# YuliangXiu/ICON

Measured on AMD Instinct MI355X. Metric: query-points/sec at 256^3 grid, higher is better.
Workload: dtype f32 via 3x f16 split MFMA (22-bit operands, f32 accumulate)

## Files before the change

icon_amd/_lib.py:

```python
from __future__ import annotations

import ctypes as C
import os
import subprocess

_HERE = os.path.dirname(os.path.abspath(__file__))
LIB_PATH = os.environ.get("ICON_AMD_LIB") or os.path.join(_HERE, "libicon_amd.so")
CSRC = os.path.join(_HERE, "csrc")

PRIOR = {"icon": 0, "pamir": 1, "pifu": 2}
CMAP = {"reference": 0, "local": 1}
SEARCH = {"bvh": 0, "brute": 1}
PRECISION = {"f32": 0, "f16x3": 1}

SYMBOLS = [
    "icon_last_error", "icon_version", "icon_device_count",
    "icon_mesh_create", "icon_mesh_destroy", "icon_mesh_vertex_normals", "icon_mesh_stats",
    "icon_mesh_arena_bytes", "icon_mesh_create_arena", "icon_mesh_status", "icon_debug_set_mesh_build", "icon_debug_mesh_layout", "icon_debug_host_mesh_build",
    "icon_sdf_query",
    "icon_feat_create", "icon_feat_destroy", "icon_feat_set_smpl_feats",
    "icon_mlp_create", "icon_mlp_destroy", "icon_mlp_forward", "icon_mlp_set_last_op",
    "icon_work_create", "icon_work_destroy", "icon_work_profile", "icon_work_stage_ms", "icon_work_profile_detail", "icon_work_profile_workgroups", "icon_work_set_steal", "icon_work_set_reserve_cus",
    "icon_query_points", "icon_query_points_dcalib", "icon_query_rows", "icon_grid_rows",
    "icon_volume_any_above", "icon_adaptive_eval", "icon_adaptive_counts", "icon_adaptive_reruns", "icon_grid_eval_slab", "icon_grid_slab_features", "icon_grid_slab_finish", "icon_grid_slab_features_msg",
    "icon_grid_slab_finish_gathered", "icon_debug_set_shell_skip", "icon_debug_set_option", "icon_work_status", "icon_sdf_query_ties", "icon_work_set_tie_rule",
    "icon_export_mesh", "icon_mc_count", "icon_mc_emit", "icon_mc_count_range", "icon_mc_emit_keyed", "icon_debug_traversal_stats", "icon_debug_set_unfused",
    "icon_visibility", "icon_mesh_components", "icon_clean_mesh", "icon_semantic_voxelize",
    "icon_mesh_batch_create", "icon_mesh_batch_destroy", "icon_mesh_batch_status", "icon_feat_create_batch", "icon_query_points_batch",
    "icon_feat_batch_set_volume", "icon_semantic_voxelize_batch",
    "icon_query_color_bytes", "icon_query_color",
    "icon_render_bytes", "icon_render_normal",
    "icon_silhouette_bytes", "icon_silhouette_forward", "icon_silhouette_backward",
    "icon_render_normal_backward_bytes", "icon_render_normal_backward",
]

_lib = None


class IconAmdError(RuntimeError):
    pass


def build(force: bool = False) -> str:
    args = ["make", "-j8", "-C", CSRC] + (["-B"] if force else [])
    proc = subprocess.run(args, stdout=subprocess.PIPE, stderr=subprocess.STDOUT, text=True)
    if proc.returncode != 0:
        raise IconAmdError("building libicon_amd.so failed:\n" + proc.stdout[-4000:])
    return LIB_PATH


def lib():
    global _lib
    if _lib is not None:
        return _lib
    if not os.path.exists(LIB_PATH):
        raise IconAmdError(f"{LIB_PATH} not found - run `python -c 'import __graft_entry__ as g; g.build()'` "
                           "or `make -C icon_amd/csrc` (needs hipcc); there is no CPU fallback")
    import torch
    L = C.CDLL(LIB_PATH)
    L.icon_last_error.restype = C.c_char_p
    for name in SYMBOLS:
        if name != "icon_last_error":
            getattr(L, name).restype = C.c_int
    _lib = L
    return L


def check(rc: int, what: str = "") -> None:
    if rc != 0:
        msg = lib().icon_last_error().decode("utf-8", "replace")
        raise IconAmdError(f"{what or 'icon_amd'} failed (code {rc}): {msg}")


def device_count() -> int:
    return int(lib().icon_device_count())


def require_device() -> None:
    if device_count() < 1:
        raise IconAmdError("icon_amd needs a HIP device (MI355X); none is visible and there is no CPU fallback")


def ptr(t) -> C.c_void_p:
    if t is None:
        return C.c_void_p(0)
    if hasattr(t, "data_ptr"):
        assert t.is_contiguous(), "tensor must be contiguous"
        return C.c_void_p(t.data_ptr())
    return C.c_void_p(t.ctypes.data)
```

icon_amd/csrc/common.h:

```cpp
#pragma once
#include <hip/hip_runtime.h>
#include <stdint.h>
#include <functional>
#include <string>
#include <vector>

#include "../../include/icon_amd.h"

namespace icon {
constexpr int kWgRec = 6;
constexpr int kMaxProfGrid = 1024;

void set_error(const std::string &msg);
int fail(int code, const std::string &msg);

#define ICON_HIP(expr)                                                                          \
    do {                                                                                        \
        hipError_t _e = (expr);                                                                 \
        if (_e != hipSuccess)                                                                   \
            return ::icon::fail(ICON_ERR_HIP, std::string(#expr) + ": " + hipGetErrorString(_e)); \
    } while (0)

#define ICON_ARG(cond, msg)                                                  \
    do {                                                                     \
        if (!(cond)) return ::icon::fail(ICON_ERR_ARG, std::string(msg));    \
    } while (0)

struct alignas(64) BvhNode {
    float lo[3][2], hi[3][2];
    int32_t child0, child1;
    int32_t pad[2];
};
static_assert(sizeof(BvhNode) == 64, "BvhNode must be 64 bytes");

struct alignas(16) TriRec {
    float a[3], b[3], c[3];
    int32_t ia, ib, ic;
};
static_assert(sizeof(TriRec) == 48, "TriRec must be 48 bytes");

struct alignas(16) TriAttr {
    float n[3][3];
    float cm[3][3];
    float vis[3];
    int32_t face;
    int32_t pad[2];
};
static_assert(sizeof(TriAttr) == 96, "TriAttr must be 96 bytes");

struct alignas(32) TriPre {
    float a[3], b[3], ab[3], ac[3], bc[3];
    float i00, i11, ibc, a00, a01, a11, inn;
    int32_t face;
    int32_t pad;
};
static_assert(sizeof(TriPre) == 96, "TriPre must be 96 bytes");

struct alignas(32) LeafRec {
    float pair[2][24][2];
};
static_assert(sizeof(LeafRec) == 384, "LeafRec must be 384 bytes");

constexpr int kLeafMax = 4;
constexpr int kShareWavesMany = 8, kShareWavesFew = 16;
inline int share_waves(int64_t packets) { return packets <= 1500 ? kShareWavesFew : (packets <= 8000 ? kShareWavesMany : 1); }
constexpr int kStackDepth = 48;
constexpr int kXRow = 16;
constexpr int kCodeSlot = 15;

constexpr uint32_t kCodeOutlier = 1u;
constexpr uint32_t kCodeSignShift = 1;
constexpr uint32_t kCodeInCube = 8u;
constexpr uint32_t kCodeInside = 16u;

constexpr int kScanBlock = 256;
constexpr int kMaxWorld = 64;

struct MeshDyn {
    int32_t root;
    int32_t gy, gz;
    float bin_y0, bin_z0, bin_y1, bin_z1, bin_inv_y, bin_inv_z;
    float box_lo[3], box_hi[3];
    int32_t n_nodes, n_leaves, depth, bin_entries, max_bin;
    int32_t status;
    int32_t pad[11];
};
static_assert(sizeof(MeshDyn) == 128, "MeshDyn layout");
constexpr int kMeshBadFace = 1;
constexpr int kMeshBadVertex = 2;
constexpr int kMeshBinOverflow = 4;
constexpr int kMeshInternal = 8;
constexpr int kMeshBuilt = 0x100;

struct MeshDev {
    const BvhNode *nodes;
    const TriRec *tris;
    const TriAttr *attr;
    const int32_t *slot2face;
    const int32_t *face2slot;
    const LeafRec *leaves;
    const MeshDyn *dyn;
    int32_t n_tris;
    const int32_t *bin_start;
    const int32_t *bin_slots;
};

struct FeatDev {
    const float *planes;
    const float *vol;
    int32_t C, H, W, n_select, csel, cpad;
    int32_t Cv, Dv, Hv, Wv, vpad;
    int32_t smpl_mask;
};
constexpr int kSmplCmap = 1, kSmplNorm = 2;

struct BilinearTaps {
    int x0, y0;
    float nw, ne, sw, se;
    bool bx0, bx1, by0, by1;
};
__device__ __forceinline__ BilinearTaps bilinear_taps(float x, float y, int H, int W)
{
    BilinearTaps t;
    const float ix = ((x + 1.0f) / 2.0f) * (float)(W - 1);
    const float iy = ((y + 1.0f) / 2.0f) * (float)(H - 1);
    const float fx = floorf(ix), fy = floorf(iy);
    t.x0 = (int)fx; t.y0 = (int)fy;
    const int x1 = t.x0 + 1, y1 = t.y0 + 1;
    t.nw = ((float)x1 - ix) * ((float)y1 - iy);
    t.ne = (ix - (float)t.x0) * ((float)y1 - iy);
    t.sw = ((float)x1 - ix) * (iy - (float)t.y0);
    t.se = (ix - (float)t.x0) * (iy - (float)t.y0);
    t.bx0 = t.x0 >= 0 && t.x0 < W; t.bx1 = x1 >= 0 && x1 < W; t.by0 = t.y0 >= 0 && t.y0 < H; t.by1 = y1 >= 0 && y1 < H;
    return t;
}

struct Calib { float m[12]; const float *d; };

struct Lattice {
    int32_t res, z0, z1;
};

struct LatticeMap {
    int res, z0, nz;
    int tx, ty, tz;
    int remap;
    int off;
    int zs, nzi;
    int sx0, sx1, sy0, sy1;
    int sz0, sz1;
    int trim;
    float trim_need;
    int pk;
};

__device__ __forceinline__ bool not_finite(float y)
{
    uint32_t u = __float_as_uint(y);
    asm volatile("" : "+v"(u));
    return (u & 0x7f800000u) == 0x7f800000u;
}

__device__ __forceinline__ float apply_last_op(float y, int last_op)
{
    return last_op == ICON_LASTOP_SIGMOID ? 1.0f / (1.0f + expf(-y)) : y;
}

struct NearRef { uint16_t *lo; uint8_t *hi; float *d2; const int32_t *map; };

enum { kSignNone = 0, kSignSelf = 1, kSignGlobal = 2, kSignSeg = 3 };
struct FusedSigns {
    int mode;
    const int8_t *list;
    const int64_t *k_dev;
    int64_t k_host, rank_offset;
    const int8_t *gathered;
    int64_t stride;
    int world, rank;
};

struct BatchDev {
    const MeshDev *meshes;
    const float *calibs;
    int64_t n;
    int64_t plane_stride;
    int B;
    int64_t vol_stride;
};
enum class Src { Lattice, Points, Batch };

}

struct icon_mesh {
    int64_t V = 0, F = 0;
    char *arena = nullptr;
    size_t arena_bytes = 0;
    bool owns_arena = false;
    float *d_vnormals = nullptr;
    icon::MeshDyn *d_dyn = nullptr;
    icon::MeshDyn *h_dyn = nullptr;
    hipEvent_t built = nullptr;
    int depth_bound = 0;
    icon::MeshDev dev{};
};

struct icon_feat {
    float *d_planes = nullptr;
    float *d_vol = nullptr;
    icon::FeatDev dev{};
    int batch = 1;
    int64_t plane_stride = 0;
    int64_t vol_stride = 0;
};

struct icon_mesh_batch {
    int B = 0;
    int64_t V = 0, F = 0;
    int depth_bound = 0;
    std::vector<const icon_mesh *> subj;
    icon::MeshDev *d_table = nullptr;
    icon::MeshDev *h_table = nullptr;
    int *h_status = nullptr;
    hipEvent_t done = nullptr;
};

struct icon_adaptive;
struct icon_mlp {
    int c0 = 0;
    int last_op = 0;
    float *d_blob = nullptr;
    size_t blob_bytes = 0;
    size_t off_w0 = 0, off_b0 = 0, off_w1 = 0, off_b1 = 0, off_w2 = 0, off_w2x = 0, off_b2 = 0, off_w3 = 0;
    size_t off_plain = 0;
    size_t off_flag = 0;
    float b3 = 0.f;
    char *d_f16 = nullptr;
    float f16_inv[3] = {1.f, 1.f, 1.f};
};

namespace icon {
void parallel_for(int n, const std::function<void(int)> &fn);
void debug_sync(const char *what, hipStream_t st);
struct MeshLayout;
int mesh_host_state_get(MeshDyn **h, hipEvent_t *ev);
void mesh_host_state_put(MeshDyn *h, hipEvent_t ev);
void mesh_bind_arena(icon_mesh *m, const MeshLayout &L);
int mesh_build_device(icon_mesh *m, const float *d_verts, const int64_t *d_faces, const float *d_cmap, const float *d_vis, hipStream_t st);
void adaptive_destroy(icon_adaptive *a);
inline int lattice_packet()
{
    static const int pk_env = getenv("ICON_AMD_PACKET") ? atoi(getenv("ICON_AMD_PACKET")) : 0;
    return pk_env == 2 ? 2 : 4;
}
int outlier_list_dev(icon_work *w, const int *n_dev, int64_t n_max, hipStream_t st);
int ensure_work_points(icon_work *w, int64_t n_points);
struct McDevState;
void mc_destroy(McDevState *s);
struct CleanState;
void clean_destroy(CleanState *s);
int morton_order(icon_work *w, const float *d_points, const float *calib12, const float *d_calib12, int64_t N, hipStream_t st, const int32_t **perm);
int mlp_launch(const icon_mlp *mlp, const float *d_x, int64_t N, float *d_out, int precision, hipStream_t st);
int mlp_launch_ex(const icon_mlp *mlp, const float *d_x, int64_t N, float *d_out, bool mask, hipStream_t st);
int mlp_rescue_rows(const icon_mlp *mlp, const float *d_x, int64_t N, float *d_out, hipStream_t st);
int mlp_flag_reset(const icon_mlp *mlp, hipStream_t st);
int rescue_always();
int mlp_pack_f16x3(icon_mlp *m, const std::vector<std::vector<float>> &W, const std::vector<std::vector<float>> &B, hipStream_t st);
int mlp_launch_f16x3(const icon_mlp *mlp, const float *d_x, int64_t N, float *d_out, bool mask, hipStream_t st);
uint16_t f32_to_f16_rtn(float f);
float f16_to_f32(uint16_t h);
float pick_scale(const std::vector<float> &W);
int launch_sign(const icon_mesh *mesh, const Calib &cal, int res, int z0, const float *d_points, int64_t N, float sdf_clip,
                const icon_work *work, bool lattice, hipStream_t st, const BatchDev *bd = nullptr);
int launch_fused_f16x3(const icon_mesh *mesh, const icon_feat *feat, const icon_mlp *mlp, int prior, const Calib &cal,
                       const LatticeMap &L, int za, int zb, const float *d_points, int64_t N, float sdf_clip, int cmap_local,
                       const icon_work *work, const FusedSigns &fs, float *d_occ, bool lattice, hipStream_t st,
                       const BatchDev *bd = nullptr);
int morton_order_batch(icon_work *w, const float *d_points, const float *d_calibs, int64_t n, int B, hipStream_t st, const int32_t **perm);
int ensure_work(icon_work *w, int64_t n_points, bool need_x);
int outlier_list(icon_work *w, int64_t N, int8_t *signs, bool counted, hipStream_t st);
int patch_self(icon_work *w, int64_t N, int cmap_slot, hipStream_t st);
bool want_fused(int precision, int search);
void mark(icon_work *w, int k, hipStream_t st);
int device_cu_count(int *n_cu);
int once_per_device(int kernel_id, const std::function<hipError_t()> &set);
struct LatticeFast;
struct ShareDbg {
    int *err;
    int ring, lose, spin_log2;
};
int work_share_dbg(icon_work *w, ShareDbg *out);
int work_check_err(icon_work *w);
extern int g_qc_lanes;
extern int g_rn_lanes;
int share_waves_override();
}

struct icon_work {
    float *d_x = nullptr;
    int64_t cap_x = 0;
    uint16_t *d_near16 = nullptr;
    uint8_t *d_near_hi = nullptr;
    float *d_near_d2 = nullptr;
    int64_t cap_points_hi = 0;
    uint8_t *d_code8 = nullptr;
    int64_t cap_points = 0;
    uint64_t *d_grp_mask = nullptr;
    int32_t *d_block_counts = nullptr;
    int64_t *d_block_offsets = nullptr;
    int32_t *d_scan_local = nullptr;
    int64_t *d_scan_part = nullptr;
    int64_t cap_blocks = 0;
    int8_t *d_signs = nullptr;
    int64_t cap_signs = 0;
    int64_t *d_total = nullptr;
    int *d_flag = nullptr;
    mutable bool flag_clean = false;
    int64_t *d_seg = nullptr;
    int32_t *d_row_count = nullptr;
    int32_t *d_row_slots = nullptr;
    int64_t cap_rows = 0;
    int *h_err = nullptr;
    icon::LatticeFast *d_lfast = nullptr;
    uint32_t *d_sort_keys = nullptr;
    int32_t *d_sort_idx = nullptr;
    void *d_sort_tmp = nullptr;
    size_t sort_tmp_bytes = 0;
    int64_t cap_sort = 0;
    int slab_res = 0, slab_z0 = 0, slab_z1 = 0, slab_c0 = 0, slab_cmap_slot = 0;
    bool slab_ready = false, slab_needs_patch = false, slab_patched = false;
    int tie_rule = 0, tie_ulps = 0;
    const icon_mesh *q_mesh = nullptr;
    const icon_feat *q_feat = nullptr;
    int q_prior = 0, q_cmap_mode = 0, q_search = 0;
    float q_sdf_clip = 0.f;
    icon::Calib q_cal{};
    icon::LatticeMap q_L{};
    const float *q_points = nullptr;
    int64_t q_N = 0;
    bool q_lattice = false, q_rows_ready = false;
    const int32_t *q_map = nullptr;
    const int *q_n_dev = nullptr;
    int reserve_cus = 0;
    int *h_any = nullptr;
    int *defer_range_flag = nullptr;
    int range_reruns = 0;
    struct icon_adaptive *ad = nullptr;
    icon::McDevState *mc = nullptr;
    icon::CleanState *clean = nullptr;
    bool prof = false;
    hipEvent_t ev[6] = {nullptr, nullptr, nullptr, nullptr, nullptr, nullptr};
    bool ev_search = false;
    unsigned long long *d_clock = nullptr;
    mutable int clock_grid = 0;
    double clock_kernel_ms = 0.0;
    unsigned int *d_steal = nullptr;
    int steal_permille = 150, steal_grp = 2;
    bool ev_valid = false;
};

namespace icon {
constexpr int kNearLoSlots = 32768;
inline NearRef work_near(const icon_work *w, const icon_mesh *mesh)
{
    NearRef r;
    r.lo = w->d_near16; r.d2 = w->d_near_d2;
    r.hi = (mesh && mesh->F > kNearLoSlots) ? w->d_near_hi : nullptr;
    r.map = w->q_map;
    return r;
}
}
```

icon_amd/csrc/geom_device.h:

```cpp
#pragma once
#pragma clang fp contract(off)

#include "common.h"
#include "mesh_rules.h"

#include <cstdlib>
#include <cstring>

namespace icon {

struct f3 { float x, y, z; };
__device__ __forceinline__ f3 mk3(float x, float y, float z) { f3 r; r.x = x; r.y = y; r.z = z; return r; }
__device__ __forceinline__ f3 sub3(f3 a, f3 b) { return mk3(a.x - b.x, a.y - b.y, a.z - b.z); }
__device__ __forceinline__ float dot3(f3 a, f3 b) { return fmaf(a.z, b.z, fmaf(a.y, b.y, a.x * b.x)); }
__device__ __forceinline__ f3 cross3(f3 a, f3 b)
{
    return mk3(fmaf(a.y, b.z, -(a.z * b.y)), fmaf(a.z, b.x, -(a.x * b.z)), fmaf(a.x, b.y, -(a.y * b.x)));
}

struct TriC {
    f3 a, b, ab, ac, bc;
    float i00, i11, ibc, a00, a01, a11, inn;
};

// ... 27 lines not shown
{
    TriC t;
    t.a = mk3(q[0], q[1], q[2]); t.b = mk3(q[3], q[4], q[5]); t.ab = mk3(q[6], q[7], q[8]);
    t.ac = mk3(q[9], q[10], q[11]); t.bc = mk3(q[12], q[13], q[14]);
    t.i00 = q[15]; t.i11 = q[16]; t.ibc = q[17]; t.a00 = q[18]; t.a01 = q[19]; t.a11 = q[20]; t.inn = q[21];
    return t;
}

typedef float f2 __attribute__((ext_vector_type(2)));
typedef __attribute__((address_space(4))) const f2 cf2;
struct f3x2 { f2 x, y, z; };
__device__ __forceinline__ f2 bc2(float v) { f2 r; r.x = v; r.y = v; return r; }
__device__ __forceinline__ f2 fma2(f2 a, f2 b, f2 c) { return __builtin_elementwise_fma(a, b, c); }
__device__ __forceinline__ f3x2 sub3x2(f3x2 a, f3x2 b) { f3x2 r; r.x = a.x - b.x; r.y = a.y - b.y; r.z = a.z - b.z; return r; }
__device__ __forceinline__ f2 dot3x2(f3x2 a, f3x2 b) { return fma2(a.z, b.z, fma2(a.y, b.y, a.x * b.x)); }
__device__ __forceinline__ f2 clamp01x2(f2 v)
{
    f2 r; r.x = fminf(fmaxf(v.x, 0.0f), 1.0f); r.y = fminf(fmaxf(v.y, 0.0f), 1.0f); return r;
}
__device__ __forceinline__ f2 seg_dist2x2(f3x2 po, f3x2 e, f2 dot_e_po, f2 inv_len2)
{
    f2 t;
    asm("v_pk_mul_f32 %0, %1, %2 clamp" : "=v"(t) : "v"(dot_e_po), "s"(inv_len2));
    const f2 nt = -t;
    f3x2 d; d.x = fma2(nt, e.x, po.x); d.y = fma2(nt, e.y, po.y); d.z = fma2(nt, e.z, po.z);
    return dot3x2(d, d);
}

__device__ __forceinline__ f2 tri_dist2_pair(f3 p1, cf2 *q)
{
    f3x2 p; p.x = bc2(p1.x); p.y = bc2(p1.y); p.z = bc2(p1.z);
    f3x2 a, b, ab, ac, bc;
    a.x = q[0]; a.y = q[1]; a.z = q[2]; b.x = q[3]; b.y = q[4]; b.z = q[5];
    ab.x = q[6]; ab.y = q[7]; ab.z = q[8]; ac.x = q[9]; ac.y = q[10]; ac.z = q[11]; bc.x = q[12]; bc.y = q[13]; bc.z = q[14];
    const f2 i00 = q[15], i11 = q[16], ibc = q[17], a00 = q[18], a01 = q[19], a11 = q[20], inn = q[21];
    const f3x2 ap = sub3x2(p, a), bp = sub3x2(p, b);
    const f2 d1 = dot3x2(ab, ap), d2 = dot3x2(ac, ap), d3 = dot3x2(bc, bp);
    const f2 s = fma2(a11, d1, -(a01 * d2)) * inn;
    const f2 u = fma2(a00, d2, -(a01 * d1)) * inn;
    const f2 su = s + u;
    const bool in0 = (s.x >= 0.0f) & (u.x >= 0.0f) & (su.x <= 1.0f);
    const bool in1 = (s.y >= 0.0f) & (u.y >= 0.0f) & (su.y <= 1.0f);
    const f2 e0 = seg_dist2x2(ap, ab, d1, i00);
    const f2 e1 = seg_dist2x2(ap, ac, d2, i11);
    const f2 e2 = seg_dist2x2(bp, bc, d3, ibc);
    f2 r; r.x = fminf(fminf(e0.x, e1.x), e2.x); r.y = fminf(fminf(e0.y, e1.y), e2.y);
    if (__any(in0 | in1)) {
        const f2 ns = -s, nu = -u;
        f3x2 df; df.x = fma2(nu, ac.x, fma2(ns, ab.x, ap.x)); df.y = fma2(nu, ac.y, fma2(ns, ab.y, ap.y)); df.z = fma2(nu, ac.z, fma2(ns, ab.z, ap.z));
        const f2 d_face = dot3x2(df, df);
        float f0 = d_face.x, f1 = d_face.y, g0 = r.x, g1 = r.y;
        asm volatile("" : "+v"(f0), "+v"(f1), "+v"(g0), "+v"(g1));
        r.x = in0 ? f0 : g0; r.y = in1 ? f1 : g1;
    }
    return r;
}

__device__ __forceinline__ float edge_fn(float yi, float zi, float yj, float zj, float qy, float qz)
{
    const float t1 = (yi - qy) * (zj - qz);
    return fmaf(-(zi - qz), (yj - qy), t1);
}
__device__ __forceinline__ bool edge_side(float yi, float zi, float yj, float zj, float e)
{
    if (e > 0.0f) return true;
    if (e < 0.0f) return false;
    const float dz = zj - zi, dy = yj - yi;
    if (dz != 0.0f) return dz < 0.0f;
    return dy > 0.0f;
}
__device__ __forceinline__ void oriented_edge(int ia, f3 a, int ib, f3 b, float qy, float qz, float &val, bool &pos)
{
    if (ia < ib) { const float e = edge_fn(a.y, a.z, b.y, b.z, qy, qz); val = e; pos = edge_side(a.y, a.z, b.y, b.z, e); }
    else         { const float e = edge_fn(b.y, b.z, a.y, a.z, qy, qz); val = -e; pos = !edge_side(b.y, b.z, a.y, a.z, e); }
}
__device__ __forceinline__ int ray_hit(f3 p, f3 a, f3 b, f3 c, int ia, int ib, int ic)
{
    float e_ab, e_bc, e_ca; bool s_ab, s_bc, s_ca;
    oriented_edge(ia, a, ib, b, p.y, p.z, e_ab, s_ab);
    oriented_edge(ib, b, ic, c, p.y, p.z, e_bc, s_bc);
    oriented_edge(ic, c, ia, a, p.y, p.z, e_ca, s_ca);
    if (!(s_ab == s_bc && s_bc == s_ca)) return 0;
    const float num = fmaf(e_ab, c.x - p.x, fmaf(e_ca, b.x - p.x, e_bc * (a.x - p.x)));
    return s_ab ? (num > 0.0f) : (num < 0.0f);
}

typedef __attribute__((address_space(4))) const float cfloat;
__device__ __forceinline__ cfloat *as_const(const void *p) { return (cfloat *)(uintptr_t)p; }

__device__ __forceinline__ void load_tri_pos_uniform(const TriRec *t, f3 &a, f3 &b, f3 &c)
{
    cfloat *q = as_const(t);
    a = mk3(q[0], q[1], q[2]); b = mk3(q[3], q[4], q[5]); c = mk3(q[6], q[7], q[8]);
}

__device__ __forceinline__ void load_tri_pos(const TriRec *t, f3 &a, f3 &b, f3 &c)
{
    const float4 *q = reinterpret_cast<const float4 *>(t);
    const float4 q0 = q[0], q1 = q[1];
    const float q2 = reinterpret_cast<const float *>(t)[8];
    a = mk3(q0.x, q0.y, q0.z); b = mk3(q0.w, q1.x, q1.y); c = mk3(q1.z, q1.w, q2);
}
__device__ __forceinline__ void load_tri_full(const TriRec *t, f3 &a, f3 &b, f3 &c, int &ia, int &ib, int &ic)
{
    const float4 *q = reinterpret_cast<const float4 *>(t);
    const float4 q0 = q[0], q1 = q[1], q2 = q[2];
    a = mk3(q0.x, q0.y, q0.z); b = mk3(q0.w, q1.x, q1.y); c = mk3(q1.z, q1.w, q2.x);
    ia = __float_as_int(q2.y); ib = __float_as_int(q2.z); ic = __float_as_int(q2.w);
}

__host__ __device__ inline float far_box_dist2(float sdf_clip)
{
    const float cb = (sdf_clip > 0.0f ? sdf_clip : 0.0f) * 1.7320508f;
    return cb * cb * 1.0001f + 1e-6f;
}

__device__ __forceinline__ float box_dist2(float lx, float ly, float lz, float hx, float hy, float hz, f3 p)
{
    const float dx = fmaxf(fmaxf(lx - p.x, p.x - hx), 0.0f);
    const float dy = fmaxf(fmaxf(ly - p.y, p.y - hy), 0.0f);
    const float dz = fmaxf(fmaxf(lz - p.z, p.z - hz), 0.0f);
    return fmaf(dz, dz, fmaf(dy, dy, dx * dx));
}

__device__ __forceinline__ f2 box_dist2_pair(cf2 *q, f3 p)
{
    const f2 px = bc2(p.x), py = bc2(p.y), pz = bc2(p.z);
    const f2 ax = q[0] - px, bx = px - q[3];
    const f2 ay = q[1] - py, by = py - q[4];
    const f2 az = q[2] - pz, bz = pz - q[5];
    f2 dx, dy, dz;
    dx.x = fmaxf(fmaxf(ax.x, bx.x), 0.0f); dx.y = fmaxf(fmaxf(ax.y, bx.y), 0.0f);
    dy.x = fmaxf(fmaxf(ay.x, by.x), 0.0f); dy.y = fmaxf(fmaxf(ay.y, by.y), 0.0f);
    dz.x = fmaxf(fmaxf(az.x, bz.x), 0.0f); dz.y = fmaxf(fmaxf(az.y, bz.y), 0.0f);
    return fma2(dz, dz, fma2(dy, dy, dx * dx));
}

struct Nearest { float d2; int slot; int face; };

__device__ __forceinline__ int mesh_root(const MeshDev &m)
{
    return __builtin_amdgcn_readfirstlane(*reinterpret_cast<__attribute__((address_space(4))) const int *>((uintptr_t)&m.dyn->root));
}

__device__ __forceinline__ float prune_threshold(float best)
{
    return fmaf(best, 1.000083f, 2.1e-7f);
}

template <bool STATS = false, bool TIES = false>
__device__ __forceinline__ Nearest nearest_packet(const MeshDev &m, f3 p, bool live, int *wstack ,
                                                  int *n_nodes = nullptr, int *n_tris = nullptr, float thr0 = INFINITY,
                                                  unsigned long long *runner_up = nullptr, int center_lane = 21,
                                                  bool have_root = false, int root = 0)
{
    Nearest nr; nr.d2 = INFINITY; nr.slot = 0; nr.face = 0x7fffffff;
    unsigned long long key = 0x7f8000007fffffffull;
    unsigned long long key2 = 0x7f8000007fffffffull;
    float thr = live ? thr0 : -INFINITY;
    int sp = 0;
    int cur = have_root ? root : mesh_root(m);
    while (true) {
        if (cur < 0) {
            const int code = ~cur;
            const int leaf = code >> 2, cnt = (code & 3) + 1;
            if (STATS) *n_tris += cnt;
            const int npairs = __builtin_amdgcn_readfirstlane((cnt + 1) >> 1);
            for (int pr = 0; pr < npairs; ++pr) {
                cf2 *q = reinterpret_cast<cf2 *>(as_const(&m.leaves[leaf].pair[pr]));
                const f2 d2 = tri_dist2_pair(p, q);
                const f2 fc = q[22];
                const unsigned long long k0 = ((unsigned long long)(unsigned)__float_as_int(d2.x) << 32) | (unsigned)__float_as_int(fc.x);
                const unsigned long long k1 = ((unsigned long long)(unsigned)__float_as_int(d2.y) << 32) | (unsigned)__float_as_int(fc.y);
                if (TIES) {
                    if (k0 < key) { key2 = key; key = k0; } else if (k0 != key && k0 < key2) key2 = k0;
                    if (k1 < key) { key2 = key; key = k1; } else if (k1 != key && k1 < key2) key2 = k1;
                } else {
                    key = (k0 < key) ? k0 : key;
                    key = (k1 < key) ? k1 : key;
                }
            }
            nr.d2 = __int_as_float((int)(key >> 32));
            thr = live ? prune_threshold(nr.d2) : thr;
            if (sp == 0) break;
            cur = __builtin_amdgcn_readfirstlane(wstack[--sp]);
        } else {
            if (STATS) ++*n_nodes;
            cf2 *q = reinterpret_cast<cf2 *>(as_const(m.nodes + cur));
            const f2 dd = box_dist2_pair(q, p);
            const float d0 = dd.x, d1 = dd.y;
            const f2 ids = q[6];
            const int c0 = __float_as_int(ids.x), c1 = __float_as_int(ids.y);
            const bool v0 = __any(d0 <= thr), v1 = __any(d1 <= thr);
            if (v0 && v1) {
                const int e0 = __builtin_amdgcn_readlane(__float_as_int(d0), center_lane);
                const int e1 = __builtin_amdgcn_readlane(__float_as_int(d1), center_lane);
                const bool first0 = e0 <= e1;
                wstack[sp++] = first0 ? c1 : c0;
                cur = first0 ? c0 : c1;
            } else if (v0) cur = c0;
            else if (v1) cur = c1;
            else {
                if (sp == 0) break;
                cur = __builtin_amdgcn_readfirstlane(wstack[--sp]);
            }
        }
    }
    nr.d2 = __int_as_float((int)(key >> 32)); nr.face = (int)(key & 0xffffffffu);
    nr.slot = (nr.face != 0x7fffffff) ? m.face2slot[nr.face] : 0;
    if (TIES) *runner_up = key2;
    return nr;
}

constexpr int kRing = 64, kRingEmpty = 0x7fffffff;
constexpr int kShareSpinLog2 = 18;
constexpr int kShareErrPop = 1;
constexpr int kShareErrPush = 2;
constexpr int kShareErrIdle = 3;
struct ShareLds {
    unsigned thr[64];
    int head, tail, avail, active;
    int mask, lose, spins, pad1;
    int pad[8];
    int ring[kRing];
    unsigned long long keys[1];
};
__host__ __device__ constexpr size_t share_lds_bytes(int nw) { return sizeof(ShareLds) + (size_t)nw * 64 * 8; }

constexpr int kShareErrClaimed = -1;
__device__ __forceinline__ void share_report(const ShareDbg &dbg, int code, int ticket, const ShareLds &S)
{
    if (!dbg.err) return;
    int expected = 0;
    if (__hip_atomic_compare_exchange_strong(dbg.err, &expected, kShareErrClaimed, __ATOMIC_RELAXED, __ATOMIC_RELAXED, __HIP_MEMORY_SCOPE_SYSTEM)) {
        dbg.err[1] = (int)blockIdx.x; dbg.err[2] = ticket;
        dbg.err[3] = *(volatile const int *)&S.head; dbg.err[4] = *(volatile const int *)&S.tail;
        dbg.err[5] = *(volatile const int *)&S.avail; dbg.err[6] = *(volatile const int *)&S.active;
        dbg.err[7] = (int)(threadIdx.x >> 6);
        __threadfence_system();
        __hip_atomic_store(dbg.err, code, __ATOMIC_RELEASE, __HIP_MEMORY_SCOPE_SYSTEM);
    }
}

__device__ __forceinline__ int share_pop(ShareLds &S, int lane, const ShareDbg &dbg)
{
    int t = 0;
    if (lane == 0) t = atomicSub(&S.avail, 1);
    t = __builtin_amdgcn_readfirstlane(t);
    if (t <= 0) { if (lane == 0) atomicAdd(&S.avail, 1); return kRingEmpty; }
    int i = 0;
    if (lane == 0) i = atomicAdd(&S.head, 1);
    i = __builtin_amdgcn_readfirstlane(i);
    volatile int *slot = &S.ring[i & S.mask];
    int v = __builtin_amdgcn_readfirstlane(*slot);
    for (int spins = 0; v == kRingEmpty; ++spins) {
        if (spins >= S.spins) {
            if (lane == 0) share_report(dbg, kShareErrPop, i, S);
            return kRingEmpty;
        }
        __builtin_amdgcn_s_sleep(1);
        v = __builtin_amdgcn_readfirstlane(*slot);
    }
    if (lane == 0) *slot = kRingEmpty;
    return v;
}
__device__ __forceinline__ bool share_push(ShareLds &S, int lane, int node, const ShareDbg &dbg)
{
    int ok = 1;
    if (lane == 0) {
        const int i = atomicAdd(&S.tail, 1);
        if (i == S.lose) {
            atomicAdd(&S.avail, 1);
        } else {
            int spins = 0;
            while (atomicCAS(&S.ring[i & S.mask], kRingEmpty, node) != kRingEmpty) {
                if (++spins >= S.spins) { ok = 0; break; }
                __builtin_amdgcn_s_sleep(1);
            }
            if (ok) atomicAdd(&S.avail, 1);
            else share_report(dbg, kShareErrPush, i, S);
        }
    }
    return __builtin_amdgcn_readfirstlane(ok) != 0;
}

template <int NW>
__device__ __forceinline__ Nearest nearest_shared(const MeshDev &m, f3 p, bool live, int *wstack, char *smem , int center_lane,
                                                  const ShareDbg &dbg)
{
    ShareLds &S = *reinterpret_cast<ShareLds *>(smem);
    const int lane = threadIdx.x & 63, wave = threadIdx.x >> 6;
    __syncthreads();
    if (threadIdx.x < 64) { S.thr[lane] = 0x7f800000u; S.ring[lane] = lane == 0 ? mesh_root(m) : kRingEmpty; }
    if (threadIdx.x == 0) {
        S.head = 0; S.tail = 1; S.avail = 1; S.active = NW;
        S.mask = (dbg.ring >= 2 && dbg.ring <= kRing ? dbg.ring : kRing) - 1;
        S.lose = dbg.lose > 0 ? dbg.lose : -1;
        S.spins = 1 << (dbg.spin_log2 > 0 && dbg.spin_log2 < 30 ? dbg.spin_log2 : kShareSpinLog2);
    }
    __syncthreads();
    unsigned long long key = 0x7f8000007fffffffull;
    float thr = live ? INFINITY : -INFINITY;
    int sp = 0;
    while (true) {
        int cur;
        if (sp > 0) cur = __builtin_amdgcn_readfirstlane(wstack[--sp]);
        else {
            cur = share_pop(S, lane, dbg);
            if (cur == kRingEmpty) {
                if (lane == 0) atomicSub(&S.active, 1);
                int spins = 0;
                while (true) {
                    const int av = __builtin_amdgcn_readfirstlane(*(volatile int *)&S.avail);
                    const int ac = __builtin_amdgcn_readfirstlane(*(volatile int *)&S.active);
                    if (av > 0) {
                        if (lane == 0) atomicAdd(&S.active, 1);
                        cur = share_pop(S, lane, dbg);
                        if (cur != kRingEmpty) break;
                        if (lane == 0) atomicSub(&S.active, 1);
                    } else if (ac <= 0) break;
                    if (++spins > (4 << kShareSpinLog2)) { if (lane == 0) share_report(dbg, kShareErrIdle, spins, S); break; }
// ... 651 lines not shown
```

icon_amd/csrc/mesh_build.cpp:

```cpp
#include <algorithm>
#include <chrono>
#include <cmath>
#include <cstdio>
#include <cstdlib>
#include <cstring>
#include <limits>
#include <atomic>
#include <condition_variable>
#include <mutex>
#include <numeric>
#include <thread>

#include "common.h"
#include "mesh_rules.h"

namespace icon {

static thread_local std::string g_err;
void set_error(const std::string &msg) { g_err = msg; }
int fail(int code, const std::string &msg) { g_err = msg; return code; }
const char *last_error_cstr() { return g_err.c_str(); }

void debug_sync(const char *what, hipStream_t st)
{
// ... 44 lines not shown
            std::lock_guard<std::mutex> lk(mu);
            fn = &f; n = nn; next.store(0); active = n_workers; ++epoch;
        }
        cv_start.notify_all();
        for (int i = next.fetch_add(1); i < nn; i = next.fetch_add(1)) f(i);
        std::unique_lock<std::mutex> lk(mu);
        cv_done.wait(lk, [&] { return active == 0; });
    }
};

Pool *pool_instance()
{
    static Pool *p = [] {
        const int hw = (int)std::min(16u, std::max(1u, std::thread::hardware_concurrency()));
        return hw > 1 ? new Pool(hw - 1) : nullptr;
    }();
    return p;
}
}

void parallel_for(int n, const std::function<void(int)> &fn)
{
    int nt = (int)std::min(16u, std::max(1u, std::thread::hardware_concurrency()));
    if (const char *e = getenv("ICON_AMD_BUILD_THREADS")) nt = std::max(atoi(e), 1);
    static thread_local bool in_section = false;
    Pool *p = (nt > 1 && n > 1 && !in_section) ? pool_instance() : nullptr;
    if (p && p->job_mu.try_lock()) {
        in_section = true;
        p->run(n, [&](int i) { in_section = true; fn(i); });
        in_section = false;
        p->job_mu.unlock();
        return;
    }
    for (int i = 0; i < n; ++i) fn(i);
}

namespace {

struct V3 { float x, y, z; };
inline V3 sub(V3 a, V3 b) { return {a.x - b.x, a.y - b.y, a.z - b.z}; }
inline V3 cross(V3 a, V3 b)
{
    return {fmaf(a.y, b.z, -(a.z * b.y)), fmaf(a.z, b.x, -(a.x * b.z)), fmaf(a.x, b.y, -(a.y * b.x))};
}

struct HostBuild {
    int64_t V, F;
    int bound;
    std::vector<float> tbox, cen;
    std::vector<int32_t> order, tmp;
    std::vector<BvhNode> nodes;
    std::vector<uint8_t> leaf_cnt;
    MeshDyn dyn{};

    void link(int parent, int side, int ref, const float box[6])
    {
        if (parent < 0) { dyn.root = ref; return; }
        BvhNode &nd = nodes[parent];
        for (int a = 0; a < 3; ++a) { nd.lo[a][side] = box[a]; nd.hi[a][side] = box[3 + a]; }
        if (side) nd.child1 = ref; else nd.child0 = ref;
    }

    void bounds(int a, int b, float box[6], float cb[6]) const
    {
        for (int k = 0; k < 3; ++k) { box[k] = INFINITY; box[3 + k] = -INFINITY; cb[k] = INFINITY; cb[3 + k] = -INFINITY; }
        for (int i = a; i < b; ++i) {
            const int e = order[i];
            for (int k = 0; k < 3; ++k) {
                box[k] = fminf(box[k], tbox[6 * (size_t)e + k]); box[3 + k] = fmaxf(box[3 + k], tbox[6 * (size_t)e + 3 + k]);
                cb[k] = fminf(cb[k], cen[3 * (size_t)e + k]); cb[3 + k] = fmaxf(cb[3 + k], cen[3 * (size_t)e + k]);
            }
        }
    }

    void build(int begin, int end, int depth, int parent, int side, const float box[6], const float cb[6])
    {
        const int n = end - begin;
        if (n <= kLeafMax) {
            leaf_cnt[begin] = (uint8_t)n;
            link(parent, side, ~((begin << 2) | (n - 1)), box);
            dyn.n_leaves++; dyn.depth = std::max(dyn.depth, depth);
            return;
        }
        float lo[3], ext[3];
        for (int a = 0; a < 3; ++a) { lo[a] = cb[a]; ext[a] = cb[3 + a] - cb[a]; }
        bool valid = false;
        int best_axis = 0, best_bin = 0, nleft = 0;
        float cbox[2][6], ccb[2][6];
        if (!force_median(depth, n, bound)) {
            double best = std::numeric_limits<double>::infinity();
            for (int ax = 0; ax < 3; ++ax) {
                if (!(ext[ax] > 0.0f)) continue;
                int cnt[kSahBins] = {0};
                float bb[kSahBins][6], bc[kSahBins][6];
                for (int b = 0; b < kSahBins; ++b)
                    for (int k = 0; k < 3; ++k) { bb[b][k] = INFINITY; bb[b][3 + k] = -INFINITY; bc[b][k] = INFINITY; bc[b][3 + k] = -INFINITY; }
                for (int i = begin; i < end; ++i) {
                    const int e = order[i];
                    const int b = sah_bin(cen[3 * (size_t)e + ax], lo[ax], ext[ax]);
                    cnt[b]++;
                    for (int k = 0; k < 3; ++k) {
                        bb[b][k] = fminf(bb[b][k], tbox[6 * (size_t)e + k]); bb[b][3 + k] = fmaxf(bb[b][3 + k], tbox[6 * (size_t)e + 3 + k]);
                        bc[b][k] = fminf(bc[b][k], cen[3 * (size_t)e + k]); bc[b][3 + k] = fmaxf(bc[b][3 + k], cen[3 * (size_t)e + k]);
                    }
                }
                for (int b = 0; b < kSahBins - 1; ++b) {
                    float sb[2][6], sc[2][6];
                    int c2[2] = {0, 0};
                    for (int s = 0; s < 2; ++s)
                        for (int k = 0; k < 3; ++k) { sb[s][k] = INFINITY; sb[s][3 + k] = -INFINITY; sc[s][k] = INFINITY; sc[s][3 + k] = -INFINITY; }
                    for (int q = 0; q < kSahBins; ++q) {
                        if (!cnt[q]) continue;
                        const int s = q <= b ? 0 : 1;
                        c2[s] += cnt[q];
                        for (int k = 0; k < 3; ++k) {
                            sb[s][k] = fminf(sb[s][k], bb[q][k]); sb[s][3 + k] = fmaxf(sb[s][3 + k], bb[q][3 + k]);
                            sc[s][k] = fminf(sc[s][k], bc[q][k]); sc[s][3 + k] = fmaxf(sc[s][3 + k], bc[q][3 + k]);
                        }
                    }
                    if (!c2[0] || !c2[1]) continue;
                    const double cost = box_area(sb[0], sb[0] + 3) * c2[0] + box_area(sb[1], sb[1] + 3) * c2[1];
                    if (cost < best) {
                        best = cost; valid = true; best_axis = ax; best_bin = b; nleft = c2[0];
                        memcpy(cbox, sb, sizeof(sb)); memcpy(ccb, sc, sizeof(sc));
                    }
                }
            }
        }
        if (valid) {
            int l = begin, r = 0;
            for (int i = begin; i < end; ++i) {
                const int e = order[i];
                if (sah_bin(cen[3 * (size_t)e + best_axis], lo[best_axis], ext[best_axis]) <= best_bin) order[l++] = e; else tmp[r++] = e;
            }
            for (int i = 0; i < r; ++i) order[l + i] = tmp[i];
        } else {
            nleft = n / 2;
            bounds(begin, begin + nleft, cbox[0], ccb[0]);
            bounds(begin + nleft, end, cbox[1], ccb[1]);
        }
        const int mid = begin + nleft, id = mid - 1;
        link(parent, side, id, box);
        dyn.n_nodes++;
        build(begin, mid, depth + 1, id, 0, cbox[0], ccb[0]);
        build(mid, end, depth + 1, id, 1, cbox[1], ccb[1]);
    }
};

struct HostArrays {
    MeshDyn dyn{};
    std::vector<float> vn;
    std::vector<BvhNode> nodes;
    std::vector<LeafRec> leafrec;
    std::vector<TriRec> tris;
    std::vector<TriAttr> attr;
    std::vector<int32_t> order, face2slot, bin_start, bin_slots;
};

int host_build(const std::vector<float> &verts, const std::vector<int64_t> &faces, const std::vector<float> &cmap, const std::vector<float> &vis,
               int64_t V, int64_t F, int bound, HostArrays &out)
{
    for (int64_t i = 0; i < 3 * F; ++i)
        ICON_ARG(faces[i] >= 0 && faces[i] < V, "icon_mesh_create: face index out of range");
    for (int64_t i = 0; i < 3 * V; ++i)
        ICON_ARG(!bad_coord(verts[i]), "icon_mesh_create: non-finite (or absurdly large) vertex coordinate");
    HostBuild hb;
    hb.V = V; hb.F = F; hb.bound = bound;

    std::vector<float> &vn = out.vn;
    vn.assign(3 * V, 0.f);
    for (int64_t f = 0; f < F; ++f) {
        const int64_t id[3] = {faces[3 * f], faces[3 * f + 1], faces[3 * f + 2]};
        const V3 a{verts[3 * id[0]], verts[3 * id[0] + 1], verts[3 * id[0] + 2]};
        const V3 b{verts[3 * id[1]], verts[3 * id[1] + 1], verts[3 * id[1] + 2]};
        const V3 c{verts[3 * id[2]], verts[3 * id[2] + 1], verts[3 * id[2] + 2]};
        const V3 n = cross(sub(b, a), sub(c, a));
        for (int k = 0; k < 3; ++k) { vn[3 * id[k]] += n.x; vn[3 * id[k] + 1] += n.y; vn[3 * id[k] + 2] += n.z; }
    }
    for (int64_t v = 0; v < V; ++v) {
        const float x = vn[3 * v], y = vn[3 * v + 1], z = vn[3 * v + 2];
        float len = sqrtf(fmaf(z, z, fmaf(y, y, x * x)));
        if (len < 1e-6f) len = 1e-6f;
        vn[3 * v] = x / len; vn[3 * v + 1] = y / len; vn[3 * v + 2] = z / len;
    }

    hb.tbox.resize(6 * F); hb.cen.resize(3 * F); hb.order.resize(F); hb.tmp.resize(F);
    hb.nodes.assign(F, BvhNode{}); hb.leaf_cnt.assign(F, 0);
    std::iota(hb.order.begin(), hb.order.end(), 0);
    float box[6], cb[6];
    for (int64_t f = 0; f < F; ++f)
        for (int a = 0; a < 3; ++a) {
            const float p0 = verts[3 * faces[3 * f] + a], p1 = verts[3 * faces[3 * f + 1] + a], p2 = verts[3 * faces[3 * f + 2] + a];
            const float lo = canon(fminf(fminf(p0, p1), p2)), hi = canon(fmaxf(fmaxf(p0, p1), p2));
            hb.tbox[6 * f + a] = lo; hb.tbox[6 * f + 3 + a] = hi; hb.cen[3 * f + a] = canon(0.5f * (lo + hi));
        }
    hb.bounds(0, (int)F, box, cb);
    hb.build(0, (int)F, 0, -1, 0, box, cb);
    MeshDyn &dyn = hb.dyn;
    for (int a = 0; a < 3; ++a) { dyn.box_lo[a] = box[a]; dyn.box_hi[a] = box[3 + a]; }
    const BinGrid g = bin_grid(dyn.box_lo, dyn.box_hi, F);
    dyn.gy = g.gy; dyn.gz = g.gz; dyn.bin_y0 = g.y0; dyn.bin_z0 = g.z0; dyn.bin_y1 = g.y1; dyn.bin_z1 = g.z1; dyn.bin_inv_y = g.inv_y; dyn.bin_inv_z = g.inv_z;

    const std::vector<int32_t> &order = hb.order;
    std::vector<TriRec> &tris = out.tris;
    std::vector<TriAttr> &attr = out.attr;
    std::vector<int32_t> &face2slot = out.face2slot;
    std::vector<LeafRec> &leafrec = out.leafrec;
    tris.resize(F); attr.resize(F); face2slot.resize(F); leafrec.resize(F);
    memset((void *)leafrec.data(), 0, sizeof(LeafRec) * F);
    for (int64_t p = 0; p < F; ++p) {
        const int64_t f = order[p];
        const int64_t id[3] = {faces[3 * f], faces[3 * f + 1], faces[3 * f + 2]};
        TriRec &tr = tris[p];
        for (int k = 0; k < 3; ++k) { tr.a[k] = verts[3 * id[0] + k]; tr.b[k] = verts[3 * id[1] + k]; tr.c[k] = verts[3 * id[2] + k]; }
        tr.ia = (int32_t)id[0]; tr.ib = (int32_t)id[1]; tr.ic = (int32_t)id[2];
        TriAttr &a = attr[p];
        for (int c = 0; c < 3; ++c) {
            for (int k = 0; k < 3; ++k) { a.n[c][k] = vn[3 * id[c] + k]; a.cm[c][k] = cmap[3 * id[c] + k]; }
            a.vis[c] = vis[id[c]];
        }
        a.face = (int32_t)f; a.pad[0] = a.pad[1] = 0;
        face2slot[f] = (int32_t)p;
    }
    for (int64_t L = 0; L < F; ++L) {
        const int cnt = hb.leaf_cnt[L];
        for (int t = 0; t < (cnt ? kLeafMax : 0); ++t) {
            const int64_t p = L + std::min(t, cnt - 1);
            TriPre pre;
            tri_setup(tris[p].a, tris[p].b, tris[p].c, order[p], pre);
            const float *src = reinterpret_cast<const float *>(&pre);
            for (int fld = 0; fld < 24; ++fld) leafrec[L].pair[t >> 1][fld][t & 1] = src[fld];
        }
    }

    const int64_t n_cells = (int64_t)g.gy * g.gz;
    std::vector<int32_t> &bin_start = out.bin_start;
    std::vector<int32_t> &bin_slots = out.bin_slots;
    bin_start.assign(n_cells + 1, 0);
    auto range = [&](int64_t p, int &cy0, int &cy1, int &cz0, int &cz1) {
        const float *tb = &hb.tbox[6 * (size_t)order[p]];
        cy0 = bin_cell_of(tb[1] - kBinEps, g.y0, g.inv_y, g.gy); cy1 = bin_cell_of(tb[4] + kBinEps, g.y0, g.inv_y, g.gy);
        cz0 = bin_cell_of(tb[2] - kBinEps, g.z0, g.inv_z, g.gz); cz1 = bin_cell_of(tb[5] + kBinEps, g.z0, g.inv_z, g.gz);
    };
    for (int64_t p = 0; p < F; ++p) {
        int cy0, cy1, cz0, cz1; range(p, cy0, cy1, cz0, cz1);
        for (int cz = cz0; cz <= cz1; ++cz)
            for (int cy = cy0; cy <= cy1; ++cy) bin_start[(size_t)cz * g.gy + cy + 1]++;
    }
    int64_t max_bin = 0, total = 0;
    for (int64_t i = 1; i <= n_cells; ++i) { max_bin = std::max<int64_t>(max_bin, bin_start[i]); total += bin_start[i]; }
    bin_slots.clear();
    if (total <= bin_entries_cap(F)) {
        for (int64_t i = 1; i <= n_cells; ++i) bin_start[i] += bin_start[i - 1];
        bin_slots.resize(total);
        std::vector<int32_t> fill(bin_start.begin(), bin_start.end() - 1);
        for (int64_t p = 0; p < F; ++p) {
            int cy0, cy1, cz0, cz1; range(p, cy0, cy1, cz0, cz1);
            for (int cz = cz0; cz <= cz1; ++cz)
                for (int cy = cy0; cy <= cy1; ++cy) bin_slots[fill[(size_t)cz * g.gy + cy]++] = (int32_t)p;
        }
        dyn.bin_entries = (int32_t)total; dyn.max_bin = (int32_t)max_bin;
    } else {
        std::fill(bin_start.begin(), bin_start.end(), 0);
        dyn.gy = dyn.gz = 0; dyn.status |= kMeshBinOverflow;
    }
    dyn.status |= kMeshBuilt;
    out.dyn = dyn;
    out.nodes.swap(hb.nodes);
    out.order.swap(hb.order);
    return ICON_OK;
}

template <class Put>
int emit_arena(const HostArrays &h, const MeshLayout &Ly, Put put_fn)
{
    int rc;
    std::vector<MeshDyn> dynv(1, h.dyn);
    if ((rc = put_fn(Ly.dyn, dynv.data(), sizeof(MeshDyn))) || (rc = put_fn(Ly.vnormals, h.vn.data(), h.vn.size() * 4)) ||
        (rc = put_fn(Ly.nodes, h.nodes.data(), h.nodes.size() * sizeof(BvhNode))) ||
        (rc = put_fn(Ly.leaves, h.leafrec.data(), h.leafrec.size() * sizeof(LeafRec))) ||
        (rc = put_fn(Ly.tris, h.tris.data(), h.tris.size() * sizeof(TriRec))) || (rc = put_fn(Ly.attr, h.attr.data(), h.attr.size() * sizeof(TriAttr))) ||
        (rc = put_fn(Ly.slot2face, h.order.data(), h.order.size() * 4)) || (rc = put_fn(Ly.face2slot, h.face2slot.data(), h.face2slot.size() * 4)) ||
        (rc = put_fn(Ly.bin_start, h.bin_start.data(), h.bin_start.size() * 4)) || (rc = put_fn(Ly.bin_slots, h.bin_slots.data(), h.bin_slots.size() * 4)))
        return rc;
    return ICON_OK;
}

int mesh_build_host(icon_mesh *m, const float *d_verts, const int64_t *d_faces, const float *d_cmap, const float *d_vis, hipStream_t st)
{
    const int64_t V = m->V, F = m->F;
    std::vector<float> verts(3 * V), cmap(3 * V), vis(V);
    std::vector<int64_t> faces(3 * F);
    ICON_HIP(hipMemcpyAsync(verts.data(), d_verts, sizeof(float) * 3 * V, hipMemcpyDeviceToHost, st));
    ICON_HIP(hipMemcpyAsync(faces.data(), d_faces, sizeof(int64_t) * 3 * F, hipMemcpyDeviceToHost, st));
    ICON_HIP(hipMemcpyAsync(cmap.data(), d_cmap, sizeof(float) * 3 * V, hipMemcpyDeviceToHost, st));
    ICON_HIP(hipMemcpyAsync(vis.data(), d_vis, sizeof(float) * V, hipMemcpyDeviceToHost, st));
    ICON_HIP(hipStreamSynchronize(st));
    HostArrays h;
    int rc = host_build(verts, faces, cmap, vis, V, F, m->depth_bound, h);
    if (rc) return rc;
    char *ar = m->arena;
    rc = emit_arena(h, mesh_layout(V, F), [&](size_t off, const void *src, size_t bytes) -> int {
        if (bytes) ICON_HIP(hipMemcpyAsync(ar + off, src, bytes, hipMemcpyHostToDevice, st));
        return ICON_OK;
    });
    if (rc) return rc;
    ICON_HIP(hipStreamSynchronize(st));
    *m->h_dyn = h.dyn;
    ICON_HIP(hipEventRecord(m->built, st));
    return ICON_OK;
}

int g_mesh_build_host = -1;

int mesh_create_common(const float *d_verts, int64_t V, const int64_t *d_faces, int64_t F, const float *d_cmap, const float *d_vis,
                       void *d_arena, size_t arena_bytes, bool owns, hipStream_t st, icon_mesh_t **out)
{
    icon_mesh *m = new icon_mesh();
    m->V = V; m->F = F; m->arena = (char *)d_arena; m->arena_bytes = arena_bytes; m->owns_arena = owns;
    m->depth_bound = depth_bound(F);
    int rc = mesh_host_state_get(&m->h_dyn, &m->built);
    if (rc) { icon_mesh_destroy(m); return rc; }
    mesh_bind_arena(m, mesh_layout(V, F));
    if (g_mesh_build_host < 0) { const char *e = getenv("ICON_AMD_MESH_BUILD"); g_mesh_build_host = (e && !strcmp(e, "host")) ? 1 : 0; }
    rc = g_mesh_build_host ? mesh_build_host(m, d_verts, d_faces, d_cmap, d_vis, st) : mesh_build_device(m, d_verts, d_faces, d_cmap, d_vis, st);
    if (rc) { icon_mesh_destroy(m); return rc; }
    *out = m;
    return ICON_OK;
}

int mesh_check_args(const float *d_verts, int64_t V, const int64_t *d_faces, int64_t F, const float *d_cmap, const float *d_vis, icon_mesh_t **out)
{
    ICON_ARG(out != nullptr, "icon_mesh_create: out is null");
    *out = nullptr;
    ICON_ARG(d_verts && d_faces && d_cmap && d_vis, "icon_mesh_create: null input pointer");
    ICON_ARG(V >= 3 && F >= 1, "icon_mesh_create: need V >= 3 and F >= 1");
    ICON_ARG(F <= (1 << 23) && V < (1ll << 31), "icon_mesh_create: mesh too large (more than 2^23 faces)");
    return ICON_OK;
}

}
}

using namespace icon;

extern "C" const char *icon_last_error(void) { return icon::last_error_cstr(); }
extern "C" int icon_version(void) { return ICON_AMD_VERSION; }
extern "C" int icon_device_count(void)
{
    int n = 0;
    if (hipGetDeviceCount(&n) != hipSuccess) { (void)hipGetLastError(); return 0; }
    return n;
}

extern "C" int icon_mesh_arena_bytes(int64_t V, int64_t F, int64_t *bytes)
{
    ICON_ARG(bytes != nullptr && V >= 3 && F >= 1 && F <= (1 << 23), "icon_mesh_arena_bytes: bad argument");
    *bytes = (int64_t)mesh_layout(V, F).total;
    return ICON_OK;
}

extern "C" int icon_mesh_create_arena(const float *d_verts, int64_t V, const int64_t *d_faces, int64_t F,
                                      const float *d_cmap, const float *d_vis, void *d_arena, int64_t arena_bytes,
                                      void *stream, icon_mesh_t **out)
{
    int rc = mesh_check_args(d_verts, V, d_faces, F, d_cmap, d_vis, out);
    if (rc) return rc;
    ICON_ARG(d_arena != nullptr && ((uintptr_t)d_arena & 255) == 0, "icon_mesh_create_arena: the arena must be 256-byte aligned device memory");
    ICON_ARG(arena_bytes >= (int64_t)mesh_layout(V, F).total, "icon_mesh_create_arena: arena smaller than icon_mesh_arena_bytes(V, F)");
    return mesh_create_common(d_verts, V, d_faces, F, d_cmap, d_vis, d_arena, (size_t)arena_bytes, false, (hipStream_t)stream, out);
}

extern "C" int icon_mesh_create(const float *d_verts, int64_t V, const int64_t *d_faces, int64_t F,
                                const float *d_cmap, const float *d_vis, void *stream, icon_mesh_t **out)
{
    int rc = mesh_check_args(d_verts, V, d_faces, F, d_cmap, d_vis, out);
    if (rc) return rc;
    const size_t bytes = mesh_layout(V, F).total;
    void *arena = nullptr;
    ICON_HIP(hipMalloc(&arena, bytes));
    rc = mesh_create_common(d_verts, V, d_faces, F, d_cmap, d_vis, arena, bytes, true, (hipStream_t)stream, out);
    if (rc && !*out) (void)hipFree(arena);
    return rc;
}

extern "C" int icon_mesh_destroy(icon_mesh_t *m)
{
    if (!m) return ICON_OK;
    if (m->owns_arena && m->arena) (void)hipFree(m->arena);
    mesh_host_state_put(m->h_dyn, m->built);
    delete m;
    return ICON_OK;
}

extern "C" int icon_debug_set_mesh_build(int host)
{
    icon::g_mesh_build_host = host ? 1 : 0;
    return ICON_OK;
}

extern "C" int icon_mesh_vertex_normals(const icon_mesh_t *m, float *d_out, void *stream)
{
    ICON_ARG(m && d_out, "icon_mesh_vertex_normals: null argument");
    ICON_HIP(hipMemcpyAsync(d_out, m->d_vnormals, sizeof(float) * 3 * m->V, hipMemcpyDeviceToDevice, (hipStream_t)stream));
    return ICON_OK;
}

extern "C" int icon_mesh_status(const icon_mesh_t *m, int wait, int *bits)
{
    ICON_ARG(m != nullptr, "icon_mesh_status: mesh is null");
    if (wait) ICON_HIP(hipEventSynchronize(m->built));
    const int st = *reinterpret_cast<const volatile int32_t *>(&m->h_dyn->status);
    if (!(st & kMeshBuilt)) { if (bits) *bits = -1; return ICON_OK; }
    if (bits) *bits = st & ~kMeshBuilt;
    if (st & kMeshBadFace) return fail(ICON_ERR_ARG, "icon_mesh_create: face index out of range");
    if (st & kMeshBadVertex) return fail(ICON_ERR_ARG, "icon_mesh_create: non-finite (or absurdly large) vertex coordinate");
    if (st & kMeshInternal) return fail(ICON_ERR_STATE, "icon_mesh_create: the device BVH build failed an internal check");
    return ICON_OK;
}

extern "C" int icon_mesh_stats(const icon_mesh_t *m, int64_t out[6])
{
    ICON_ARG(m && out, "icon_mesh_stats: null argument");
    ICON_HIP(hipEventSynchronize(m->built));
    const MeshDyn &d = *m->h_dyn;
    out[0] = d.n_nodes; out[1] = d.depth; out[2] = d.bin_entries; out[3] = d.max_bin; out[4] = d.n_leaves; out[5] = m->F;
    return ICON_OK;
}

extern "C" int icon_debug_host_mesh_build(const float *h_verts, int64_t V, const int64_t *h_faces, int64_t F,
                                          const float *h_cmap, const float *h_vis, void *h_arena, int64_t arena_bytes)
{
    ICON_ARG(h_verts && h_faces && h_cmap && h_vis && h_arena, "icon_debug_host_mesh_build: null argument");
    ICON_ARG(V >= 3 && F >= 1 && F <= (1 << 23), "icon_debug_host_mesh_build: bad sizes");
    const MeshLayout Ly = mesh_layout(V, F);
    ICON_ARG(arena_bytes >= (int64_t)Ly.total, "icon_debug_host_mesh_build: arena too small");
    std::vector<float> verts(h_verts, h_verts + 3 * V), cmap(h_cmap, h_cmap + 3 * V), vis(h_vis, h_vis + V);
    std::vector<int64_t> faces(h_faces, h_faces + 3 * F);
    HostArrays h;
    int rc = host_build(verts, faces, cmap, vis, V, F, depth_bound(F), h);
    if (rc) return rc;
    char *ar = (char *)h_arena;
    return emit_arena(h, Ly, [&](size_t off, const void *src, size_t bytes) -> int { if (bytes) memcpy(ar + off, src, bytes); return ICON_OK; });
}

extern "C" int icon_debug_mesh_layout(int64_t V, int64_t F, int64_t out[12])
{
    ICON_ARG(out && V >= 3 && F >= 1 && F <= (1 << 23), "icon_debug_mesh_layout: bad argument");
    const MeshLayout L = mesh_layout(V, F);
    const size_t v[12] = {L.dyn, L.vnormals, L.nodes, L.leaves, L.tris, L.attr, L.slot2face, L.face2slot, L.bin_start, L.bin_slots, L.tbox, L.total};
    for (int k = 0; k < 12; ++k) out[k] = (int64_t)v[k];
    return ICON_OK;
}
```

icon_amd/csrc/mesh_device.hip:

```cpp
#pragma clang fp contract(off)

#include "common.h"
#include "mesh_rules.h"

#include <cstring>
#include <mutex>
#include <vector>

namespace icon {

namespace {

struct BuildCtx {
    const float *verts; const int64_t *faces; const float *cmap; const float *vis;
    int32_t V, F, bound;
    MeshDyn *dyn; BuildHdr *hdr;
    int32_t *valence; uint8_t *leaf_cnt; BTask *tasks; uint32_t *hist; int32_t *cell_count, *cell_cursor;
    float *vnormals; BvhNode *nodes; LeafRec *leaves; TriRec *tris; TriAttr *attr; int32_t *slot2face, *face2slot;
    int32_t *bin_start, *bin_slots;
    float *tbox, *cen; int32_t *order[2]; int32_t *adj; int32_t *chunkcnt; int32_t *subq; struct STask *sublist; uint32_t *bounds_part;
    int32_t nck; int64_t cells_cap, entries_cap;
};

__device__ __forceinline__ uint32_t enc(float f) { const uint32_t u = __float_as_uint(f); return (u & 0x80000000u) ? ~u : (u | 0x80000000u); }
__device__ __forceinline__ float dec(uint32_t u) { return __uint_as_float((u & 0x80000000u) ? (u & 0x7fffffffu) : ~u); }
__device__ __forceinline__ uint32_t enc_min(float f) { return ~enc(f); }
__device__ __forceinline__ float dec_min(uint32_t u) { return dec(~u); }

template <bool GLOBAL = false>
__device__ __forceinline__ void wave_sync()
{
    if (GLOBAL) asm volatile("s_waitcnt vmcnt(0) lgkmcnt(0)" ::: "memory");
    else asm volatile("s_waitcnt lgkmcnt(0)" ::: "memory");
    __builtin_amdgcn_wave_barrier();
}

__device__ __forceinline__ float sane(float v, int *bad) { if (bad_coord(v)) { *bad = 1; return 0.0f; } return v; }

__device__ __forceinline__ void load_face(const BuildCtx &c, int f, int id[3], float p[3][3], int *bad_face, int *bad_vert)
{
    for (int k = 0; k < 3; ++k) {
        int64_t v = c.faces[3 * (int64_t)f + k];
        if (v < 0 || v >= c.V) { *bad_face = 1; v = 0; }
        id[k] = (int)v;
        for (int a = 0; a < 3; ++a) p[k][a] = sane(c.verts[3 * v + a], bad_vert);
    }
}

__global__ __launch_bounds__(256) void k_face_prep(BuildCtx c)
{
    const int f = blockIdx.x * 256 + threadIdx.x;
    const bool live = f < c.F;
    float lo[3] = {INFINITY, INFINITY, INFINITY}, hi[3] = {-INFINITY, -INFINITY, -INFINITY}, ce[3] = {0.f, 0.f, 0.f};
    int bf = 0, bv = 0;
    if (live) {
        int id[3]; float p[3][3];
        load_face(c, f, id, p, &bf, &bv);
        for (int a = 0; a < 3; ++a) {
            lo[a] = canon(fminf(fminf(p[0][a], p[1][a]), p[2][a]));
            hi[a] = canon(fmaxf(fmaxf(p[0][a], p[1][a]), p[2][a]));
            ce[a] = canon(0.5f * (lo[a] + hi[a]));
            c.tbox[6 * f + a] = lo[a]; c.tbox[6 * f + 3 + a] = hi[a]; c.cen[3 * f + a] = ce[a];
        }
        c.order[0][f] = f;
        if (!bf)
            for (int k = 0; k < 3; ++k) {
                const int pos = atomicAdd(&c.valence[id[k]], 1);
                if (pos < kAdjCap) c.adj[(size_t)id[k] * kAdjCap + pos] = 3 * f + k;
            }
        if (bf | bv) atomicOr(&c.dyn->status, (bf ? kMeshBadFace : 0) | (bv ? kMeshBadVertex : 0));
    }
    __shared__ uint32_t s_part[4][12];
    uint32_t u[12];
    for (int a = 0; a < 3; ++a) {
        u[a] = live ? enc_min(lo[a]) : 0u; u[3 + a] = live ? enc(hi[a]) : 0u;
        u[6 + a] = live ? enc_min(ce[a]) : 0u; u[9 + a] = live ? enc(ce[a]) : 0u;
    }
#pragma unroll
    for (int k = 0; k < 12; ++k) {
        uint32_t v = u[k];
        for (int d = 1; d < 64; d <<= 1) { const uint32_t o = (uint32_t)__shfl_xor((int)v, d); v = v > o ? v : o; }
        if ((threadIdx.x & 63) == 0) s_part[threadIdx.x >> 6][k] = v;
    }
    __syncthreads();
    if (threadIdx.x < 12) {
        const uint32_t a0 = s_part[0][threadIdx.x], a1 = s_part[1][threadIdx.x], a2 = s_part[2][threadIdx.x], a3 = s_part[3][threadIdx.x];
        const uint32_t m01 = a0 > a1 ? a0 : a1, m23 = a2 > a3 ? a2 : a3;
        c.bounds_part[(size_t)blockIdx.x * 12 + threadIdx.x] = m01 > m23 ? m01 : m23;
    }
}

__device__ __forceinline__ void face_normal(const BuildCtx &c, int f, float n[3])
{
    int id[3]; float p[3][3]; int bf = 0, bv = 0;
    load_face(c, f, id, p, &bf, &bv);
    const float ux = p[1][0] - p[0][0], uy = p[1][1] - p[0][1], uz = p[1][2] - p[0][2];
    const float vx = p[2][0] - p[0][0], vy = p[2][1] - p[0][1], vz = p[2][2] - p[0][2];
    n[0] = fmaf(uy, vz, -(uz * vy)); n[1] = fmaf(uz, vx, -(ux * vz)); n[2] = fmaf(ux, vy, -(uy * vx));
}

__global__ __launch_bounds__(256) void k_vertex_normals(BuildCtx c)
{
    const int v = blockIdx.x * 256 + threadIdx.x;
    __shared__ uint32_t s_red[256];
    if (blockIdx.x == 0) {
        const int nbF = (c.F + 255) / 256;
        const int k = threadIdx.x % 12, r0 = threadIdx.x / 12;
        uint32_t m = 0;
        if (threadIdx.x < 252)
            for (int r = r0; r < nbF; r += 21) { const uint32_t x = c.bounds_part[(size_t)r * 12 + k]; m = x > m ? x : m; }
        s_red[threadIdx.x] = m;
        __syncthreads();
        uint32_t mm = 0;
        if (threadIdx.x < 12)
            for (int g = 0; g < 21; ++g) { const uint32_t x = s_red[g * 12 + threadIdx.x]; mm = x > mm ? x : mm; }
        __syncthreads();
        if (threadIdx.x < 12) s_red[threadIdx.x] = mm;
        __syncthreads();
    }
    if (v == 0) {
        float box[6], cb[6];
        for (int a = 0; a < 3; ++a) {
            box[a] = dec_min(s_red[a]); box[3 + a] = dec(s_red[3 + a]);
            cb[a] = dec_min(s_red[6 + a]); cb[3 + a] = dec(s_red[9 + a]);
        }
        BTask &r = c.tasks[0];
        r.begin = 0; r.end = c.F; r.depth = 0; r.parent = -1; r.side = 0; r.buf = 0; r.from_atomics = 0;
        for (int k = 0; k < 6; ++k) { r.box[k] = box[k]; r.cb[k] = cb[k]; }
        if (c.F > kSubMax && kTopLevels > 0) r.kind = 1;
        else { r.kind = 2; c.subq[atomicAdd(&c.hdr->n_sub, 1)] = 0; }
        MeshDyn &d = *c.dyn;
        for (int a = 0; a < 3; ++a) { d.box_lo[a] = box[a]; d.box_hi[a] = box[3 + a]; }
        const BinGrid g = bin_grid(d.box_lo, d.box_hi, c.F);
        d.gy = g.gy; d.gz = g.gz; d.bin_y0 = g.y0; d.bin_z0 = g.z0; d.bin_y1 = g.y1; d.bin_z1 = g.z1; d.bin_inv_y = g.inv_y; d.bin_inv_z = g.inv_z;
    }
    if (v >= c.V) return;
    int bv = 0;
    for (int a = 0; a < 3; ++a) (void)sane(c.verts[3 * (int64_t)v + a], &bv);
    if (bv) atomicOr(&c.dyn->status, kMeshBadVertex);
    float x = 0.f, y = 0.f, z = 0.f;
    const int cnt = c.valence[v];
    if (cnt <= kAdjCap) {
        int e[kAdjCap];
        for (int k = 0; k < kAdjCap; ++k) e[k] = k < cnt ? c.adj[(size_t)v * kAdjCap + k] : 0x7fffffff;
        for (int i = 1; i < kAdjCap; ++i) {
            const int key = e[i];
            int j = i - 1;
            while (j >= 0 && e[j] > key) { e[j + 1] = e[j]; --j; }
            e[j + 1] = key;
        }
        for (int k = 0; k < cnt; ++k) {
            float n[3];
            face_normal(c, e[k] / 3, n);
            x += n[0]; y += n[1]; z += n[2];
        }
    } else {
        for (int f = 0; f < c.F; ++f) {
            int hit = 0; bool ok = true;
            for (int k = 0; k < 3; ++k) {
                const int64_t q = c.faces[3 * (int64_t)f + k];
                if (q < 0 || q >= c.V) ok = false;
                if (q == v) ++hit;
            }
            if (!ok || !hit) continue;
            float n[3];
            face_normal(c, f, n);
            for (int h = 0; h < hit; ++h) { x += n[0]; y += n[1]; z += n[2]; }
        }
    }
    float len = sqrtf(fmaf(z, z, fmaf(y, y, x * x)));
    if (len < 1e-6f) len = 1e-6f;
// ... 305 lines not shown
            hist_add(h, lo, ext, [&](int a) { return acc.cen(j, a); }, [&](int q) { return acc.tb(j, q); });
        }
        wave_sync<A::kGlobal>();
        sah_choose(h, ext, lane, D);
        wave_sync<A::kGlobal>();
        valid = D->valid != 0;
    }
    int nleft, cbuf;
    float cbox[2][6], ccb[2][6];
    if (valid) {
        const int axis = D->axis, bin = D->bin;
        nleft = D->nleft;
        for (int s = 0; s < 2; ++s)
            for (int k = 0; k < 6; ++k) { cbox[s][k] = D->cbox[s][k]; ccb[s][k] = D->ccb[s][k]; }
        int lb = 0, rb = nleft;
        const unsigned long long lt = (1ull << lane) - 1ull;
        const float lo_ax = axis == 0 ? lo[0] : (axis == 1 ? lo[1] : lo[2]), ext_ax = axis == 0 ? ext[0] : (axis == 1 ? ext[1] : ext[2]);
        for (int i0 = 0; i0 < n; i0 += 64) {
            const int i = i0 + lane;
            const bool act = i < n;
            const int j = act ? acc.get(t.buf, t.begin + i) : 0;
            const bool isl = act && sah_bin(acc.cen(j, axis), lo_ax, ext_ax) <= bin;
            const unsigned long long bl = __ballot(isl), br = __ballot(act && !isl);
            if (isl) acc.put(t.buf ^ 1, t.begin + lb + __popcll(bl & lt), j);
            else if (act) acc.put(t.buf ^ 1, t.begin + rb + __popcll(br & lt), j);
            lb += __popcll(bl); rb += __popcll(br);
        }
        if (lb != nleft && lane == 0) atomicOr(&c.dyn->status, kMeshInternal);
        cbuf = t.buf ^ 1;
        wave_sync<A::kGlobal>();
    } else {
        nleft = n / 2; cbuf = t.buf;
        range_bounds(acc, t.buf, t.begin, t.begin + nleft, lane, cbox[0], ccb[0]);
        range_bounds(acc, t.buf, t.begin + nleft, t.end, lane, cbox[1], ccb[1]);
    }
    const int mid = t.begin + nleft, id = mid - 1;
    if (lane == 0) { link_node(c, t.parent, t.side, id, t.box); atomicAdd(&S->n_nodes, 1); }
#pragma unroll
    for (int s = 0; s < 2; ++s) {
        STask ch;
        ch.begin = s ? mid : t.begin; ch.end = s ? t.end : mid; ch.depth = t.depth + 1; ch.parent = id; ch.side = s; ch.buf = cbuf;
        for (int k = 0; k < 6; ++k) { ch.box[k] = cbox[s][k]; ch.cb[k] = ccb[s][k]; }
        ch.pad[0] = ch.pad[1] = 0;
        if (ch.end - ch.begin <= kLeafMax) finalize_leaf(c, acc, S, ch, lane);
        else emit(ch);
    }
}

template <class A>
__device__ __forceinline__ void sub_levels(const BuildCtx &c, const A &acc, SubLds *S, STask *list0, STask *list1, int cap,
                                           int wave, int lane, int nwaves)
{
    for (int lv = 0;; ++lv) {
        __syncthreads();
        const int cur = lv & 1, nc = S->count[cur];
        if (nc == 0) break;
        STask *const lcur = cur ? list1 : list0, *const lnext = cur ? list0 : list1;
        for (int i = wave; i < nc; i += nwaves) {
            const STask t = lcur[i];
            process_node(c, acc, S, S->hist[wave], &S->dec[wave], t, lane, [&](const STask &ch) {
                int idx = 0;
                if (lane == 0) idx = atomicAdd(&S->count[cur ^ 1], 1);
                idx = __builtin_amdgcn_readfirstlane(idx);
                if (idx < cap) {
                    if (lane == 0) lnext[idx] = ch;
                } else if (lane == 0) {
                    atomicOr(&c.dyn->status, kMeshInternal);
                }
            });
        }
        __syncthreads();
        if (threadIdx.x == 0) S->count[cur] = 0;
    }
}

__global__ __launch_bounds__(kSubWaves * 64) void k_bvh_sub(BuildCtx c)
{
    extern __shared__ __attribute__((aligned(16))) char sub_smem[];
    SubLds *S = reinterpret_cast<SubLds *>(sub_smem);
    if ((int)blockIdx.x >= c.hdr->n_sub) return;
    const BTask &T = c.tasks[c.subq[blockIdx.x]];
    const int lane = threadIdx.x & 63, wave = threadIdx.x >> 6;
    const int n = T.end - T.begin;
    const bool in_lds = n <= kSubMax;
    if (threadIdx.x == 0) {
        STask r;
        r.begin = T.begin; r.end = T.end; r.depth = T.depth; r.parent = T.parent; r.side = T.side;
        r.buf = in_lds ? 0 : T.buf;
        task_bounds(T, r.box, r.cb);
        r.pad[0] = r.pad[1] = 0;
        (in_lds ? S->list[0] : c.sublist + (size_t)(T.begin / 5) * 2)[0] = r;
        S->count[0] = 1; S->count[1] = 0;
        S->n_nodes = 0; S->n_leaves = 0; S->depth = 0;
    }
    if (in_lds) {
        for (int i = threadIdx.x; i < n; i += kSubWaves * 64) {
            const int e = (T.buf ? c.order[1] : c.order[0])[T.begin + i];
            S->gid[i] = e; S->ord[0][i] = (uint16_t)i;
            for (int a = 0; a < 3; ++a) S->cen[i * 3 + a] = c.cen[3 * (size_t)e + a];
            for (int q = 0; q < 6; ++q) S->tbox[i * 6 + q] = c.tbox[6 * (size_t)e + q];
        }
        LdsAcc acc{S, T.begin};
        sub_levels(c, acc, S, S->list[0], S->list[1], kListCap, wave, lane, kSubWaves);
    } else {
        GlbAcc acc{{c.order[0], c.order[1]}, c.cen, c.tbox};
        STask *base = c.sublist + (size_t)(T.begin / 5) * 2;
        const int cap = n / 5;
        sub_levels(c, acc, S, base, base + cap, cap, wave, lane, kSubWaves);
    }
    if (threadIdx.x == 0) {
        if (S->n_nodes) atomicAdd(&c.dyn->n_nodes, S->n_nodes);
        atomicAdd(&c.dyn->n_leaves, S->n_leaves);
        atomicMax(&c.dyn->depth, S->depth);
    }
}

__device__ __forceinline__ BinGrid grid_of(const BuildCtx &c) { return bin_grid(c.dyn->box_lo, c.dyn->box_hi, c.F); }
__device__ __forceinline__ void cell_range(const BinGrid &g, const float *tb, int &cy0, int &cy1, int &cz0, int &cz1)
{
    cy0 = bin_cell_of(tb[1] - kBinEps, g.y0, g.inv_y, g.gy); cy1 = bin_cell_of(tb[4] + kBinEps, g.y0, g.inv_y, g.gy);
    cz0 = bin_cell_of(tb[2] - kBinEps, g.z0, g.inv_z, g.gz); cz1 = bin_cell_of(tb[5] + kBinEps, g.z0, g.inv_z, g.gz);
}

__global__ __launch_bounds__(256) void k_tri_records(BuildCtx c)
{
    const int p = blockIdx.x * 256 + threadIdx.x;
    if (p >= c.F) return;
    const int f = c.slot2face[p];
    int id[3]; float v[3][3]; int bf = 0, bv = 0;
    load_face(c, f, id, v, &bf, &bv);
    c.face2slot[f] = p;
    TriRec &tr = c.tris[p];
    for (int k = 0; k < 3; ++k) { tr.a[k] = v[0][k]; tr.b[k] = v[1][k]; tr.c[k] = v[2][k]; }
    tr.ia = id[0]; tr.ib = id[1]; tr.ic = id[2];
    TriAttr &at = c.attr[p];
    for (int q = 0; q < 3; ++q) {
        for (int k = 0; k < 3; ++k) { at.n[q][k] = c.vnormals[3 * (size_t)id[q] + k]; at.cm[q][k] = c.cmap[3 * (size_t)id[q] + k]; }
        at.vis[q] = c.vis[id[q]];
    }
    at.face = f; at.pad[0] = at.pad[1] = 0;
    int leaf = -1, myt = 0, cnt = 0;
    for (int t = 0; t < kLeafMax; ++t) {
        const int q = p - t;
        if (q >= 0 && c.leaf_cnt[q] > t) { leaf = q; myt = t; cnt = c.leaf_cnt[q]; break; }
    }
    if (leaf < 0) { atomicOr(&c.dyn->status, kMeshInternal); return; }
    TriPre pre;
    tri_setup(v[0], v[1], v[2], f, pre);
    const float *src = reinterpret_cast<const float *>(&pre);
    LeafRec &lr = c.leaves[leaf];
    const int tend = (myt == cnt - 1) ? kLeafMax : myt + 1;
    for (int t = myt; t < tend; ++t)
        for (int fld = 0; fld < 24; ++fld) lr.pair[t >> 1][fld][t & 1] = src[fld];
    const BinGrid g = grid_of(c);
    int cy0, cy1, cz0, cz1;
    cell_range(g, c.tbox + 6 * (size_t)f, cy0, cy1, cz0, cz1);
    for (int cz = cz0; cz <= cz1; ++cz)
        for (int cy = cy0; cy <= cy1; ++cy) atomicAdd(&c.cell_count[(size_t)cz * g.gy + cy], 1);
}

__global__ __launch_bounds__(1024) void k_scan_cells(BuildCtx c)
{
    __shared__ int wtot[16];
    const BinGrid g = grid_of(c);
    const int n = g.gy * g.gz;
    const int lane = threadIdx.x & 63, w = threadIdx.x >> 6;
    int64_t carry = 0;
    for (int base = 0; base < n; base += 4096) {
        const int i = base + (int)threadIdx.x * 4;
        int v[4];
#pragma unroll
        for (int k = 0; k < 4; ++k) v[k] = (i + k < n) ? c.cell_count[i + k] : 0;
        const int mine = v[0] + v[1] + v[2] + v[3];
        int incl = mine;
        for (int d = 1; d < 64; d <<= 1) { const int up = __shfl_up(incl, d); if (lane >= d) incl += up; }
        __syncthreads();
        if (lane == 63) wtot[w] = incl;
        __syncthreads();
        int before = 0, all = 0;
#pragma unroll
        for (int q = 0; q < 16; ++q) { const int t = wtot[q]; before += q < w ? t : 0; all += t; }
        int64_t run = carry + before + incl - mine;
#pragma unroll
        for (int k = 0; k < 4; ++k) { if (i + k < n) c.bin_start[i + k] = (int32_t)run; run += v[k]; }
        carry += all;
    }
    const bool fits = carry <= c.entries_cap;
    __syncthreads();
    if (!fits)
        for (int i = threadIdx.x; i <= n; i += 1024) c.bin_start[i] = 0;
    if (threadIdx.x == 0) {
        if (fits) c.bin_start[n] = (int32_t)carry;
        c.dyn->bin_entries = fits ? (int32_t)carry : 0;
        if (!fits) { c.dyn->gy = 0; c.dyn->gz = 0; atomicOr(&c.dyn->status, kMeshBinOverflow); }
    }
}

__global__ __launch_bounds__(256) void k_bin_fill(BuildCtx c)
{
    const int t = blockIdx.x * 256 + threadIdx.x;
    const int p = t >> 3, sub = t & 7;
    if (p >= c.F || (c.dyn->status & kMeshBinOverflow)) return;
    const BinGrid g = grid_of(c);
    int cy0, cy1, cz0, cz1;
    cell_range(g, c.tbox + 6 * (size_t)c.slot2face[p], cy0, cy1, cz0, cz1);
    int q = 0;
    for (int cz = cz0; cz <= cz1; ++cz)
        for (int cy = cy0; cy <= cy1; ++cy, ++q) {
            if ((q & 7) != sub) continue;
            const size_t cell = (size_t)cz * g.gy + cy;
            c.bin_slots[c.bin_start[cell] + atomicAdd(&c.cell_cursor[cell], 1)] = p;
        }
}

template <int N>
__device__ __forceinline__ void sort_regs(int32_t *q, int len)
{
    int v[N];
#pragma unroll
    for (int k = 0; k < N; ++k) v[k] = k < len ? q[k] : 0x7fffffff;
#pragma unroll
    for (int p = 1; p < N; p <<= 1)
#pragma unroll
        for (int k = p; k >= 1; k >>= 1)
#pragma unroll
            for (int j = k % p; j + k < N; j += 2 * k)
#pragma unroll
                for (int i = 0; i < k; ++i)
                    if (i + j + k < N && (i + j) / (2 * p) == (i + j + k) / (2 * p)) {
                        const int lo = min(v[i + j], v[i + j + k]), hi = max(v[i + j], v[i + j + k]);
                        v[i + j] = lo; v[i + j + k] = hi;
                    }
#pragma unroll
    for (int k = 0; k < N; ++k) if (k < len) q[k] = v[k];
}

__global__ __launch_bounds__(256) void k_bin_sort(BuildCtx c)
{
    const int64_t cell = (int64_t)blockIdx.x * 256 + threadIdx.x;
    if (cell == 0) atomicOr(&c.dyn->status, kMeshBuilt);
    if (c.dyn->status & kMeshBinOverflow) return;
    const BinGrid g = grid_of(c);
    const bool live = cell < (int64_t)g.gy * g.gz;
    const int a = live ? c.bin_start[cell] : 0, b = live ? c.bin_start[cell + 1] : 0, len = b - a;
    {
        int m = len;
        for (int d = 1; d < 64; d <<= 1) m = max(m, __shfl_xor(m, d));
        if ((threadIdx.x & 63) == 0 && m > 0) atomicMax(&c.dyn->max_bin, m);
    }
    int32_t *q = c.bin_slots + a;
    if (len > 1 && len <= 32) sort_regs<32>(q, len);
    else if (len > 32 && len <= 64) sort_regs<64>(q, len);
    else if (len > 64) {
        for (int i = 1; i < len; ++i) {
            const int key = q[i];
            int j = i - 1;
            while (j >= 0 && q[j] > key) { q[j + 1] = q[j]; --j; }
            q[j + 1] = key;
        }
    }
}

std::mutex g_pool_mu;
std::vector<MeshDyn *> g_free_dyn;
std::vector<hipEvent_t> g_free_ev;
std::vector<std::pair<MeshDyn *, hipEvent_t>> g_in_flight;

}

int mesh_host_state_get(MeshDyn **h, hipEvent_t *ev)
{
    std::lock_guard<std::mutex> lk(g_pool_mu);
    for (size_t i = 0; i < g_in_flight.size();) {
        if (hipEventQuery(g_in_flight[i].second) != hipErrorNotReady) {
            g_free_dyn.push_back(g_in_flight[i].first); g_free_ev.push_back(g_in_flight[i].second);
            g_in_flight[i] = g_in_flight.back(); g_in_flight.pop_back();
        } else ++i;
    }
    (void)hipGetLastError();
    if (g_free_dyn.empty()) {
        constexpr int kBatch = 32;
        MeshDyn *blk = nullptr;
        ICON_HIP(hipHostMalloc((void **)&blk, sizeof(MeshDyn) * kBatch, hipHostMallocDefault));
        for (int i = 0; i < kBatch; ++i) g_free_dyn.push_back(blk + i);
    }
    if (g_free_ev.empty()) {
        hipEvent_t e;
        ICON_HIP(hipEventCreateWithFlags(&e, hipEventDisableTiming));
        g_free_ev.push_back(e);
    }
    *h = g_free_dyn.back(); g_free_dyn.pop_back();
    *ev = g_free_ev.back(); g_free_ev.pop_back();
    memset(*h, 0, sizeof(MeshDyn));
    return ICON_OK;
}

void mesh_host_state_put(MeshDyn *h, hipEvent_t ev)
{
    std::lock_guard<std::mutex> lk(g_pool_mu);
    if (h && ev && hipEventQuery(ev) == hipErrorNotReady) { g_in_flight.emplace_back(h, ev); (void)hipGetLastError(); return; }
    (void)hipGetLastError();
    if (h) g_free_dyn.push_back(h);
    if (ev) g_free_ev.push_back(ev);
}

void mesh_bind_arena(icon_mesh *m, const MeshLayout &L)
{
    char *b = m->arena;
    m->d_dyn = reinterpret_cast<MeshDyn *>(b + L.dyn);
    m->d_vnormals = reinterpret_cast<float *>(b + L.vnormals);
    MeshDev &d = m->dev;
    d.nodes = reinterpret_cast<const BvhNode *>(b + L.nodes);
    d.tris = reinterpret_cast<const TriRec *>(b + L.tris);
    d.attr = reinterpret_cast<const TriAttr *>(b + L.attr);
    d.slot2face = reinterpret_cast<const int32_t *>(b + L.slot2face);
    d.face2slot = reinterpret_cast<const int32_t *>(b + L.face2slot);
    d.leaves = reinterpret_cast<const LeafRec *>(b + L.leaves);
    d.dyn = m->d_dyn;
    d.n_tris = (int32_t)m->F;
    d.bin_start = reinterpret_cast<const int32_t *>(b + L.bin_start);
    d.bin_slots = reinterpret_cast<const int32_t *>(b + L.bin_slots);
}

int mesh_build_device(icon_mesh *m, const float *d_verts, const int64_t *d_faces, const float *d_cmap, const float *d_vis, hipStream_t st)
{
    const MeshLayout L = mesh_layout(m->V, m->F);
    char *b = m->arena;
    BuildCtx c{};
    c.verts = d_verts; c.faces = d_faces; c.cmap = d_cmap; c.vis = d_vis;
    c.V = (int32_t)m->V; c.F = (int32_t)m->F; c.bound = m->depth_bound;
    c.dyn = reinterpret_cast<MeshDyn *>(b + L.dyn); c.hdr = reinterpret_cast<BuildHdr *>(b + L.hdr);
    c.valence = reinterpret_cast<int32_t *>(b + L.valence); c.leaf_cnt = reinterpret_cast<uint8_t *>(b + L.leaf_cnt);
    c.tasks = reinterpret_cast<BTask *>(b + L.tasks); c.hist = reinterpret_cast<uint32_t *>(b + L.hist);
    c.cell_count = reinterpret_cast<int32_t *>(b + L.cell_count); c.cell_cursor = reinterpret_cast<int32_t *>(b + L.cell_cursor);
    c.vnormals = reinterpret_cast<float *>(b + L.vnormals); c.nodes = reinterpret_cast<BvhNode *>(b + L.nodes);
    c.leaves = reinterpret_cast<LeafRec *>(b + L.leaves); c.tris = reinterpret_cast<TriRec *>(b + L.tris);
    c.attr = reinterpret_cast<TriAttr *>(b + L.attr); c.slot2face = reinterpret_cast<int32_t *>(b + L.slot2face);
    c.face2slot = reinterpret_cast<int32_t *>(b + L.face2slot); c.bin_start = reinterpret_cast<int32_t *>(b + L.bin_start);
    c.bin_slots = reinterpret_cast<int32_t *>(b + L.bin_slots); c.tbox = reinterpret_cast<float *>(b + L.tbox);
    c.cen = reinterpret_cast<float *>(b + L.cen); c.order[0] = reinterpret_cast<int32_t *>(b + L.order0);
    c.order[1] = reinterpret_cast<int32_t *>(b + L.order1); c.adj = reinterpret_cast<int32_t *>(b + L.adj);
    c.chunkcnt = reinterpret_cast<int32_t *>(b + L.chunkcnt); c.subq = reinterpret_cast<int32_t *>(b + L.subq);
    c.sublist = reinterpret_cast<STask *>(b + L.sublist); c.bounds_part = reinterpret_cast<uint32_t *>(b + L.bounds_part);
    c.nck = (int32_t)L.nck; c.cells_cap = bin_cells_cap(m->F); c.entries_cap = bin_entries_cap(m->F);

    ICON_HIP(hipMemsetAsync(b + L.dyn, 0, L.zero_end - L.dyn, st));
    const unsigned nbF = (unsigned)((m->F + 255) / 256), nbV = (unsigned)((m->V + 255) / 256);
    hipLaunchKernelGGL(k_face_prep, dim3(nbF), dim3(256), 0, st, c);
    debug_sync("k_face_prep", st);
    hipLaunchKernelGGL(k_vertex_normals, dim3(nbV), dim3(256), 0, st, c);
    debug_sync("k_vertex_normals", st);
    if (m->F > kSubMax) {
        for (int lv = 0; lv < kTopLevels; ++lv) {
            const unsigned nb = (unsigned)(m->F / kChunk + (1 << lv) + 1);
            hipLaunchKernelGGL(k_bvh_bin, dim3(nb), dim3(kChunk), 0, st, c, lv);
            hipLaunchKernelGGL(k_bvh_part, dim3(nb), dim3(kChunk), 0, st, c, lv);
            debug_sync("k_bvh_bin + k_bvh_part", st);
        }
    }
    static_assert(sizeof(SubLds) <= 160 * 1024 - 2048, "k_bvh_sub: LDS");
    {
        const int rc = once_per_device(8, [] { return hipFuncSetAttribute(reinterpret_cast<const void *>(k_bvh_sub), hipFuncAttributeMaxDynamicSharedMemorySize, (int)sizeof(SubLds)); });
        if (rc) return rc;
    }
    hipLaunchKernelGGL(k_bvh_sub, dim3((unsigned)(m->F > kSubMax ? kTaskSlots + 1 : 1)), dim3(kSubWaves * 64), sizeof(SubLds), st, c);
    debug_sync("k_bvh_sub", st);
    hipLaunchKernelGGL(k_tri_records, dim3(nbF), dim3(256), 0, st, c);
    debug_sync("k_tri_records", st);
    hipLaunchKernelGGL(k_scan_cells, dim3(1), dim3(1024), 0, st, c);
    hipLaunchKernelGGL(k_bin_fill, dim3((unsigned)((m->F * 8 + 255) / 256)), dim3(256), 0, st, c);
    hipLaunchKernelGGL(k_bin_sort, dim3((unsigned)((c.cells_cap + 255) / 256)), dim3(256), 0, st, c);
    debug_sync("ray bins", st);
    ICON_HIP(hipGetLastError());
    ICON_HIP(hipMemcpyAsync(m->h_dyn, c.dyn, sizeof(MeshDyn), hipMemcpyDeviceToHost, st));
    ICON_HIP(hipEventRecord(m->built, st));
    return ICON_OK;
}

}
```

icon_amd/csrc/mesh_rules.h:

```cpp
#pragma once
#include "common.h"

namespace icon {

__host__ __device__ inline int ilog2_ceil(int64_t n) { int l = 0; while (((int64_t)1 << l) < n) ++l; return l; }
__host__ __device__ inline int median_levels(int n) { int l = 0; while (n > kLeafMax) { n = (n + 1) / 2; ++l; } return l; }
__host__ __device__ inline int depth_bound(int64_t F)
{
    const int b = ilog2_ceil(F < 2 ? 2 : F) + 10;
    return b < kStackDepth - 2 ? b : kStackDepth - 2;
}
__host__ __device__ inline bool force_median(int depth, int n, int bound) { return depth + 1 + median_levels(n - 1) > bound; }

__host__ __device__ inline bool bad_coord(float v) { return !(v >= -1e6f && v <= 1e6f); }
__host__ __device__ inline float canon(float v) { return v + 0.0f; }

constexpr int kSahBins = 16;
__host__ __device__ inline int sah_bin(float c, float lo, float ext)
{
    int b = (int)((c - lo) / ext * (float)kSahBins);
    return b < 0 ? 0 : (b > kSahBins - 1 ? kSahBins - 1 : b);
}
struct BoxD { float lo[3], hi[3]; };
__host__ __device__ inline double box_area(const float lo[3], const float hi[3])
{
    const double dx0 = (double)hi[0] - lo[0], dy0 = (double)hi[1] - lo[1], dz0 = (double)hi[2] - lo[2];
    const double dx = dx0 > 0.0 ? dx0 : 0.0, dy = dy0 > 0.0 ? dy0 : 0.0, dz = dz0 > 0.0 ? dz0 : 0.0;
    return 2.0 * (dx * dy + dy * dz + dz * dx);
}

struct BinGrid { float y0, z0, y1, z1, inv_y, inv_z; int gy, gz; };
constexpr float kBinEps = 1e-5f;
__host__ __device__ inline BinGrid bin_grid(const float box_lo[3], const float box_hi[3], int64_t F)
{
    BinGrid g;
    g.y0 = box_lo[1] - 4 * kBinEps; g.y1 = box_hi[1] + 4 * kBinEps;
    g.z0 = box_lo[2] - 4 * kBinEps; g.z1 = box_hi[2] + 4 * kBinEps;
    const float ey = g.y1 - g.y0, ez = g.z1 - g.z0;
    float a = ey * ez;
    if (!(a > 1e-12f)) a = 1e-12f;
    const float cell = sqrtf(a / (2.0f * (float)F));
    int gy = (int)ceilf(ey / cell), gz = (int)ceilf(ez / cell);
    g.gy = gy < 1 ? 1 : (gy > 2048 ? 2048 : gy);
    g.gz = gz < 1 ? 1 : (gz > 2048 ? 2048 : gz);
    g.inv_y = (float)g.gy / ey; g.inv_z = (float)g.gz / ez;
    return g;
}
__host__ __device__ inline int bin_cell_of(float v, float v0, float inv, int g)
{
    const int c = (int)floorf((v - v0) * inv);
    return c < 0 ? 0 : (c > g - 1 ? g - 1 : c);
}
__host__ __device__ inline int64_t bin_cells_cap(int64_t F) { return 2 * F + 4100; }
__host__ __device__ inline int64_t bin_entries_cap(int64_t F) { return 48 * F + 2 * bin_cells_cap(F); }

__host__ __device__ inline float dot3r(const float *a, const float *b) { return fmaf(a[2], b[2], fmaf(a[1], b[1], a[0] * b[0])); }
__host__ __device__ inline void tri_setup(const float *a, const float *b, const float *c, int32_t face, TriPre &t)
{
    for (int k = 0; k < 3; ++k) { t.a[k] = a[k]; t.b[k] = b[k]; t.ab[k] = b[k] - a[k]; t.ac[k] = c[k] - a[k]; t.bc[k] = c[k] - b[k]; }
    t.a00 = dot3r(t.ab, t.ab); t.a01 = dot3r(t.ab, t.ac); t.a11 = dot3r(t.ac, t.ac);
    const float b11 = dot3r(t.bc, t.bc);
    t.i00 = (t.a00 > 0.0f) ? 1.0f / t.a00 : 0.0f;
    t.i11 = (t.a11 > 0.0f) ? 1.0f / t.a11 : 0.0f;
    t.ibc = (b11 > 0.0f) ? 1.0f / b11 : 0.0f;
    const float nn = fmaf(t.a00, t.a11, -(t.a01 * t.a01));
    t.inn = (nn > 0.0f) ? 1.0f / nn : __builtin_nanf("");
    t.face = face; t.pad = 0;
}

constexpr int kTopLevels = 7;
constexpr int kSubMax = 256;
constexpr int kChunk = 256;
constexpr int kAdjCap = 16;
constexpr int kHistWords = 3 * kSahBins * 13;
constexpr int kTaskSlots = (1 << (kTopLevels + 1)) - 1;

struct BTask {
    int32_t begin, end, depth, parent, side, kind, buf, from_atomics;
    float box[6], cb[6];
    uint32_t ubox[12];
};
static_assert(sizeof(BTask) == 128, "BTask layout");

struct BuildHdr {
    int32_t n_sub;
    int32_t pad[3];
};

struct MeshLayout {
    size_t dyn, hdr, valence, leaf_cnt, tasks, hist, cell_count, cell_cursor, zero_end;
    size_t vnormals, nodes, leaves, tris, attr, slot2face, face2slot, bin_start, bin_slots;
    size_t tbox, cen, order0, order1, adj, chunkcnt, subq, sublist, bounds_part, total;
    int64_t nck;
};
inline size_t align_up(size_t v, size_t a = 256) { return (v + a - 1) / a * a; }
inline MeshLayout mesh_layout(int64_t V, int64_t F)
{
    MeshLayout L{};
    size_t o = 0;
    auto take = [&](size_t bytes) { const size_t at = o; o = align_up(o + bytes); return at; };
    const int64_t cells = bin_cells_cap(F);
    L.nck = F / kChunk + (1 << kTopLevels) + 2;
    L.dyn = take(sizeof(MeshDyn));
    L.hdr = take(sizeof(BuildHdr));
    L.valence = take(sizeof(int32_t) * V);
    L.leaf_cnt = take((size_t)F);
    L.tasks = take(sizeof(BTask) * kTaskSlots);
    L.hist = take(sizeof(uint32_t) * kHistWords * ((1 << kTopLevels) - 1));
    L.cell_count = take(sizeof(int32_t) * (cells + 1));
    L.cell_cursor = take(sizeof(int32_t) * cells);
    L.zero_end = o;
    L.vnormals = take(sizeof(float) * 3 * V);
    L.nodes = take(sizeof(BvhNode) * F);
    L.leaves = take(sizeof(LeafRec) * F);
    L.tris = take(sizeof(TriRec) * F);
    L.attr = take(sizeof(TriAttr) * F);
    L.slot2face = take(sizeof(int32_t) * F);
    L.face2slot = take(sizeof(int32_t) * F);
    L.bin_start = take(sizeof(int32_t) * (cells + 1));
    L.bin_slots = take(sizeof(int32_t) * bin_entries_cap(F));
    L.tbox = take(sizeof(float) * 6 * F);
    L.cen = take(sizeof(float) * 3 * F);
    L.order0 = take(sizeof(int32_t) * F);
    L.order1 = take(sizeof(int32_t) * F);
    L.adj = take(sizeof(int32_t) * kAdjCap * V);
    L.chunkcnt = take(sizeof(int32_t) * 3 * kSahBins * L.nck * kTopLevels);
    L.subq = take(sizeof(int32_t) * (kTaskSlots + 1));
    L.sublist = take((size_t)80 * 2 * (F / 5 + 4));
    L.bounds_part = take(sizeof(uint32_t) * 12 * ((size_t)F / 256 + 1));
    L.total = o;
    return L;
}

}
```

icon_amd/csrc/query_kernels.hip:

```cpp
#pragma clang fp contract(off)

#include "query_device.h"

namespace icon {

template <bool BRUTE>
__global__ __launch_bounds__(kBlock) void k_sdf_query(MeshDev m, const float *__restrict__ pts, int64_t N,
                                                      float *sdf, float *nrm, float *cm, float *vis,
                                                      int64_t *face, uint8_t *inside_out, const int32_t *__restrict__ perm)
{
    __shared__ int lds[kBruteTile * 24];
    int64_t i = (int64_t)blockIdx.x * kBlock + threadIdx.x;
    const bool live = i < N;
    if (live && perm) i = perm[i];
    const int64_t ic = live ? i : (N - 1);
    const f3 p = clamp_raw(mk3(pts[3 * ic], pts[3 * ic + 1], pts[3 * ic + 2]));
    Nearest nr;
    bool ins;
    if (BRUTE) { nr = nearest_brute<kBlock>(m, p, reinterpret_cast<float *>(lds)); ins = inside_brute(m, p); }
    else       { nr = nearest_packet(m, p, live, lds + (threadIdx.x >> 6) * kStackDepth); ins = inside_bins(m, p); }
    if (!live) return;
    const SdfOut o = sdf_attrs(m, p, nr, ins);
    sdf[i] = o.sdf;
    nrm[3 * i] = o.nrm.x; nrm[3 * i + 1] = o.nrm.y; nrm[3 * i + 2] = o.nrm.z;
    cm[3 * i] = o.cm.x; cm[3 * i + 1] = o.cm.y; cm[3 * i + 2] = o.cm.z;
    vis[i] = o.vis;
    if (face) face[i] = nr.face;
    if (inside_out) inside_out[i] = ins ? 1 : 0;
}

__global__ __launch_bounds__(kCoopWaves * 64) void k_sdf_query_coop(MeshDev m, const float *__restrict__ pts, int64_t N,
                                                                   float *sdf, float *nrm, float *cm, float *vis,
                                                                   int64_t *face, uint8_t *inside_out, int cap)
{
    extern __shared__ __attribute__((aligned(16))) char coop_smem[];
    const int64_t i = (int64_t)blockIdx.x * kCoopWaves + (threadIdx.x >> 6);
    if (i >= N) return;
    const f3 p = clamp_raw(mk3(pts[3 * i], pts[3 * i + 1], pts[3 * i + 2]));
    const Nearest nr = nearest_coop(m, p, coop_lds(coop_smem, threadIdx.x >> 6, cap));
    if ((threadIdx.x & 63) != 0) return;
    const bool ins = inside_bins(m, p);
    const SdfOut o = sdf_attrs(m, p, nr, ins);
    sdf[i] = o.sdf;
    nrm[3 * i] = o.nrm.x; nrm[3 * i + 1] = o.nrm.y; nrm[3 * i + 2] = o.nrm.z;
    cm[3 * i] = o.cm.x; cm[3 * i + 1] = o.cm.y; cm[3 * i + 2] = o.cm.z;
    vis[i] = o.vis;
    if (face) face[i] = nr.face;
    if (inside_out) inside_out[i] = ins ? 1 : 0;
}

template <bool LATTICE, bool ALT = false>
__global__ __launch_bounds__(kBlock) void k_nearest(MeshDev m, Calib cal, LatticeMap L, const float *__restrict__ pts, int64_t N,
                                                    NearRef near, const int32_t *__restrict__ perm,
                                                    float sdf_clip, int tie_ulps, const LatticeFast *lf)
{
    __shared__ int lds[(kBlock / 64) * kStackDepth];
    int64_t i; bool live; f3 p;
    int root = 0;
    if (LATTICE) {
        int cx, cy, cz;
        if (lf) {
            const LatticeFast F = lattice_fast_load(lf);
            if ((int)blockIdx.x >= F.nb) return;
            live = lattice_point_fast(F, blockIdx.x, threadIdx.x >> 6, threadIdx.x & 63, cx, cy, cz);
            p = lattice_world_fast(lf, cx, cy, cz + L.z0);
            root = F.root;
        } else {
            L = lattice_trim(L, m);
            if ((int)blockIdx.x >= L.tx * L.ty * L.tz) return;
            int ix, iy, iz;
            live = lattice_point(L, ix, iy, iz);
            lattice_clamp(L, ix, iy, iz, cx, cy, cz);
            p = lattice_world(L.res, cx, cy, cz + L.z0);
            root = mesh_root(m);
        }
        i = ((int64_t)cz * L.res + cy) * L.res + cx;
    } else {
        i = (int64_t)blockIdx.x * kBlock + threadIdx.x;
        live = i < N;
        if (!live) i = N - 1;
        if (perm) i = perm[i];
        p = project(resolve_calib(cal), mk3(pts[3 * i], pts[3 * i + 1], pts[3 * i + 2]));
        root = mesh_root(m);
    }
    Nearest nr = nearest_packet(m, p, live, lds + (threadIdx.x >> 6) * kStackDepth, nullptr, nullptr, INFINITY, nullptr,
                                LATTICE ? packet_center_lane(L) : 21, true, root);
    if (ALT) nr = nearest_packet_alt(m, p, live, lds + (threadIdx.x >> 6) * kStackDepth, (uint32_t)__float_as_int(nr.d2), (uint32_t)tie_ulps);
    if (live) store_near(near, i, nr, sdf_clip);
}

template <int NW>
__global__ __launch_bounds__(NW * 64) void k_nearest_shared(MeshDev m, LatticeMap L, NearRef near, float sdf_clip, ShareDbg dbg)
{
    __shared__ int lds[NW * kStackDepth];
    __shared__ __attribute__((aligned(16))) char smem[share_lds_bytes(NW)];
    L = lattice_trim(L, m);
    if ((int)(blockIdx.x >> 2) >= L.tx * L.ty * L.tz) return;
    int ix, iy, iz, cx, cy, cz;
    const bool live = lattice_point_at(L, (int)(blockIdx.x >> 2), (int)(blockIdx.x & 3), threadIdx.x & 63, ix, iy, iz);
    lattice_clamp(L, ix, iy, iz, cx, cy, cz);
    const f3 p = lattice_world(L.res, cx, cy, cz + L.z0);
    const Nearest nr = nearest_shared<NW>(m, p, live, lds + (threadIdx.x >> 6) * kStackDepth, smem, packet_center_lane(L), dbg);
    if (live && threadIdx.x < 64) store_near(near, ((int64_t)cz * L.res + cy) * L.res + cx, nr, sdf_clip);
}

__global__ __launch_bounds__(kBlock) void k_nearest_ties(MeshDev m, const float *__restrict__ pts, int64_t N, const int32_t *__restrict__ perm,
                                                         int32_t *__restrict__ face, int32_t *__restrict__ face2, uint8_t *__restrict__ ulps)
{
    __shared__ int lds[(kBlock / 64) * kStackDepth];
    int64_t i = (int64_t)blockIdx.x * kBlock + threadIdx.x;
    const bool live = i < N;
    if (!live) i = N - 1;
    if (perm) i = perm[i];
    const f3 p = clamp_raw(mk3(pts[3 * i], pts[3 * i + 1], pts[3 * i + 2]));
    unsigned long long k2 = 0;
    const Nearest nr = nearest_packet<false, true>(m, p, live, lds + (threadIdx.x >> 6) * kStackDepth, nullptr, nullptr, INFINITY, &k2);
    if (!live) return;
    const uint32_t b1 = (uint32_t)__float_as_int(nr.d2), b2 = (uint32_t)(k2 >> 32);
    const int f2 = (int)(k2 & 0xffffffffu);
    const bool has2 = f2 != 0x7fffffff && b2 >= b1;
    face[i] = nr.face;
    face2[i] = has2 ? f2 : -1;
    ulps[i] = (uint8_t)(has2 ? min(b2 - b1, 255u) : 255u);
}

__global__ __launch_bounds__(kBlock) void k_traversal_stats(MeshDev m, LatticeMap L, unsigned long long *out , int seeded)
{
    __shared__ int lds[(kBlock / 64) * kStackDepth];
    L = lattice_trim(L, m);
    if ((int)blockIdx.x >= L.tx * L.ty * L.tz) return;
    int ix, iy, iz, cx, cy, cz;
    const bool live = lattice_point(L, ix, iy, iz);
    lattice_clamp(L, ix, iy, iz, cx, cy, cz);
    const f3 p = lattice_world(L.res, cx, cy, cz + L.z0);
    int nn = 0, nt = 0;
    Nearest nr = nearest_packet<true>(m, p, live, lds + (threadIdx.x >> 6) * kStackDepth, &nn, &nt);
    if (seeded) {
        nn = 0; nt = 0;
        float thr0 = prune_threshold(nr.d2);
        if (seeded == 2) {
            const float dc = sqrtf(__int_as_float(__builtin_amdgcn_readlane(__float_as_int(nr.d2), 21)));
            const float h = 2.0f / (float)(L.res - 1);
            const float rad = 2.6f * h;
            thr0 = prune_threshold((dc + rad) * (dc + rad));
        }
        if (seeded == 3) {
            const float h = 2.0f / (float)(L.res - 1);
            int na = 0, nb = 0;
            const Nearest pv = nearest_packet<true>(m, mk3(p.x - 4.0f * h, p.y, p.z), live, lds + (threadIdx.x >> 6) * kStackDepth, &na, &nb);
            const float dn = sqrtf(pv.d2) + 4.0001f * h;
            thr0 = prune_threshold(dn * dn);
        }
        nr = nearest_packet<true>(m, p, live, lds + (threadIdx.x >> 6) * kStackDepth, &nn, &nt, thr0);
    }
    if ((threadIdx.x & 63) == 0) {
        atomicAdd(&out[0], 1ull); atomicAdd(&out[1], (unsigned long long)nn); atomicAdd(&out[2], (unsigned long long)nt);
    }
    if (live && nr.slot < 0) atomicAdd(&out[3], 1ull);
    if ((threadIdx.x & 63) == 0) atomicMax(&out[4], (unsigned long long)(nn + nt));
}

__global__ __launch_bounds__(kBlock) void k_row_crossings(MeshDev m, LatticeMap L, int32_t *row_count, int32_t *row_slots, LatticeFast *lf)
{
    if (lf && blockIdx.x == 0 && threadIdx.x == 0) lattice_fast_write(lf, L, m);
    if (lf) lattice_fast_coords(lf, L.res, (int64_t)blockIdx.x * kBlock + threadIdx.x);
    const int64_t row = (int64_t)blockIdx.x * kBlock + threadIdx.x;
    if (row >= (int64_t)L.nz * L.res) return;
    const int iy = (int)(row % L.res), iz = (int)(row / L.res);
    const f3 p = lattice_world(L.res, 0, iy, iz + L.z0);
    int n = 0;
    const MeshDyn &d = *m.dyn;
    if (d.gy == 0) { row_count[row] = -1; return; }
    if (p.y >= d.bin_y0 && p.y <= d.bin_y1 && p.z >= d.bin_z0 && p.z <= d.bin_z1) {
        const int cy = bin_cell(p.y, d.bin_y0, d.bin_inv_y, d.gy);
        const int cz = bin_cell(p.z, d.bin_z0, d.bin_inv_z, d.gz);
        const int cell = cz * d.gy + cy;
        const int beg = m.bin_start[cell], end = m.bin_start[cell + 1];
        for (int k = beg; k < end; ++k) {
            const int slot = m.bin_slots[k];
            f3 a, b, c; int ia, ib, ic;
            load_tri_full(m.tris + slot, a, b, c, ia, ib, ic);
            if (ray_covers(p, a, b, c, ia, ib, ic)) {
                if (n < kRowCap) row_slots[row * kRowCap + n] = slot;
                ++n;
            }
        }
    }
    row_count[row] = (n <= kRowCap) ? n : -1;
}


__device__ __forceinline__ uint32_t row_code(const float *X, int64_t i)
{
    return (uint32_t)__float_as_int(X[i * kXRow + kCodeSlot]);
}

__global__ __launch_bounds__(kScanBlock) void k_outlier_count(const uint8_t *__restrict__ code8, int64_t N, int32_t *block_counts)
{
    __shared__ int wsum[kScanBlock / 64];
    const int64_t i = (int64_t)blockIdx.x * kScanBlock + threadIdx.x;
    const bool o = (i < N) && (code8[i] & kCodeOutlier);
    const unsigned long long b = __ballot(o);
    if ((threadIdx.x & 63) == 0) wsum[threadIdx.x >> 6] = __popcll(b);
    __syncthreads();
    if (threadIdx.x == 0) {
        int s = 0;
        for (int w = 0; w < kScanBlock / 64; ++w) s += wsum[w];
        block_counts[blockIdx.x] = s;
    }
}

__global__ __launch_bounds__(kBlock) void k_row_crossings_wide(MeshDev m, LatticeMap L, int32_t *row_count, int32_t *row_slots, LatticeFast *lf)
{
    if (lf && blockIdx.x == 0 && threadIdx.x == 0) lattice_fast_write(lf, L, m);
    if (lf) lattice_fast_coords(lf, L.res, (int64_t)blockIdx.x * kBlock + threadIdx.x);
    const int lane = threadIdx.x & 63, g = lane >> 4, s = lane & 15;
    const int64_t row = ((int64_t)blockIdx.x * kBlock + threadIdx.x) >> 4;
    const bool have = row < (int64_t)L.nz * L.res;
    const MeshDyn &d = *m.dyn;
    if (d.gy == 0) { if (have && s == 0) row_count[row] = -1; return; }
    const int iy = have ? (int)(row % L.res) : 0, iz = have ? (int)(row / L.res) : 0;
    const f3 p = lattice_world(L.res, 0, iy, iz + L.z0);
    int beg = 0, end = 0;
    if (have && p.y >= d.bin_y0 && p.y <= d.bin_y1 && p.z >= d.bin_z0 && p.z <= d.bin_z1) {
        const int cy = bin_cell(p.y, d.bin_y0, d.bin_inv_y, d.gy);
        const int cz = bin_cell(p.z, d.bin_z0, d.bin_inv_z, d.gz);
        const int cell = cz * d.gy + cy;
        beg = m.bin_start[cell]; end = m.bin_start[cell + 1];
    }
    int n = 0;
    for (int k = beg + s; __any(k - s < end); k += 16) {
        bool hit = false;
        int slot = 0;
        if (k < end) {
            slot = m.bin_slots[k];
            f3 a, b, c; int ia, ib, ic;
            load_tri_full(m.tris + slot, a, b, c, ia, ib, ic);
            hit = ray_covers(p, a, b, c, ia, ib, ic);
        }
        const unsigned grp = (unsigned)(__ballot(hit) >> (16 * g)) & 0xffffu;
        const int at = n + __popc(grp & ((1u << s) - 1u));
        if (hit && at < kRowCap) row_slots[row * kRowCap + at] = slot;
        n += __popc(grp);
    }
    if (have && s == 0) row_count[row] = (n <= kRowCap) ? n : -1;
}

__device__ __forceinline__ int64_t block_exclusive_scan_1024(int64_t v, int64_t *wtot , int64_t *block_total)
{
    const int lane = threadIdx.x & 63, w = threadIdx.x >> 6;
    int64_t incl = v;
#pragma unroll
    for (int d = 1; d < 64; d <<= 1) {
        const int64_t up = __shfl_up(incl, d);
        if (lane >= d) incl += up;
    }
    if (lane == 63) wtot[w] = incl;
    __syncthreads();
    int64_t base = 0, all = 0;
#pragma unroll
    for (int k = 0; k < 16; ++k) { const int64_t t = wtot[k]; if (k < w) base += t; all += t; }
    *block_total = all;
    return base + incl - v;
}

__global__ __launch_bounds__(1024) void k_scan_local(const int32_t *__restrict__ counts, int64_t n, int32_t *__restrict__ local, int64_t *__restrict__ part,
                                                     const int *__restrict__ n_points_dev)
{
    __shared__ int64_t wtot[16];
    if (n_points_dev) n = ((int64_t)*n_points_dev + kScanBlock - 1) / kScanBlock;
    const int64_t i = (int64_t)blockIdx.x * 1024 + threadIdx.x;
    const int64_t v = (i < n) ? counts[i] : 0;
    int64_t total;
    const int64_t ex = block_exclusive_scan_1024(v, wtot, &total);
    if (i < n) local[i] = (int32_t)ex;
    if (threadIdx.x == 0) part[blockIdx.x] = total;
}

__global__ __launch_bounds__(1024) void k_scan_apply(const int32_t *__restrict__ local, const int64_t *__restrict__ part, int64_t nchunks, int64_t n,
                                                     int64_t *__restrict__ offsets, int64_t *__restrict__ total, const int *__restrict__ n_points_dev)
{
    __shared__ int64_t wtot[16];
    if (n_points_dev) n = ((int64_t)*n_points_dev + kScanBlock - 1) / kScanBlock;
    int64_t before = 0, all = 0;
    for (int64_t k = threadIdx.x; k < nchunks; k += 1024) { const int64_t t = part[k]; all += t; if (k < blockIdx.x) before += t; }
    int64_t sum_all, sum_before;
    (void)block_exclusive_scan_1024(all, wtot, &sum_all);
    __syncthreads();
    (void)block_exclusive_scan_1024(before, wtot, &sum_before);
    const int64_t i = (int64_t)blockIdx.x * 1024 + threadIdx.x;
    if (i < n) offsets[i] = sum_before + local[i];
    if (blockIdx.x == 0 && threadIdx.x == 0) *total = sum_all;
}

__device__ __forceinline__ int64_t outlier_rank(bool o, const int64_t *block_offsets, int *wsum)
{
    const unsigned long long b = __ballot(o);
    const int lane = threadIdx.x & 63, w = threadIdx.x >> 6;
    if (lane == 0) wsum[w] = __popcll(b);
    __syncthreads();
    int before = 0;
    for (int k = 0; k < w; ++k) before += wsum[k];
    before += __popcll(b & ((1ull << lane) - 1ull));
    return block_offsets[blockIdx.x] + before;
}

__global__ __launch_bounds__(kScanBlock) void k_outlier_compact(const uint8_t *__restrict__ code8, int64_t N,
                                                                const int64_t *block_offsets, int8_t *signs, const int *__restrict__ n_dev)
{
    __shared__ int wsum[kScanBlock / 64];
    if (n_dev) { N = *n_dev; if ((int64_t)blockIdx.x * kScanBlock >= N) return; }
    const int64_t i = (int64_t)blockIdx.x * kScanBlock + threadIdx.x;
    const uint32_t code = (i < N) ? code8[i] : 0u;
    const bool o = code & kCodeOutlier;
// ... 274 lines not shown
    return ICON_OK;
}

extern "C" int icon_work_profile_detail(icon_work_t *w, double out[4])
{
    ICON_ARG(w != nullptr && out != nullptr, "icon_work_profile_detail: null argument");
    if (!w->prof || !w->ev_valid) return fail(ICON_ERR_STATE, "icon_work_profile_detail: no profiled call on this workspace");
    ICON_HIP(hipEventSynchronize(w->ev[3]));
    out[0] = out[1] = out[2] = out[3] = 0.0;
    if (w->ev_search) {
        float ms = 0.0f;
        ICON_HIP(hipEventElapsedTime(&ms, w->ev[4], w->ev[5]));
        out[0] = ms;
    }
    unsigned long long c[4] = {0, 0, 0, 0};
    ICON_HIP(hipMemcpy(c, w->d_clock, sizeof(c), hipMemcpyDeviceToHost));
    int dev = 0, khz = 0;
    ICON_HIP(hipGetDevice(&dev));
    ICON_HIP(hipDeviceGetAttribute(&khz, hipDeviceAttributeWallClockRate, dev));
    if (c[2] > c[0] && c[3] > c[1] && khz > 0) {
        out[1] = (double)(c[2] - c[0]);
        out[2] = (double)(c[3] - c[1]) / (double)khz;
        out[3] = out[1] / out[2] * 1e-3;
    }
    return ICON_OK;
}

extern "C" int icon_work_profile_workgroups(icon_work_t *w, double *rec, int cap, int *n)
{
    ICON_ARG(w != nullptr && rec != nullptr && n != nullptr && cap >= 0, "icon_work_profile_workgroups: bad argument");
    if (!w->prof || !w->ev_valid) return fail(ICON_ERR_STATE, "icon_work_profile_workgroups: no profiled call on this workspace");
    ICON_HIP(hipEventSynchronize(w->ev[3]));
    const int g = std::min(w->clock_grid, kMaxProfGrid);
    *n = g;
    if (g <= 0) return ICON_OK;
    std::vector<unsigned long long> c((size_t)kWgRec * g);
    ICON_HIP(hipMemcpy(c.data(), w->d_clock + 4, c.size() * sizeof(unsigned long long), hipMemcpyDeviceToHost));
    int dev = 0, khz = 0;
    ICON_HIP(hipGetDevice(&dev));
    ICON_HIP(hipDeviceGetAttribute(&khz, hipDeviceAttributeWallClockRate, dev));
    ICON_ARG(khz > 0, "icon_work_profile_workgroups: the device reports no wall clock rate");
    unsigned long long t0 = ~0ull;
    for (int b = 0; b < g; ++b) t0 = std::min(t0, c[(size_t)kWgRec * b + 1]);
    for (int b = 0; b < g && b < cap; ++b) {
        const unsigned long long *r = &c[(size_t)kWgRec * b];
        rec[5 * b + 0] = (double)(r[4] >> 32);
        rec[5 * b + 1] = (double)(r[1] - t0) / (double)khz;
        rec[5 * b + 2] = (double)(r[3] - r[1]) / (double)khz;
        rec[5 * b + 3] = (double)(r[2] - r[0]);
        rec[5 * b + 4] = (double)r[5];
    }
    return ICON_OK;
}

extern "C" int icon_work_set_steal(icon_work_t *w, int permille, int group)
{
    ICON_ARG(w != nullptr && permille >= 0 && permille <= 1000 && group >= 1 && group <= 127, "icon_work_set_steal: bad argument");
    w->steal_permille = permille; w->steal_grp = group;
    return ICON_OK;
}

namespace icon {
__global__ __launch_bounds__(256) void k_any_above(const float *__restrict__ occ, int res, int sx, int sy, int sz, int nx, int ny, int nz, float level, int *flag)
{
    const int64_t i = (int64_t)blockIdx.x * 256 + threadIdx.x;
    bool pos = false;
    if (i < (int64_t)nx * ny * nz) {
        const int x = (int)(i % nx), y = (int)((i / nx) % ny), z = (int)(i / ((int64_t)nx * ny));
        pos = occ[((int64_t)z * sz * res + (int64_t)y * sy) * res + (int64_t)x * sx] > level;
    }
    if (__any(pos) && (threadIdx.x & 63) == 0) *flag = 1;
}
}

extern "C" int icon_volume_any_above(const float *d_occ, int res, int sx, int sy, int sz, float level, icon_work_t *w, void *stream, int *h_any)
{
    ICON_ARG(d_occ && w && h_any && res >= 1 && sx >= 1 && sy >= 1 && sz >= 1, "icon_volume_any_above: bad argument");
    if (!w->h_any) {
        ICON_HIP(hipHostMalloc((void **)&w->h_any, sizeof(int), hipHostMallocMapped | hipHostMallocPortable));
    }
    void *dev = nullptr;
    ICON_HIP(hipHostGetDevicePointer(&dev, w->h_any, 0));
    *(volatile int *)w->h_any = 0;
    const int nx = (res - 1) / sx + 1, ny = (res - 1) / sy + 1, nz = (res - 1) / sz + 1;
    const int64_t n = (int64_t)nx * ny * nz;
    hipStream_t st = (hipStream_t)stream;
    hipLaunchKernelGGL(icon::k_any_above, dim3((unsigned)((n + 255) / 256)), dim3(256), 0, st, d_occ, res, sx, sy, sz, nx, ny, nz, level, (int *)dev);
    ICON_HIP(hipGetLastError());
    ICON_HIP(hipStreamSynchronize(st));
    *h_any = *(volatile int *)w->h_any;
    return ICON_OK;
}

extern "C" int icon_work_set_reserve_cus(icon_work_t *w, int n)
{
    ICON_ARG(w != nullptr && n >= 0, "icon_work_set_reserve_cus: bad argument");
    w->reserve_cus = n;
    return ICON_OK;
}

extern "C" int icon_work_profile(icon_work_t *w, int enable)
{
    ICON_ARG(w != nullptr, "icon_work_profile: work is null");
    if (enable && !w->ev[0])
        for (int k = 0; k < 6; ++k) ICON_HIP(hipEventCreate(&w->ev[k]));
    if (enable && !w->d_clock) {
        const size_t bytes = (size_t)(4 + kWgRec * kMaxProfGrid) * sizeof(unsigned long long);
        ICON_HIP(hipMalloc((void **)&w->d_clock, bytes));
        ICON_HIP(hipMemset(w->d_clock, 0, bytes));
    }
    w->clock_grid = 0;
    w->ev_search = false;
    w->prof = enable != 0;
    w->ev_valid = false;
    return ICON_OK;
}

extern "C" int icon_work_stage_ms(icon_work_t *w, float out_ms[3])
{
    ICON_ARG(w && out_ms, "icon_work_stage_ms: null argument");
    if (!w->prof || !w->ev_valid) return fail(ICON_ERR_STATE, "icon_work_stage_ms: no profiled call on this workspace");
    ICON_HIP(hipEventSynchronize(w->ev[3]));
    for (int k = 0; k < 3; ++k) ICON_HIP(hipEventElapsedTime(&out_ms[k], w->ev[k], w->ev[k + 1]));
    return ICON_OK;
}

namespace icon {
__global__ __launch_bounds__(kScanBlock) void k_outlier_patch_self(float *__restrict__ X, const uint8_t *__restrict__ code8, int64_t N, int cmap_slot,
                                                                   const int64_t *block_offsets, const int8_t *signs,
                                                                   const int64_t *k_total_dev)
{
    __shared__ int wsum[kScanBlock / 64];
    const int64_t K = *k_total_dev;
    const int64_t i = (int64_t)blockIdx.x * kScanBlock + threadIdx.x;
    const uint32_t code = (i < N) ? code8[i] : 0u;
    const bool o = code & kCodeOutlier;
    const int64_t j = outlier_rank(o, block_offsets, wsum);
    if (o) {
        float *row = X + i * kXRow + cmap_slot;
#pragma unroll
        for (int k = 0; k < 3; ++k) {
            int64_t mm = 3 * j + k;
            if (mm >= K) mm -= K;
            if (mm >= K) mm -= K;
            row[k] = (float)signs[mm];
        }
    }
}
}

namespace icon {
int g_share_ring = 0, g_share_lose = 0, g_share_spin_log2 = 0;
int g_lattice_fast = -1;
int g_share_waves = -2;
int share_waves_override()
{
    if (g_share_waves == -2) g_share_waves = getenv("ICON_AMD_SHARE") ? atoi(getenv("ICON_AMD_SHARE")) : -1;
    return g_share_waves;
}

int work_share_dbg(icon_work *w, ShareDbg *out)
{
    if (!w->h_err) {
        ICON_HIP(hipHostMalloc((void **)&w->h_err, 8 * sizeof(int), hipHostMallocMapped | hipHostMallocPortable));
        memset(w->h_err, 0, 8 * sizeof(int));
    }
    void *dev = nullptr;
    ICON_HIP(hipHostGetDevicePointer(&dev, w->h_err, 0));
    out->err = (int *)dev;
    out->ring = g_share_ring; out->lose = g_share_lose; out->spin_log2 = g_share_spin_log2;
    return ICON_OK;
}

int work_check_err(icon_work *w)
{
    if (!w || !w->h_err) return ICON_OK;
    volatile int *e = w->h_err;
    const int code = e[0];
    if (code == 0 || code == kShareErrClaimed) return ICON_OK;
    char buf[320];
    static const char *what[] = {"", "a wave waited in vain for the node of its queue ticket (lost or abandoned push)",
                                 "a wave waited in vain for its ring slot to be cleared (ring a full turn behind)",
                                 "an idle wave outlasted its bound while the workgroup was still active"};
    snprintf(buf, sizeof(buf), "shared-walk search: %s [code %d, workgroup %d, wave %d, ticket %d, head %d, tail %d, avail %d, active %d]; the results of "
             "that launch are not to be trusted", what[code >= 1 && code <= 3 ? code : 0], code, e[1], e[7], e[2], e[3], e[4], e[5], e[6]);
    for (int k = 0; k < 8; ++k) e[k] = 0;
    return fail(ICON_ERR_STATE, buf);
}


void mark(icon_work *w, int k, hipStream_t st)
{
    if (w->prof) { (void)hipEventRecord(w->ev[k], st); if (k == 3) w->ev_valid = true; }
}

int ensure_work(icon_work *w, int64_t n_points, bool need_x)
{
    { const int rc = work_check_err(w); if (rc) return rc; }
    if (n_points > w->cap_points) {
        (void)hipFree(w->d_near16); (void)hipFree(w->d_near_d2); w->d_near16 = nullptr; w->d_near_d2 = nullptr; w->cap_points = 0;
        ICON_HIP(hipMalloc((void **)&w->d_near16, (size_t)n_points * sizeof(uint16_t)));
        ICON_HIP(hipMalloc((void **)&w->d_near_d2, (size_t)n_points * sizeof(float)));
        (void)hipFree(w->d_code8); w->d_code8 = nullptr;
        ICON_HIP(hipMalloc((void **)&w->d_code8, (size_t)n_points));
        w->cap_points = n_points;
    }
    if (need_x && n_points > w->cap_x) {
        (void)hipFree(w->d_x); w->d_x = nullptr; w->cap_x = 0;
        ICON_HIP(hipMalloc((void **)&w->d_x, (size_t)n_points * kXRow * sizeof(float)));
        w->cap_x = n_points;
    }
    const int64_t nblk = (n_points + kScanBlock - 1) / kScanBlock;
    if (nblk > w->cap_blocks) {
        (void)hipFree(w->d_block_counts); (void)hipFree(w->d_block_offsets); (void)hipFree(w->d_scan_local); (void)hipFree(w->d_scan_part);
        w->d_block_counts = nullptr; w->d_block_offsets = nullptr; w->d_scan_local = nullptr; w->d_scan_part = nullptr; w->cap_blocks = 0;
        (void)hipFree(w->d_grp_mask); w->d_grp_mask = nullptr;
        ICON_HIP(hipMalloc((void **)&w->d_grp_mask, (size_t)nblk * 4 * sizeof(uint64_t)));
        ICON_HIP(hipMalloc((void **)&w->d_block_counts, (size_t)nblk * sizeof(int32_t)));
        ICON_HIP(hipMalloc((void **)&w->d_block_offsets, (size_t)nblk * sizeof(int64_t)));
        ICON_HIP(hipMalloc((void **)&w->d_scan_local, (size_t)nblk * sizeof(int32_t)));
        ICON_HIP(hipMalloc((void **)&w->d_scan_part, (size_t)((nblk + 1023) / 1024) * sizeof(int64_t)));
        w->cap_blocks = nblk;
    }
    if (n_points > w->cap_signs) {
        (void)hipFree(w->d_signs); w->d_signs = nullptr; w->cap_signs = 0;
        ICON_HIP(hipMalloc((void **)&w->d_signs, (size_t)n_points));
        w->cap_signs = n_points;
    }
    if (!w->d_total) ICON_HIP(hipMalloc((void **)&w->d_total, sizeof(int64_t)));
    if (!w->d_flag) ICON_HIP(hipMalloc((void **)&w->d_flag, sizeof(int)));
    if (!w->d_steal) {
        ICON_HIP(hipMalloc((void **)&w->d_steal, 9 * sizeof(unsigned int)));
        ICON_HIP(hipMemset(w->d_steal, 0, 9 * sizeof(unsigned int)));
    }
    if (!w->d_seg) ICON_HIP(hipMalloc((void **)&w->d_seg, (kMaxWorld + 1) * sizeof(int64_t)));
    return ICON_OK;
}

}

namespace {

int check_prior(const icon_mesh_t *mesh, const icon_feat_t *feat, int prior, int *c0)
{
    ICON_ARG(feat != nullptr, "feature handle is null");
    const FeatDev &f = feat->dev;
    if (prior == ICON_PRIOR_ICON) {
        ICON_ARG(mesh != nullptr, "icon prior needs a mesh handle");
        *c0 = f.csel + 1 + ((f.smpl_mask & kSmplCmap) ? 3 : 0) + ((f.smpl_mask & kSmplNorm) ? 3 : 0);
    } else if (prior == ICON_PRIOR_PAMIR) {
        ICON_ARG(f.n_select == 1 && f.vol != nullptr, "pamir prior needs n_select = 1 and a volume");
        *c0 = f.csel + f.Cv;
    } else if (prior == ICON_PRIOR_PIFU) {
        ICON_ARG(f.n_select == 1, "pifu prior needs n_select = 1");
        *c0 = f.csel + 1;
    } else {
        return fail(ICON_ERR_ARG, "unknown prior_type");
    }
    if (*c0 > kCodeSlot) return fail(ICON_ERR_UNSUPPORTED, "more than 15 MLP input channels");
    return ICON_OK;
}

template <bool LATTICE>
int launch_nearest(const icon_mesh_t *mesh, const Calib &cal, const LatticeMap &L, const float *d_points, int64_t N, float sdf_clip,
                   icon_work *work, hipStream_t st)
{
    LatticeFast *lf = nullptr;
    if (LATTICE) {
        const int64_t rows = (int64_t)L.nz * L.res;
        if (rows > work->cap_rows) {
            (void)hipFree(work->d_row_count); (void)hipFree(work->d_row_slots);
            work->d_row_count = nullptr; work->d_row_slots = nullptr; work->cap_rows = 0;
            ICON_HIP(hipMalloc((void **)&work->d_row_count, (size_t)rows * sizeof(int32_t)));
            ICON_HIP(hipMalloc((void **)&work->d_row_slots, (size_t)rows * kRowCap * sizeof(int32_t)));
            work->cap_rows = rows;
        }
        if (g_lattice_fast < 0) g_lattice_fast = getenv("ICON_AMD_LATTICE_FAST") ? (atoi(getenv("ICON_AMD_LATTICE_FAST")) != 0) : 1;
        if (g_lattice_fast && (L.pk == 0 || L.pk == 4) && L.remap == 0 && L.res <= kLatticeFastMaxRes) {
            if (!work->d_lfast) ICON_HIP(hipMalloc((void **)&work->d_lfast, kLatticeFastBytes));
            lf = work->d_lfast;
        }
        if (rows <= 20000)
            hipLaunchKernelGGL(k_row_crossings_wide, dim3((unsigned)((rows * 16 + kBlock - 1) / kBlock)), dim3(kBlock), 0, st, mesh->dev, L,
                               work->d_row_count, work->d_row_slots, lf);
        else
            hipLaunchKernelGGL(k_row_crossings, dim3((unsigned)((rows + kBlock - 1) / kBlock)), dim3(kBlock), 0, st, mesh->dev, L,
                               work->d_row_count, work->d_row_slots, lf);
    }
    int64_t nb;
    if (LATTICE) nb = (int64_t)L.tx * L.ty * L.tz; else nb = (N + kBlock - 1) / kBlock;
    ICON_ARG(nb >= 0 && nb < (1ll << 31), "too many workgroups for one launch");
    if (mesh->F > kNearLoSlots && work->cap_points_hi < work->cap_points) {
        (void)hipFree(work->d_near_hi); work->d_near_hi = nullptr; work->cap_points_hi = 0;
        ICON_HIP(hipMalloc((void **)&work->d_near_hi, (size_t)work->cap_points));
        work->cap_points_hi = work->cap_points;
    }
    const NearRef near = work_near(work, mesh);
    const int32_t *perm = nullptr;
    static const int mode = getenv("ICON_AMD_POINT_SEARCH") ? atoi(getenv("ICON_AMD_POINT_SEARCH")) : 0;
    const bool alt = work->tie_rule != 0;
    if (!LATTICE && !alt && mode != 3 && (N < kPacketMinPoints || mode == 2)) {
        const int cap = coop_cap(mesh->depth_bound);
        hipLaunchKernelGGL(k_nearest_coop<false>, dim3((unsigned)((N + kCoopWaves - 1) / kCoopWaves)), dim3(kCoopWaves * 64),
                           kCoopWaves * coop_wave_bytes(cap), st, mesh->dev, cal, d_points, N, near, cap, sdf_clip, BatchDev{});
    } else if (nb > 0) {
        if (!LATTICE) {
// ... 287 lines not shown
    const int64_t N = (int64_t)L.nz * res * res;
    ICON_ARG(N < (1ll << 31), "icon_grid_slab_features: more than 2^31 points in one slab");
    if ((rc = ensure_work(work, N, false))) return rc;
    Calib cal{};
    work->slab_ready = false;
    mark(work, 0, st);
    if ((rc = phase1<true>(mesh, feat, prior_type, sdf_clip, cmap_mode, cal, L, nullptr, N, search, d_signs_local, work, st))) return rc;
    work->slab_c0 = c0;
    if (d_count_local) {
        if (work->slab_needs_patch) ICON_HIP(hipMemcpyAsync(d_count_local, work->d_total, sizeof(int64_t), hipMemcpyDeviceToDevice, st));
        else ICON_HIP(hipMemsetAsync(d_count_local, 0, sizeof(int64_t), st));
    }
    if (d_msg) {
        const int64_t cap = msg_bytes - 8;
        ICON_ARG(msg_bytes >= 8 && cap * 4 >= N, "icon_grid_slab_features_msg: message buffer too small (8 + ceil(points / 4) bytes)");
        if (work->slab_needs_patch) {
            const int64_t nb = (std::max<int64_t>(cap, 1) + 255) / 256;
            hipLaunchKernelGGL(k_pack_signs, dim3((unsigned)nb), dim3(256), 0, st, d_signs_local ? d_signs_local : work->d_signs, work->d_total,
                               (uint8_t *)d_msg, cap);
            ICON_HIP(hipGetLastError());
        } else {
            ICON_HIP(hipMemsetAsync(d_msg, 0, sizeof(int64_t), st));
        }
    }
    mark(work, 1, st);
    work->slab_res = res; work->slab_z0 = z0; work->slab_z1 = z1; work->slab_ready = true;
    return ICON_OK;
}

extern "C" int icon_grid_slab_features(const icon_mesh_t *mesh, const icon_feat_t *feat,
                                       int prior_type, float sdf_clip, int cmap_mode,
                                       int res, int z0, int z1, int8_t *d_signs_local, int64_t *d_count_local,
                                       int search, icon_work_t *work, void *stream)
{
    return slab_features_impl(mesh, feat, prior_type, sdf_clip, cmap_mode, res, z0, z1, d_signs_local, d_count_local, nullptr, 0, search, work, stream);
}

extern "C" int icon_grid_slab_features_msg(const icon_mesh_t *mesh, const icon_feat_t *feat,
                                           int prior_type, float sdf_clip, int cmap_mode,
                                           int res, int z0, int z1, void *d_msg, int64_t msg_bytes,
                                           int search, icon_work_t *work, void *stream)
{
    ICON_ARG(d_msg != nullptr, "icon_grid_slab_features_msg: message buffer is null");
    return slab_features_impl(mesh, feat, prior_type, sdf_clip, cmap_mode, res, z0, z1, nullptr, nullptr, d_msg, msg_bytes, search, work, stream);
}

extern "C" int icon_grid_slab_finish(const icon_mlp_t *mlp, int res, int z0, int z1,
                                     const int8_t *d_signs_global, int64_t k_total, int64_t rank_offset,
                                     float *d_occ, int precision, icon_work_t *work, void *stream)
{
    ICON_ARG(mlp && work && d_occ, "icon_grid_slab_finish: null argument");
    if (!work->slab_ready || work->slab_res != res || work->slab_z0 != z0 || work->slab_z1 != z1)
        return fail(ICON_ERR_STATE, "icon_grid_slab_finish: no matching icon_grid_slab_features call on this workspace");
    ICON_ARG(work->slab_c0 == mlp->c0, "icon_grid_slab_finish: MLP input width does not match the feature layout");
    FusedSigns fs{};
    if (work->slab_needs_patch) {
        ICON_ARG(k_total == 0 || d_signs_global != nullptr, "icon_grid_slab_finish: sign list is null");
        fs.mode = kSignGlobal; fs.list = d_signs_global; fs.k_host = k_total; fs.rank_offset = rank_offset;
    }
    work->slab_ready = false;
    return phase2(mlp, fs, d_occ, precision, work, (hipStream_t)stream, z0, z1);
}

extern "C" int icon_grid_slab_finish_gathered(const icon_mlp_t *mlp, int res, int z0, int z1, int za, int zb,
                                              const void *d_gathered, int64_t stride, int world, int rank,
                                              float *d_occ, int precision, icon_work_t *work, void *stream)
{
    ICON_ARG(mlp && work && d_occ, "icon_grid_slab_finish_gathered: null argument");
    if (!work->slab_ready || work->slab_res != res || work->slab_z0 != z0 || work->slab_z1 != z1)
        return fail(ICON_ERR_STATE, "icon_grid_slab_finish_gathered: no matching icon_grid_slab_features call on this workspace");
    ICON_ARG(za >= z0 && zb > za && zb <= z1, "icon_grid_slab_finish_gathered: planes [za, zb) must lie inside the slab");
    ICON_ARG(work->slab_c0 == mlp->c0, "icon_grid_slab_finish_gathered: MLP input width does not match the feature layout");
    FusedSigns fs{};
    if (work->slab_needs_patch) {
        if (d_gathered) {
            ICON_ARG(world >= 1 && world <= kMaxWorld && rank >= 0 && rank < world, "icon_grid_slab_finish_gathered: bad world / rank");
            ICON_ARG(stride >= 8 && (stride & 7) == 0, "icon_grid_slab_finish_gathered: stride must be a multiple of 8 (int64 header)");
            fs.mode = kSignSeg; fs.gathered = (const int8_t *)d_gathered; fs.stride = stride; fs.world = world; fs.rank = rank;
        } else {
            fs = self_signs(work);
        }
    }
    return phase2(mlp, fs, d_occ, precision, work, (hipStream_t)stream, za, zb);
}

static int copy_rows_out(icon_work *work, float *d_rows, hipStream_t st)
{
    int rc = materialise_rows(work, self_signs(work), st);
    if (rc) return rc;
    ICON_HIP(hipMemcpyAsync(d_rows, work->d_x, (size_t)work->q_N * kXRow * sizeof(float), hipMemcpyDeviceToDevice, st));
    return ICON_OK;
}

extern "C" int icon_query_rows(const icon_mesh_t *mesh, const icon_feat_t *feat, int prior_type, float sdf_clip, int cmap_mode,
                               const float *h_calib, const float *d_calib, const float *d_points, int64_t N, float *d_rows,
                               int search, icon_work_t *work, void *stream)
{
    ICON_ARG(work && d_points && d_rows, "icon_query_rows: null argument");
    ICON_ARG(N >= 0, "icon_query_rows: negative N");
    int c0 = 0;
    int rc = check_prior(mesh, feat, prior_type, &c0);
    if (rc) return rc;
    if (N == 0) return ICON_OK;
    hipStream_t st = (hipStream_t)stream;
    if ((rc = ensure_work(work, N, false))) return rc;
    Calib cal;
    static const float ident[12] = {1, 0, 0, 0, 0, 1, 0, 0, 0, 0, 1, 0};
    memcpy(cal.m, h_calib ? h_calib : ident, sizeof(cal.m));
    cal.d = d_calib;
    LatticeMap L{};
    work->slab_ready = false;
    if ((rc = phase1<false>(mesh, feat, prior_type, sdf_clip, cmap_mode, cal, L, d_points, N, search, nullptr, work, st))) return rc;
    return copy_rows_out(work, d_rows, st);
}

extern "C" int icon_grid_rows(const icon_mesh_t *mesh, const icon_feat_t *feat, int prior_type, float sdf_clip, int cmap_mode,
                              int res, int z0, int z1, float *d_rows, int search, icon_work_t *work, void *stream)
{
    ICON_ARG(work && d_rows, "icon_grid_rows: null argument");
    int c0 = 0;
    int rc = check_prior(mesh, feat, prior_type, &c0);
    if (rc) return rc;
    LatticeMap L;
    if ((rc = lattice_map(res, z0, z1, nullptr, sdf_clip, false, &L))) return rc;
    hipStream_t st = (hipStream_t)stream;
    const int64_t N = (int64_t)L.nz * res * res;
    ICON_ARG(N < (1ll << 31), "icon_grid_rows: more than 2^31 points in one slab");
    if ((rc = ensure_work(work, N, false))) return rc;
    Calib cal{};
    work->slab_ready = false;
    if ((rc = phase1<true>(mesh, feat, prior_type, sdf_clip, cmap_mode, cal, L, nullptr, N, search, nullptr, work, st))) return rc;
    return copy_rows_out(work, d_rows, st);
}

extern "C" int icon_debug_traversal_stats(const icon_mesh_t *mesh, int res, int z0, int z1, uint64_t out[4])
{
    ICON_ARG(mesh && out, "icon_debug_traversal_stats: null argument");
    LatticeMap L;
    int rc = lattice_map(res, z0, z1, mesh, 0.05f, true, &L);
    if (rc) return rc;
    unsigned long long *d = nullptr;
    ICON_HIP(hipMalloc((void **)&d, 8 * sizeof(unsigned long long)));
    ICON_HIP(hipMemset(d, 0, 8 * sizeof(unsigned long long)));
    hipLaunchKernelGGL(k_traversal_stats, dim3((unsigned)(L.tx * L.ty * L.tz)), dim3(kBlock), 0, 0, mesh->dev, L, d,
                       getenv("ICON_AMD_STATS_SEEDED") ? atoi(getenv("ICON_AMD_STATS_SEEDED")) : 0);
    unsigned long long h[8];
    hipError_t e = hipMemcpy(h, d, sizeof(h), hipMemcpyDeviceToHost);
    (void)hipFree(d);
    if (e != hipSuccess) return fail(ICON_ERR_HIP, std::string("traversal stats: ") + hipGetErrorString(e));
    out[0] = h[0]; out[1] = h[1]; out[2] = h[2]; out[3] = h[4];
    return ICON_OK;
}

extern "C" int icon_grid_eval_slab(const icon_mesh_t *mesh, const icon_feat_t *feat, const icon_mlp_t *mlp,
                                   int prior_type, float sdf_clip, int cmap_mode,
                                   int res, int z0, int z1, float *d_occ,
                                   int search, int precision, icon_work_t *work, void *stream)
{
    ICON_ARG(mlp && work && d_occ, "icon_grid_eval_slab: null argument");
    int rc = icon_grid_slab_features(mesh, feat, prior_type, sdf_clip, cmap_mode, res, z0, z1, nullptr, nullptr, search, work, stream);
    if (rc) return rc;
    ICON_ARG(work->slab_c0 == mlp->c0, "icon_grid_eval_slab: MLP input width does not match the feature layout");
    work->slab_ready = false;
    return phase2(mlp, self_signs(work), d_occ, precision, work, (hipStream_t)stream, z0, z1);
}

extern "C" int icon_work_status(icon_work_t *work)
{
    ICON_ARG(work != nullptr, "icon_work_status: work is null");
    return work_check_err(work);
}

extern "C" int icon_debug_set_option(const char *key, int value)
{
    ICON_ARG(key != nullptr, "icon_debug_set_option: key is null");
    const std::string k(key);
    if (k == "lattice_fast") g_lattice_fast = value ? 1 : 0;
    else if (k == "share_waves") { ICON_ARG(value == -1 || value == 1 || value == 4 || value == 8 || value == 16, "share_waves: -1 (by launch size), 1, 4, 8 or 16"); g_share_waves = value; }
    else if (k == "share_ring") { ICON_ARG(value == 0 || (value >= 2 && value <= 64 && (value & (value - 1)) == 0), "share_ring: 0 or a power of two in 2..64"); g_share_ring = value; }
    else if (k == "share_lose_push") { ICON_ARG(value >= 0, "share_lose_push: a ticket >= 1, or 0"); g_share_lose = value; }
    else if (k == "share_spin_log2") { ICON_ARG(value >= 0 && value < 30, "share_spin_log2: 0..29"); g_share_spin_log2 = value; }
    else if (k == "qc_lanes") { ICON_ARG(value == 0 || value == 64, "qc_lanes: 0 (default) or 64"); g_qc_lanes = value; }
    else if (k == "rn_lanes") { ICON_ARG(value == 0 || value == 1 || value == 8, "rn_lanes: 0 (default), 1 or 8"); g_rn_lanes = value; }
    else return fail(ICON_ERR_ARG, "icon_debug_set_option: unknown key " + k);
    return ICON_OK;
}

extern "C" int icon_debug_set_shell_skip(int on)
{
    g_shell_skip = on ? 1 : 0;
    return ICON_OK;
}

extern "C" int icon_work_set_tie_rule(icon_work_t *work, int rule, int ulps)
{
    ICON_ARG(work != nullptr, "icon_work_set_tie_rule: work is null");
    ICON_ARG(rule == 0 || rule == 1, "icon_work_set_tie_rule: rule must be 0 (definition) or 1 (highest index within ulps)");
    ICON_ARG(ulps >= 0 && ulps <= 255, "icon_work_set_tie_rule: ulps must be 0..255");
    work->tie_rule = rule; work->tie_ulps = ulps;
    return ICON_OK;
}

extern "C" int icon_sdf_query_ties(const icon_mesh_t *mesh, const float *d_points, int64_t N,
                                   int32_t *d_face, int32_t *d_face2, uint8_t *d_ulps, void *stream)
{
    ICON_ARG(mesh && d_points && d_face && d_face2 && d_ulps, "icon_sdf_query_ties: null argument");
    ICON_ARG(N >= 0, "icon_sdf_query_ties: negative N");
    if (N == 0) return ICON_OK;
    const int64_t nb = (N + kBlock - 1) / kBlock;
    ICON_ARG(nb < (1ll << 31), "icon_sdf_query_ties: N too large for one launch");
    hipStream_t st = (hipStream_t)stream;
    icon_work tmp;
    static const float ident[12] = {1, 0, 0, 0, 0, 1, 0, 0, 0, 0, 1, 0};
    const int32_t *perm = nullptr;
    int rc = morton_order(&tmp, d_points, ident, nullptr, N, st, &perm);
    if (!rc) {
        hipLaunchKernelGGL(k_nearest_ties, dim3((unsigned)nb), dim3(kBlock), 0, st, mesh->dev, d_points, N, perm, d_face, d_face2, d_ulps);
        if (hipGetLastError() != hipSuccess || hipStreamSynchronize(st) != hipSuccess) rc = fail(ICON_ERR_HIP, "icon_sdf_query_ties: launch failed");
    }
    (void)hipFree(tmp.d_sort_keys); (void)hipFree(tmp.d_sort_idx); (void)hipFree(tmp.d_sort_tmp);
    return rc;
}
```

icon_amd/engine.py:

```python
from __future__ import annotations

import contextlib
import ctypes as C
from typing import Optional, Sequence

import numpy as np
import torch
import torch.nn as nn

from . import _lib
from ._lib import IconAmdError, check, ptr


def _stream() -> C.c_void_p:
    return C.c_void_p(torch.cuda.current_stream().cuda_stream)


def _on(t: torch.Tensor):
    return torch.cuda.device(t.device) if t.is_cuda else contextlib.nullcontext()


def _key(*tensors) -> tuple:
    return tuple((t.data_ptr(), t._version, t.shape, t.device) for t in tensors)


def _dev_f32(t: torch.Tensor, what: str) -> torch.Tensor:
    if not t.is_cuda:
        raise IconAmdError(f"{what} is on {t.device}; icon_amd has no CPU path - move it to the HIP device")
    return t.detach().to(torch.float32).contiguous()


class _Handle:
    _destroy = None

    def __init__(self):
        self.h = C.c_void_p(0)

    def close(self):
        if self.h and self.h.value:
            getattr(_lib.lib(), self._destroy)(self.h)
            self.h = C.c_void_p(0)

    def __del__(self):
        try:
            self.close()
        except Exception:
            pass


class MeshHandle(_Handle):
    _destroy = "icon_mesh_destroy"

    def __init__(self, smpl_verts, smpl_faces, smpl_cmap, smpl_vis, validate: bool = True):
        super().__init__()
        _lib.require_device()
        for t, what in ((smpl_verts, "smpl_verts"), (smpl_faces, "smpl_faces"), (smpl_cmap, "smpl_cmap"), (smpl_vis, "smpl_vis")):
            if t.dim() == 3 and t.shape[0] > 1:
                raise IconAmdError(f"{what} has batch size {t.shape[0]}: a MeshHandle holds one subject (MeshBatchHandle for [B,...])")
        v = _dev_f32(smpl_verts, "smpl_verts").reshape(-1, 3)
        f = smpl_faces.detach()
        if not f.is_cuda:
            raise IconAmdError("smpl_faces must be on the HIP device")
        f = f.to(torch.int64).reshape(-1, 3).contiguous()
        cm = _dev_f32(smpl_cmap, "smpl_cmap").reshape(-1, 3)
        vs = _dev_f32(smpl_vis, "smpl_vis").reshape(-1)
        if cm.shape[0] != v.shape[0] or vs.shape[0] != v.shape[0]:
            raise IconAmdError("smpl_cmap / smpl_vis do not match smpl_verts")
        self.V, self.F = int(v.shape[0]), int(f.shape[0])
        self.device = v.device
        self.checked = False
        nbytes = C.c_int64(0)
        check(_lib.lib().icon_mesh_arena_bytes(C.c_int64(self.V), C.c_int64(self.F), C.byref(nbytes)), "icon_mesh_arena_bytes")
        with _on(v):
            self.arena = torch.empty(int(nbytes.value), dtype=torch.uint8, device=v.device)
            check(_lib.lib().icon_mesh_create_arena(ptr(v), C.c_int64(self.V), ptr(f), C.c_int64(self.F), ptr(cm), ptr(vs),
                                                    ptr(self.arena), nbytes, _stream(), C.byref(self.h)), "icon_mesh_create")
        if validate:
            self.status(wait=True)

    def status(self, wait: bool = False) -> Optional[int]:
        if self.checked:
            return 0
        bits = C.c_int(0)
        check(_lib.lib().icon_mesh_status(self.h, C.c_int(int(wait)), C.byref(bits)), "icon_mesh_create")
        if bits.value < 0:
            return None
        self.checked = True
        return int(bits.value)

    def vertex_normals(self) -> torch.Tensor:
        out = torch.empty((self.V, 3), dtype=torch.float32, device=self.device)
        check(_lib.lib().icon_mesh_vertex_normals(self.h, ptr(out), _stream()), "icon_mesh_vertex_normals")
        return out

    def stats(self) -> dict:
        arr = (C.c_int64 * 6)()
        check(_lib.lib().icon_mesh_stats(self.h, arr), "icon_mesh_stats")
        return dict(nodes=arr[0], depth=arr[1], bin_entries=arr[2], max_bin=arr[3], leaves=arr[4], slots=arr[5])

    def traversal_stats(self, res: int, z0: int = 0, z1: Optional[int] = None) -> dict:
        arr = (C.c_uint64 * 4)()
        check(_lib.lib().icon_debug_traversal_stats(self.h, C.c_int(res), C.c_int(z0), C.c_int(res if z1 is None else z1), arr),
              "icon_debug_traversal_stats")
        return dict(waves=arr[0], nodes=arr[1], tris=arr[2], nodes_per_wave=arr[1] / max(arr[0], 1),
                    tris_per_wave=arr[2] / max(arr[0], 1), longest_walk=arr[3])

    def sdf_query(self, points: torch.Tensor, search: str = "bvh"):
        p = _dev_f32(points, "points").reshape(-1, 3)
        n = p.shape[0]
        dev = p.device
        out = dict(sdf=torch.empty(n, device=dev), norm=torch.empty((n, 3), device=dev),
                   cmap=torch.empty((n, 3), device=dev), vis=torch.empty(n, device=dev),
                   face=torch.empty(n, dtype=torch.int64, device=dev),
                   inside=torch.empty(n, dtype=torch.uint8, device=dev))
        check(_lib.lib().icon_sdf_query(self.h, ptr(p), C.c_int64(n), ptr(out["sdf"]), ptr(out["norm"]),
                                        ptr(out["cmap"]), ptr(out["vis"]), ptr(out["face"]), ptr(out["inside"]),
                                        C.c_int(_lib.SEARCH[search]), _stream()), "icon_sdf_query")
        out["inside"] = out["inside"].bool()
        return out


    def sdf_query_ties(self, points: torch.Tensor) -> dict:
        p = _dev_f32(points, "points").reshape(-1, 3)
        n, dev = p.shape[0], p.device
        out = dict(face=torch.empty(n, dtype=torch.int32, device=dev), face2=torch.empty(n, dtype=torch.int32, device=dev),
                   ulps=torch.empty(n, dtype=torch.uint8, device=dev))
        check(_lib.lib().icon_sdf_query_ties(self.h, ptr(p), C.c_int64(n), ptr(out["face"]), ptr(out["face2"]), ptr(out["ulps"]),
                                             _stream()), "icon_sdf_query_ties")
        return out


class MeshBatchHandle(_Handle):
    _destroy = "icon_mesh_batch_destroy"

    def __init__(self, smpl_verts, smpl_faces, smpl_cmap, smpl_vis):
        super().__init__()
        ts = (smpl_verts, smpl_faces, smpl_cmap, smpl_vis)
        if any(t.dim() != 3 for t in ts):
            raise IconAmdError("smpl_feat_dict tensors must be [B,V,3] / [B,F,3] / [B,V,3] / [B,V,1] for a batched query")
        self.B = int(smpl_verts.shape[0])
        if any(int(t.shape[0]) != self.B for t in ts):
            raise IconAmdError(f"smpl_feat_dict batch sizes disagree: {[int(t.shape[0]) for t in ts]}")
        self.subjects = [MeshHandle(smpl_verts[b], smpl_faces[b], smpl_cmap[b], smpl_vis[b], validate=False) for b in range(self.B)]
        arr = (C.c_void_p * self.B)(*[m.h.value for m in self.subjects])
        with _on(smpl_verts):
            check(_lib.lib().icon_mesh_batch_create(arr, C.c_int(self.B), _stream(), C.byref(self.h)), "icon_mesh_batch_create")
        self.checked = False

    @property
    def V(self):
        return self.subjects[0].V

    def status(self, wait: bool = False) -> Optional[int]:
        if self.checked:
            return 0
        pending = False
        for m in self.subjects:
            if m.status(wait) is None:
                pending = True
        bits = C.c_int(0)
        try:
            check(_lib.lib().icon_mesh_batch_status(self.h, C.c_int(int(wait)), C.byref(bits)), "icon_mesh_batch")
        except IconAmdError:
            self.reported = True
            raise
        if pending or bits.value < 0:
            return None
        self.checked = True
        return int(bits.value)

    def close(self):
        super().close()
        for m in getattr(self, "subjects", ()):
            m.close()


class FeatBatchHandle(_Handle):
    _destroy = "icon_feat_destroy"

    def __init__(self, planes: torch.Tensor, n_select: int, smpl_feats: Sequence[str] = ("sdf", "norm", "vis", "cmap"),
                 vol: Optional[torch.Tensor] = None):
        super().__init__()
        _lib.require_device()
        p = _dev_f32(planes, "features")
        if p.dim() != 4:
            raise IconAmdError("features must be [B,C,H,W]")
        B, Cc, H, W = (int(x) for x in p.shape)
        self.B, self.C, self.H, self.W, self.n_select, self.Cv = B, Cc, H, W, n_select, 0
        with _on(p):
            check(_lib.lib().icon_feat_create_batch(ptr(p), C.c_int(B), C.c_int(Cc), C.c_int(H), C.c_int(W), C.c_int(n_select), _stream(),
                                                    C.byref(self.h)), "icon_feat_create_batch")
            if vol is not None:
                v = _dev_f32(vol, "vol_feat")
                if v.dim() != 5:
                    raise IconAmdError(f"vol_feat {tuple(v.shape)} must be [B,Cv,D,H,W]")
                Bv, self.Cv, Dv, Hv, Wv = (int(x) for x in v.shape)
                check(_lib.lib().icon_feat_batch_set_volume(self.h, ptr(v), C.c_int(Bv), C.c_int(self.Cv), C.c_int(Dv), C.c_int(Hv), C.c_int(Wv),
                                                            _stream()), "icon_feat_batch_set_volume")
        if set(smpl_feats) | {"vis"} != {"sdf", "norm", "vis", "cmap"}:
            check(_lib.lib().icon_feat_set_smpl_feats(self.h, C.c_int(int("cmap" in smpl_feats)), C.c_int(int("norm" in smpl_feats))),
                  "icon_feat_set_smpl_feats")


class FeatHandle(FeatBatchHandle):

    def __init__(self, planes: torch.Tensor, n_select: int, vol: Optional[torch.Tensor] = None,
                 smpl_feats: Sequence[str] = ("sdf", "norm", "vis", "cmap")):
        if planes.dim() == 4 and planes.shape[0] != 1:
            raise IconAmdError("batch size must be 1 (lib/common/seg3d_lossless.py:73)")
        if vol is not None:
            vol = vol[:1] if vol.dim() == 5 else vol[None]
        super().__init__(planes if planes.dim() == 4 else planes[None], n_select, smpl_feats, vol)


def _np32(t) -> np.ndarray:
    if isinstance(t, torch.Tensor):
        t = t.detach().to("cpu", torch.float32).numpy()
    return np.ascontiguousarray(t, dtype=np.float32)


def effective_filters(state_dict: dict) -> dict:
    if not any(k.endswith("weight_g") for k in state_dict):
        return state_dict
    out = {k: v for k, v in state_dict.items() if not (k.endswith("weight_g") or k.endswith("weight_v"))}
    for k, g in state_dict.items():
        if k.endswith("weight_g"):
            v = state_dict[k[:-1] + "v"]
            g, v = (torch.as_tensor(t).detach().float().cpu() for t in (g, v))
            out[k[:-2]] = torch._weight_norm(v, g, 0)
    return out


class MlpHandle(_Handle):
    _destroy = "icon_mlp_destroy"

    def __init__(self, state_dict, res_layers: Sequence[int] = (2, 3, 4), bn_eps: float = 1e-5, last_op: Optional[str] = None):
        super().__init__()
        if last_op not in (None, "sigmoid"):
            raise IconAmdError(f"unsupported last_op {last_op!r} (None or 'sigmoid')")
        _lib.require_device()
        state_dict = effective_filters(state_dict)
        n = 0
        while f"filters.{n}.weight" in state_dict:
            n += 1
        if n == 0:
            raise IconAmdError("state_dict has no filters.0.weight")
        W = [_np32(state_dict[f"filters.{l}.weight"]) for l in range(n)]
        W = [w.reshape(w.shape[0], -1) for w in W]
        b = [_np32(state_dict[f"filters.{l}.bias"]) for l in range(n)]
        has_bn = f"norms.0.running_mean" in state_dict
        cin = (C.c_int * n)(*[w.shape[1] for w in W])
        cout = (C.c_int * n)(*[w.shape[0] for w in W])
        is_res = (C.c_int * n)(*[1 if l in tuple(res_layers) else 0 for l in range(n)])
        self.c0 = int(W[0].shape[1])

        def parr(arrs):
            return (C.c_void_p * len(arrs))(*[a.ctypes.data for a in arrs])

# ... 785 lines not shown
```

include/icon_amd.h:

```cpp
#ifndef ICON_AMD_H
#define ICON_AMD_H

#include <stdint.h>

#ifdef __cplusplus
extern "C" {
#endif

#define ICON_AMD_VERSION 100

enum {
    ICON_OK = 0,
    ICON_ERR_ARG = 1,
    ICON_ERR_HIP = 2,
    ICON_ERR_UNSUPPORTED = 3,
    ICON_ERR_STATE = 4
};

enum { ICON_PRIOR_ICON = 0, ICON_PRIOR_PAMIR = 1, ICON_PRIOR_PIFU = 2 };

enum { ICON_CMAP_REFERENCE = 0, ICON_CMAP_LOCAL = 1 };

enum { ICON_PRECISION_F32 = 0, ICON_PRECISION_F16X3 = 1 };

enum { ICON_SEARCH_BVH = 0, ICON_SEARCH_BRUTE = 1 };


typedef struct icon_mesh icon_mesh_t;
typedef struct icon_feat icon_feat_t;
typedef struct icon_mlp  icon_mlp_t;
typedef struct icon_work icon_work_t;

const char *icon_last_error(void);
int icon_version(void);
int icon_device_count(void);

int icon_mesh_create(const float *d_verts, int64_t V, const int64_t *d_faces, int64_t F,
                     const float *d_cmap, const float *d_vis, void *stream, icon_mesh_t **out);
int icon_mesh_arena_bytes(int64_t V, int64_t F, int64_t *bytes);
int icon_mesh_create_arena(const float *d_verts, int64_t V, const int64_t *d_faces, int64_t F,
                           const float *d_cmap, const float *d_vis, void *d_arena, int64_t arena_bytes,
                           void *stream, icon_mesh_t **out);
int icon_mesh_destroy(icon_mesh_t *mesh);
int icon_mesh_status(const icon_mesh_t *mesh, int wait, int *bits);
int icon_mesh_vertex_normals(const icon_mesh_t *mesh, float *d_out, void *stream);
int icon_mesh_stats(const icon_mesh_t *mesh, int64_t out[6]);

int icon_sdf_query(const icon_mesh_t *mesh, const float *d_points, int64_t N,
                   float *d_sdf, float *d_norm, float *d_cmap, float *d_vis,
                   int64_t *d_face, uint8_t *d_inside, int search, void *stream);

int icon_feat_create(const float *d_planes, int C, int H, int W, int n_select,
                     const float *d_vol, int Cv, int Dv, int Hv, int Wv,
                     void *stream, icon_feat_t **out);
int icon_feat_destroy(icon_feat_t *feat);
int icon_feat_set_smpl_feats(icon_feat_t *feat, int has_cmap, int has_norm);

int icon_mlp_create(int n_layers, const int *cin, const int *cout, const int *is_res,
                    const float *const *h_W, const float *const *h_b,
                    const float *const *h_bn_gamma, const float *const *h_bn_beta,
                    const float *const *h_bn_mean, const float *const *h_bn_var,
                    float bn_eps, void *stream, icon_mlp_t **out);
int icon_mlp_destroy(icon_mlp_t *mlp);
enum { ICON_LASTOP_NONE = 0, ICON_LASTOP_SIGMOID = 1 };
int icon_mlp_set_last_op(icon_mlp_t *mlp, int last_op);
int icon_mlp_forward(const icon_mlp_t *mlp, const float *d_x, int64_t N, float *d_out,
                     int precision, void *stream);

int icon_work_create(icon_work_t **out);
int icon_work_destroy(icon_work_t *work);
int icon_work_profile(icon_work_t *work, int enable);
int icon_work_set_reserve_cus(icon_work_t *work, int n);
int icon_work_stage_ms(icon_work_t *work, float out_ms[3]);
int icon_work_profile_detail(icon_work_t *work, double out[4]);
int icon_work_profile_workgroups(icon_work_t *work, double *rec, int cap, int *n);
int icon_work_set_steal(icon_work_t *work, int permille, int group);

int icon_query_points(const icon_mesh_t *mesh, const icon_feat_t *feat, const icon_mlp_t *mlp,
                      int prior_type, float sdf_clip, int cmap_mode, const float *h_calib,
                      const float *d_points, int64_t N, float *d_occ,
                      int search, int precision, icon_work_t *work, void *stream);

int icon_query_points_dcalib(const icon_mesh_t *mesh, const icon_feat_t *feat, const icon_mlp_t *mlp,
                             int prior_type, float sdf_clip, int cmap_mode, const float *d_calib,
                             const float *d_points, int64_t N, float *d_occ,
                             int search, int precision, icon_work_t *work, void *stream);

typedef struct icon_mesh_batch icon_mesh_batch_t;
int icon_mesh_batch_create(const icon_mesh_t *const *meshes, int B, void *stream, icon_mesh_batch_t **out);
int icon_mesh_batch_destroy(icon_mesh_batch_t *mb);
#define ICON_MESH_BATCH_FACES_DIFFER 0x10
int icon_mesh_batch_status(const icon_mesh_batch_t *mb, int wait, int *bits);

int icon_feat_create_batch(const float *d_planes, int B, int C, int H, int W, int n_select, void *stream, icon_feat_t **out);

int icon_feat_batch_set_volume(icon_feat_t *feat, const float *d_vol, int B, int Cv, int Dv, int Hv, int Wv, void *stream);

int icon_query_points_batch(const icon_mesh_batch_t *mb, const icon_feat_t *feat, const icon_mlp_t *mlp,
                            int prior_type, float sdf_clip, int cmap_mode, const float *d_calibs,
                            const float *d_points, int64_t N, int B, float *d_occ,
                            int search, int precision, icon_work_t *work, void *stream);

int icon_grid_eval_slab(const icon_mesh_t *mesh, const icon_feat_t *feat, const icon_mlp_t *mlp,
                        int prior_type, float sdf_clip, int cmap_mode,
                        int res, int z0, int z1, float *d_occ,
                        int search, int precision, icon_work_t *work, void *stream);

int icon_grid_slab_features(const icon_mesh_t *mesh, const icon_feat_t *feat,
                            int prior_type, float sdf_clip, int cmap_mode,
                            int res, int z0, int z1, int8_t *d_signs_local, int64_t *d_count_local,
                            int search, icon_work_t *work, void *stream);
int icon_grid_slab_finish(const icon_mlp_t *mlp, int res, int z0, int z1,
                          const int8_t *d_signs_global, int64_t k_total, int64_t rank_offset,
                          float *d_occ, int precision, icon_work_t *work, void *stream);
int icon_grid_slab_features_msg(const icon_mesh_t *mesh, const icon_feat_t *feat,
                                int prior_type, float sdf_clip, int cmap_mode,
                                int res, int z0, int z1, void *d_msg, int64_t msg_bytes,
                                int search, icon_work_t *work, void *stream);
int icon_grid_slab_finish_gathered(const icon_mlp_t *mlp, int res, int z0, int z1, int za, int zb,
                                   const void *d_gathered, int64_t stride, int world, int rank,
                                   float *d_occ, int precision, icon_work_t *work, void *stream);

int icon_adaptive_eval(const icon_mesh_t *mesh, const icon_feat_t *feat, const icon_mlp_t *mlp, int prior_type, float sdf_clip,
                       int cmap_mode, const int *resolutions, int n_levels, float balance, float *d_out, int64_t *h_counts,
                       int search, int precision, icon_work_t *work, void *stream);
int icon_adaptive_counts(icon_work_t *work, int n_levels, int64_t *h_counts, void *stream);
int icon_adaptive_reruns(icon_work_t *work, int *n);

int icon_query_rows(const icon_mesh_t *mesh, const icon_feat_t *feat, int prior_type, float sdf_clip, int cmap_mode,
                    const float *h_calib, const float *d_calib, const float *d_points, int64_t N, float *d_rows,
                    int search, icon_work_t *work, void *stream);
int icon_grid_rows(const icon_mesh_t *mesh, const icon_feat_t *feat, int prior_type, float sdf_clip, int cmap_mode,
                   int res, int z0, int z1, float *d_rows, int search, icon_work_t *work, void *stream);

int icon_debug_set_unfused(int on);
int icon_debug_set_mesh_build(int host);
int icon_debug_mesh_layout(int64_t V, int64_t F, int64_t out[12]);
int icon_debug_host_mesh_build(const float *h_verts, int64_t V, const int64_t *h_faces, int64_t F,
                               const float *h_cmap, const float *h_vis, void *h_arena, int64_t arena_bytes);
int icon_debug_set_shell_skip(int on);
int icon_debug_set_option(const char *key, int value);
int icon_work_status(icon_work_t *work);

int icon_sdf_query_ties(const icon_mesh_t *mesh, const float *d_points, int64_t N,
                        int32_t *d_face, int32_t *d_face2, uint8_t *d_ulps, void *stream);
int icon_work_set_tie_rule(icon_work_t *work, int rule, int ulps);

int icon_debug_traversal_stats(const icon_mesh_t *mesh, int res, int z0, int z1, uint64_t out[4]);

int icon_volume_any_above(const float *d_occ, int res, int sx, int sy, int sz, float level, icon_work_t *work, void *stream, int *h_any);

int icon_export_mesh(const float *h_occ, int res, float level,
                     float *h_verts, int64_t *n_verts, int64_t *h_faces, int64_t *n_faces);

int icon_mc_count(const float *d_occ, int res, float level, icon_work_t *work, void *stream,
                  int64_t *n_verts, int64_t *n_faces);
int icon_mc_emit(float *d_verts, int64_t *d_faces, icon_work_t *work, void *stream);
int icon_mc_count_range(const float *d_occ, int res, float level, int zc0, int zc1, int halo, icon_work_t *work, void *stream,
                        int64_t *n_verts, int64_t *n_faces);
int icon_mc_emit_keyed(float *d_verts, int64_t *d_faces, int64_t *d_keys, icon_work_t *work, void *stream);

int icon_semantic_voxelize(const float *d_verts, int64_t V, int64_t V_surf, const float *d_code,
                           const int64_t *d_tets, int64_t T, int res, float sigma, float *d_out, void *stream);

int icon_semantic_voxelize_batch(const float *d_verts, int B, int64_t V, int64_t V_surf, const float *d_code,
                                 const int64_t *d_tets, int64_t T, int res, float sigma, uint8_t *d_occ, float *d_out, void *stream);

int icon_mesh_components(const int64_t *d_faces, int64_t F, int64_t V, int32_t *d_labels, void *stream);

int icon_clean_mesh(const float *d_verts, int64_t V, const int64_t *d_faces, int64_t F, float *d_out_verts, int32_t *d_out_faces,
                    int64_t *h_counts, icon_work_t *work, void *stream);

int icon_visibility(const float *d_xy, const float *d_z, int64_t V, const int64_t *d_faces, int64_t F,
                    int image_size, float *d_vis, void *stream);

int icon_query_color_bytes(int64_t V, int64_t F, int image_size, int64_t *bytes);
int icon_query_color(const float *d_verts, int64_t V, const void *d_faces, int64_t F, int faces_int64,
                     const float *d_image, int H, int W, int image_size, float *d_colors, float *d_vis,
                     void *d_scratch, int64_t scratch_bytes, void *stream);

int icon_render_bytes(int64_t V, int64_t F, int size, int n_views, int64_t *bytes);
int icon_render_normal(const float *d_verts, int64_t V, const void *d_faces, int64_t F, int faces_int64,
                       const int *cam_ids, int n_views, int size, float *d_images, float *d_depth, int32_t *d_pix_to_face,
                       void *d_scratch, int64_t scratch_bytes, void *stream);

int icon_silhouette_bytes(int64_t V, int64_t F, int size, int n_views, int64_t *bytes);
int icon_silhouette_forward(const float *d_verts, int64_t V, const void *d_faces, int64_t F, int faces_int64,
                            const int *cam_ids, int n_views, int size, float *d_alpha,
                            void *d_scratch, int64_t scratch_bytes, void *stream);
int icon_silhouette_backward(const float *d_verts, int64_t V, const void *d_faces, int64_t F, int faces_int64,
                             const int *cam_ids, int n_views, int size, const float *d_alpha, const float *d_grad_alpha,
                             float *d_grad_verts, void *d_scratch, int64_t scratch_bytes, void *stream);

int icon_render_normal_backward_bytes(int64_t V, int64_t F, int size, int n_views, int64_t *bytes);
int icon_render_normal_backward(const float *d_verts, int64_t V, const void *d_faces, int64_t F, int faces_int64,
                                const int *cam_ids, int n_views, int size, const int32_t *d_pix_to_face,
                                const float *d_grad_images, float *d_grad_verts,
                                void *d_scratch, int64_t scratch_bytes, void *stream);

#ifdef __cplusplus
}
#endif
#endif
```

Baseline: 998.2 million.

## Cull BVH leaf triangle pairs with oriented bounding boxes per pair

Adds a per-leaf PairBox record, built on both the host and device mesh-build paths, holding an oriented (or axis-aligned fallback) bounding box for each triangle pair. During nearest-triangle packet traversal, each wave computes a lower-bound distance to each pair box and skips exact triangle-pair distance tests when no lane could beat its current threshold. This trades an extra 128-byte load and a few FMAs per leaf for fewer full triangle distance evaluations. It also grows the mesh arena and adds debug stats entry points.

New measurement: 1.023 billion (median of 6 runs). 2.5% higher.

```diff
diff --git a/icon_amd/_lib.py b/icon_amd/_lib.py
--- a/icon_amd/_lib.py
+++ b/icon_amd/_lib.py
@@ -24,7 +24,7 @@
     "icon_query_points", "icon_query_points_dcalib", "icon_query_rows", "icon_grid_rows",
     "icon_volume_any_above", "icon_adaptive_eval", "icon_adaptive_counts", "icon_adaptive_reruns", "icon_grid_eval_slab", "icon_grid_slab_features", "icon_grid_slab_finish", "icon_grid_slab_features_msg",
     "icon_grid_slab_finish_gathered", "icon_debug_set_shell_skip", "icon_debug_set_option", "icon_work_status", "icon_sdf_query_ties", "icon_work_set_tie_rule",
-    "icon_export_mesh", "icon_mc_count", "icon_mc_emit", "icon_mc_count_range", "icon_mc_emit_keyed", "icon_debug_traversal_stats", "icon_debug_set_unfused",
+    "icon_export_mesh", "icon_mc_count", "icon_mc_emit", "icon_mc_count_range", "icon_mc_emit_keyed", "icon_debug_traversal_stats", "icon_debug_pair_stats", "icon_debug_pair_box", "icon_debug_set_unfused",
     "icon_visibility", "icon_mesh_components", "icon_clean_mesh", "icon_semantic_voxelize",
     "icon_mesh_batch_create", "icon_mesh_batch_destroy", "icon_mesh_batch_status", "icon_feat_create_batch", "icon_query_points_batch",
     "icon_feat_batch_set_volume", "icon_semantic_voxelize_batch",
diff --git a/icon_amd/csrc/common.h b/icon_amd/csrc/common.h
--- a/icon_amd/csrc/common.h
+++ b/icon_amd/csrc/common.h
@@ -60,6 +60,11 @@
     float pair[2][24][2];
 };
 static_assert(sizeof(LeafRec) == 384, "LeafRec must be 384 bytes");
+
+struct alignas(32) PairBox {
+    float f[16][2];
+};
+static_assert(sizeof(PairBox) == 128, "PairBox must be 128 bytes");
 
 constexpr int kLeafMax = 4;
 constexpr int kShareWavesMany = 8, kShareWavesFew = 16;
@@ -101,6 +106,7 @@
     const LeafRec *leaves;
     const MeshDyn *dyn;
     int32_t n_tris;
+    int32_t pbox_off;
     const int32_t *bin_start;
     const int32_t *bin_slots;
 };
@@ -292,6 +298,7 @@
 int work_check_err(icon_work *w);
 extern int g_qc_lanes;
 extern int g_rn_lanes;
+int pair_box_enabled();
 int share_waves_override();
 }
 
diff --git a/icon_amd/csrc/geom_device.h b/icon_amd/csrc/geom_device.h
--- a/icon_amd/csrc/geom_device.h
+++ b/icon_amd/csrc/geom_device.h
@@ -203,9 +203,10 @@
 __device__ __forceinline__ Nearest nearest_packet(const MeshDev &m, f3 p, bool live, int *wstack ,
                                                   int *n_nodes = nullptr, int *n_tris = nullptr, float thr0 = INFINITY,
                                                   unsigned long long *runner_up = nullptr, int center_lane = 21,
-                                                  bool have_root = false, int root = 0)
+                                                  bool have_root = false, int root = 0, int *n_offered = nullptr, int *n_tested = nullptr)
 {
     Nearest nr; nr.d2 = INFINITY; nr.slot = 0; nr.face = 0x7fffffff;
+    const PairBox *pbox = m.pbox_off ? reinterpret_cast<const PairBox *>(m.leaves) + m.pbox_off : nullptr;
     unsigned long long key = 0x7f8000007fffffffull;
     unsigned long long key2 = 0x7f8000007fffffffull;
     float thr = live ? thr0 : -INFINITY;
@@ -217,7 +218,20 @@
             const int leaf = code >> 2, cnt = (code & 3) + 1;
             if (STATS) *n_tris += cnt;
             const int npairs = __builtin_amdgcn_readfirstlane((cnt + 1) >> 1);
-            for (int pr = 0; pr < npairs; ++pr) {
+            int need = (1 << npairs) - 1;
+            if (pbox) {
+                const f2 bb = pair_box_bound(reinterpret_cast<cf2 *>(as_const(pbox + leaf)), p.x, p.y, p.z);
+                const int any0 = __builtin_amdgcn_ballot_w64(bb.x <= thr) != 0 ? 1 : 0, any1 = __builtin_amdgcn_ballot_w64(bb.y <= thr) != 0 ? 2 : 0;
+                need &= any0 | any1;
+            }
+            if (STATS && n_offered) { *n_offered += npairs; *n_tested += __builtin_popcount((unsigned)need); }
+            if (need == 0) {
+                if (sp == 0) break;
+                cur = __builtin_amdgcn_readfirstlane(wstack[--sp]);
+                continue;
+            }
+            for (; need; need &= need - 1) {
+                const int pr = __builtin_ctz((unsigned)need);
                 cf2 *q = reinterpret_cast<cf2 *>(as_const(&m.leaves[leaf].pair[pr]));
                 const f2 d2 = tri_dist2_pair(p, q);
                 const f2 fc = q[22];
diff --git a/icon_amd/csrc/mesh_build.cpp b/icon_amd/csrc/mesh_build.cpp
--- a/icon_amd/csrc/mesh_build.cpp
+++ b/icon_amd/csrc/mesh_build.cpp
@@ -220,6 +220,7 @@
     std::vector<float> vn;
     std::vector<BvhNode> nodes;
     std::vector<LeafRec> leafrec;
+    std::vector<PairBox> pbox;
     std::vector<TriRec> tris;
     std::vector<TriAttr> attr;
     std::vector<int32_t> order, face2slot, bin_start, bin_slots;
@@ -300,6 +301,23 @@
             for (int fld = 0; fld < 24; ++fld) leafrec[L].pair[t >> 1][fld][t & 1] = src[fld];
         }
     }
+    std::vector<PairBox> &pbox = out.pbox;
+    pbox.resize(F);
+    memset((void *)pbox.data(), 0, sizeof(PairBox) * F);
+    for (int64_t L = 0; L < F; ++L) {
+        const int cnt = hb.leaf_cnt[L];
+        for (int pr = 0; pr < (cnt ? 2 : 0); ++pr) {
+            const int t0 = std::min(2 * pr, (cnt - 1) & ~1);
+            const int64_t p0 = L + t0, p1 = L + std::min(t0 + 1, cnt - 1);
+            float v[6][3], rec[15];
+            for (int k = 0; k < 3; ++k) {
+                v[0][k] = tris[p0].a[k]; v[1][k] = tris[p0].b[k]; v[2][k] = tris[p0].c[k];
+                v[3][k] = tris[p1].a[k]; v[4][k] = tris[p1].b[k]; v[5][k] = tris[p1].c[k];
+            }
+            pair_box_setup(v, rec);
+            for (int fld = 0; fld < 15; ++fld) pbox[L].f[fld][pr] = rec[fld];
+        }
+    }
 
     const int64_t n_cells = (int64_t)g.gy * g.gz;
     std::vector<int32_t> &bin_start = out.bin_start;
@@ -347,6 +365,7 @@
     if ((rc = put_fn(Ly.dyn, dynv.data(), sizeof(MeshDyn))) || (rc = put_fn(Ly.vnormals, h.vn.data(), h.vn.size() * 4)) ||
         (rc = put_fn(Ly.nodes, h.nodes.data(), h.nodes.size() * sizeof(BvhNode))) ||
         (rc = put_fn(Ly.leaves, h.leafrec.data(), h.leafrec.size() * sizeof(LeafRec))) ||
+        (rc = put_fn(Ly.pbox, h.pbox.data(), h.pbox.size() * sizeof(PairBox))) ||
         (rc = put_fn(Ly.tris, h.tris.data(), h.tris.size() * sizeof(TriRec))) || (rc = put_fn(Ly.attr, h.attr.data(), h.attr.size() * sizeof(TriAttr))) ||
         (rc = put_fn(Ly.slot2face, h.order.data(), h.order.size() * 4)) || (rc = put_fn(Ly.face2slot, h.face2slot.data(), h.face2slot.size() * 4)) ||
         (rc = put_fn(Ly.bin_start, h.bin_start.data(), h.bin_start.size() * 4)) || (rc = put_fn(Ly.bin_slots, h.bin_slots.data(), h.bin_slots.size() * 4)))
@@ -512,6 +531,33 @@
     return emit_arena(h, Ly, [&](size_t off, const void *src, size_t bytes) -> int { if (bytes) memcpy(ar + off, src, bytes); return ICON_OK; });
 }
 
+extern "C" int icon_debug_pair_box(const float *corners, int64_t n_pairs, const float *pts, int64_t n_pts, int shared_pts,
+                                   float *rec, int32_t *kind, float *bound)
+{
+    ICON_ARG(corners && pts && rec && kind && bound && n_pairs >= 1 && n_pts >= 1, "icon_debug_pair_box: bad argument");
+    parallel_for((int)((n_pairs + 1) / 2), [&](int k) {
+        PairBox pb;
+        memset((void *)&pb, 0, sizeof(pb));
+        for (int s = 0; s < 2; ++s) {
+            const int64_t i = std::min<int64_t>(2 * (int64_t)k + s, n_pairs - 1);
+            float r[15];
+            kind[i] = pair_box_setup(reinterpret_cast<const float(*)[3]>(corners + 18 * i), r);
+            for (int f = 0; f < 15; ++f) { pb.f[f][s] = r[f]; rec[15 * i + f] = r[f]; }
+        }
+        const pbf2 *q = reinterpret_cast<const pbf2 *>(&pb);
+        for (int s = 0; s < 2; ++s) {
+            const int64_t i = 2 * (int64_t)k + s;
+            if (i >= n_pairs) break;
+            const float *pp = shared_pts ? pts : pts + 3 * n_pts * i;
+            for (int64_t j = 0; j < n_pts; ++j) {
+                const pbf2 b = pair_box_bound(q, pp[3 * j], pp[3 * j + 1], pp[3 * j + 2]);
+                bound[n_pts * i + j] = s ? b.y : b.x;
+            }
+        }
+    });
+    return ICON_OK;
+}
+
 extern "C" int icon_debug_mesh_layout(int64_t V, int64_t F, int64_t out[12])
 {
     ICON_ARG(out && V >= 3 && F >= 1 && F <= (1 << 23), "icon_debug_mesh_layout: bad argument");
diff --git a/icon_amd/csrc/mesh_device.hip b/icon_amd/csrc/mesh_device.hip
--- a/icon_amd/csrc/mesh_device.hip
+++ b/icon_amd/csrc/mesh_device.hip
@@ -16,7 +16,7 @@
     int32_t V, F, bound;
     MeshDyn *dyn; BuildHdr *hdr;
     int32_t *valence; uint8_t *leaf_cnt; BTask *tasks; uint32_t *hist; int32_t *cell_count, *cell_cursor;
-    float *vnormals; BvhNode *nodes; LeafRec *leaves; TriRec *tris; TriAttr *attr; int32_t *slot2face, *face2slot;
+    float *vnormals; BvhNode *nodes; LeafRec *leaves; PairBox *pbox; TriRec *tris; TriAttr *attr; int32_t *slot2face, *face2slot;
     int32_t *bin_start, *bin_slots;
     float *tbox, *cen; int32_t *order[2]; int32_t *adj; int32_t *chunkcnt; int32_t *subq; struct STask *sublist; uint32_t *bounds_part;
     int32_t nck; int64_t cells_cap, entries_cap;
@@ -628,6 +628,22 @@
     const int tend = (myt == cnt - 1) ? kLeafMax : myt + 1;
     for (int t = myt; t < tend; ++t)
         for (int fld = 0; fld < 24; ++fld) lr.pair[t >> 1][fld][t & 1] = src[fld];
+    if ((myt & 1) == 0) {
+        float pv[6][3], rec[15];
+        for (int q = 0; q < 3; ++q) for (int k = 0; k < 3; ++k) { pv[q][k] = v[q][k]; pv[3 + q][k] = v[q][k]; }
+        if (myt + 1 < cnt) {
+            int id1[3]; float v1[3][3]; int bf1 = 0, bv1 = 0;
+            load_face(c, c.slot2face[p + 1], id1, v1, &bf1, &bv1);
+            for (int q = 0; q < 3; ++q) for (int k = 0; k < 3; ++k) pv[3 + q][k] = v1[q][k];
+        }
+        pair_box_setup(pv, rec);
+        PairBox &pb = c.pbox[leaf];
+        const int pend = (myt + 2 >= cnt) ? 2 : (myt >> 1) + 1;
+        for (int pr = myt >> 1; pr < pend; ++pr) {
+            for (int fld = 0; fld < 15; ++fld) pb.f[fld][pr] = rec[fld];
+            pb.f[15][pr] = 0.0f;
+        }
+    }
     const BinGrid g = grid_of(c);
     int cy0, cy1, cz0, cz1;
     cell_range(g, c.tbox + 6 * (size_t)f, cy0, cy1, cz0, cz1);
@@ -794,6 +810,7 @@
     d.leaves = reinterpret_cast<const LeafRec *>(b + L.leaves);
     d.dyn = m->d_dyn;
     d.n_tris = (int32_t)m->F;
+    d.pbox_off = pair_box_enabled() ? (int32_t)((L.pbox - L.leaves) / sizeof(PairBox)) : 0;
     d.bin_start = reinterpret_cast<const int32_t *>(b + L.bin_start);
     d.bin_slots = reinterpret_cast<const int32_t *>(b + L.bin_slots);
 }
@@ -810,7 +827,7 @@
     c.tasks = reinterpret_cast<BTask *>(b + L.tasks); c.hist = reinterpret_cast<uint32_t *>(b + L.hist);
     c.cell_count = reinterpret_cast<int32_t *>(b + L.cell_count); c.cell_cursor = reinterpret_cast<int32_t *>(b + L.cell_cursor);
     c.vnormals = reinterpret_cast<float *>(b + L.vnormals); c.nodes = reinterpret_cast<BvhNode *>(b + L.nodes);
-    c.leaves = reinterpret_cast<LeafRec *>(b + L.leaves); c.tris = reinterpret_cast<TriRec *>(b + L.tris);
+    c.leaves = reinterpret_cast<LeafRec *>(b + L.leaves); c.pbox = reinterpret_cast<PairBox *>(b + L.pbox); c.tris = reinterpret_cast<TriRec *>(b + L.tris);
     c.attr = reinterpret_cast<TriAttr *>(b + L.attr); c.slot2face = reinterpret_cast<int32_t *>(b + L.slot2face);
     c.face2slot = reinterpret_cast<int32_t *>(b + L.face2slot); c.bin_start = reinterpret_cast<int32_t *>(b + L.bin_start);
     c.bin_slots = reinterpret_cast<int32_t *>(b + L.bin_slots); c.tbox = reinterpret_cast<float *>(b + L.tbox);
diff --git a/icon_amd/csrc/mesh_rules.h b/icon_amd/csrc/mesh_rules.h
--- a/icon_amd/csrc/mesh_rules.h
+++ b/icon_amd/csrc/mesh_rules.h
@@ -68,6 +68,120 @@
     t.face = face; t.pad = 0;
 }
 
+constexpr float kPairBoxScale = 0.9999f;
+constexpr float kPairBoxGram = 4e-6f;
+constexpr float kPairBoxEps = 4e-6f;
+constexpr float kPairBoxFloor = 1e-15f;
+enum { kPairBoxOriented = 0, kPairBoxAabb = 1, kPairBoxNever = 2 };
+
+__host__ __device__ inline bool pb_finite(float v)
+{
+    uint32_t u; __builtin_memcpy(&u, &v, 4);
+    return (u & 0x7f800000u) != 0x7f800000u;
+}
+__host__ __device__ inline void pb_cross(const float *a, const float *b, float *r)
+{
+    r[0] = fmaf(a[1], b[2], -(a[2] * b[1])); r[1] = fmaf(a[2], b[0], -(a[0] * b[2])); r[2] = fmaf(a[0], b[1], -(a[1] * b[0]));
+}
+__host__ __device__ inline int pair_box_setup(const float v[6][3], float out[15])
+{
+    bool fin = true;
+    for (int i = 0; i < 6; ++i) for (int k = 0; k < 3; ++k) fin = fin && pb_finite(v[i][k]);
+    float ax[3][3] = {{1.f, 0.f, 0.f}, {0.f, 1.f, 0.f}, {0.f, 0.f, 1.f}};
+    int kind = kPairBoxAabb;
+    if (fin) {
+        float e[6][3], l2[6];
+        for (int t = 0; t < 2; ++t)
+            for (int k = 0; k < 3; ++k) {
+                e[3 * t][k] = v[3 * t + 1][k] - v[3 * t][k]; e[3 * t + 1][k] = v[3 * t + 2][k] - v[3 * t][k];
+                e[3 * t + 2][k] = v[3 * t + 2][k] - v[3 * t + 1][k];
+            }
+        int best = 0;
+        for (int i = 0; i < 6; ++i) { l2[i] = dot3r(e[i], e[i]); if (l2[i] > l2[best]) best = i; }
+        const float L2 = l2[best];
+        float n0[3], n1[3], n[3];
+        pb_cross(e[0], e[1], n0); pb_cross(e[3], e[4], n1);
+        for (int k = 0; k < 3; ++k) n[k] = n0[k] + n1[k];
+        const float nn = dot3r(n, n);
+        if (nn > 1e-10f * (L2 * L2)) {
+            const float ln = sqrtf(nn);
+            float a0[3], u[3], a1[3], a2[3];
+            for (int k = 0; k < 3; ++k) a0[k] = n[k] / ln;
+            const float en = dot3r(e[best], a0);
+            for (int k = 0; k < 3; ++k) u[k] = fmaf(-en, a0[k], e[best][k]);
+            const float uu = dot3r(u, u);
+            if (uu > 1e-10f * L2) {
+                const float lu = sqrtf(uu);
+                for (int k = 0; k < 3; ++k) a1[k] = u[k] / lu;
+                pb_cross(a0, a1, a2);
+                const float g[6] = {dot3r(a0, a0) - 1.0f, dot3r(a1, a1) - 1.0f, dot3r(a2, a2) - 1.0f, dot3r(a0, a1), dot3r(a0, a2), dot3r(a1, a2)};
+                bool ok = true;
+                for (int i = 0; i < 6; ++i) ok = ok && (fabsf(g[i]) <= kPairBoxGram);
+                if (ok) {
+                    for (int k = 0; k < 3; ++k) { ax[0][k] = a0[k]; ax[1][k] = a1[k]; ax[2][k] = a2[k]; }
+                    kind = kPairBoxOriented;
+                }
+            }
+        }
+    }
+    for (int attempt = 0; attempt < 2 && fin; ++attempt) {
+        float c[3];
+        for (int k = 0; k < 3; ++k) {
+            float lo = v[0][k], hi = v[0][k];
+            for (int i = 1; i < 6; ++i) { lo = fminf(lo, v[i][k]); hi = fmaxf(hi, v[i][k]); }
+            c[k] = canon(0.5f * (lo + hi));
+        }
+        float mid[3];
+        for (int a = 0; a < 3; ++a) {
+            float lo = 0.f, hi = 0.f;
+            for (int i = 0; i < 6; ++i) {
+                const float d[3] = {v[i][0] - c[0], v[i][1] - c[1], v[i][2] - c[2]};
+                const float t = dot3r(ax[a], d);
+                lo = i ? fminf(lo, t) : t; hi = i ? fmaxf(hi, t) : t;
+            }
+            mid[a] = 0.5f * (lo + hi);
+        }
+        for (int k = 0; k < 3; ++k) c[k] = canon(fmaf(mid[2], ax[2][k], fmaf(mid[1], ax[1][k], fmaf(mid[0], ax[0][k], c[k]))));
+        float h[3];
+        for (int a = 0; a < 3; ++a) {
+            for (int k = 0; k < 3; ++k) out[3 + 3 * a + k] = canon(ax[a][k] * kPairBoxScale);
+            float m = 0.f;
+            for (int i = 0; i < 6; ++i) {
+                const float d[3] = {v[i][0] - c[0], v[i][1] - c[1], v[i][2] - c[2]};
+                m = fmaxf(m, fabsf(dot3r(out + 3 + 3 * a, d)));
+            }
+            h[a] = m;
+        }
+        const float pad = fmaf(kPairBoxEps, (h[0] + h[1]) + h[2], kPairBoxFloor);
+        bool ok = true;
+        for (int k = 0; k < 3; ++k) { out[k] = c[k]; out[12 + k] = h[k] + pad; ok = ok && pb_finite(c[k]) && pb_finite(out[12 + k]); }
+        if (ok) return kind;
+        if (kind == kPairBoxAabb) break;
+        kind = kPairBoxAabb;
+        for (int a = 0; a < 3; ++a) for (int k = 0; k < 3; ++k) ax[a][k] = (a == k) ? 1.f : 0.f;
+    }
+    for (int k = 0; k < 3; ++k) { out[k] = 0.f; out[12 + k] = __builtin_inff(); }
+    for (int a = 0; a < 3; ++a) for (int k = 0; k < 3; ++k) out[3 + 3 * a + k] = (a == k) ? kPairBoxScale : 0.f;
+    return kPairBoxNever;
+}
+
+typedef float pbf2 __attribute__((ext_vector_type(2)));
+template <class Ptr>
+__host__ __device__ inline pbf2 pair_box_bound(Ptr q, float px, float py, float pz)
+{
+    pbf2 bx, by, bz; bx.x = px; bx.y = px; by.x = py; by.y = py; bz.x = pz; bz.y = pz;
+    const pbf2 dx = bx - q[0], dy = by - q[1], dz = bz - q[2];
+    const pbf2 t0 = __builtin_elementwise_fma(q[5], dz, __builtin_elementwise_fma(q[4], dy, q[3] * dx));
+    const pbf2 t1 = __builtin_elementwise_fma(q[8], dz, __builtin_elementwise_fma(q[7], dy, q[6] * dx));
+    const pbf2 t2 = __builtin_elementwise_fma(q[11], dz, __builtin_elementwise_fma(q[10], dy, q[9] * dx));
+    const pbf2 h0 = q[12], h1 = q[13], h2 = q[14];
+    pbf2 e0, e1, e2;
+    e0.x = fmaxf(fabsf(t0.x) - h0.x, 0.0f); e0.y = fmaxf(fabsf(t0.y) - h0.y, 0.0f);
+    e1.x = fmaxf(fabsf(t1.x) - h1.x, 0.0f); e1.y = fmaxf(fabsf(t1.y) - h1.y, 0.0f);
+    e2.x = fmaxf(fabsf(t2.x) - h2.x, 0.0f); e2.y = fmaxf(fabsf(t2.y) - h2.y, 0.0f);
+    return __builtin_elementwise_fma(e2, e2, __builtin_elementwise_fma(e1, e1, e0 * e0));
+}
+
 constexpr int kTopLevels = 7;
 constexpr int kSubMax = 256;
 constexpr int kChunk = 256;
@@ -89,7 +203,7 @@
 
 struct MeshLayout {
     size_t dyn, hdr, valence, leaf_cnt, tasks, hist, cell_count, cell_cursor, zero_end;
-    size_t vnormals, nodes, leaves, tris, attr, slot2face, face2slot, bin_start, bin_slots;
+    size_t vnormals, nodes, leaves, pbox, tris, attr, slot2face, face2slot, bin_start, bin_slots;
     size_t tbox, cen, order0, order1, adj, chunkcnt, subq, sublist, bounds_part, total;
     int64_t nck;
 };
@@ -113,6 +227,7 @@
     L.vnormals = take(sizeof(float) * 3 * V);
     L.nodes = take(sizeof(BvhNode) * F);
     L.leaves = take(sizeof(LeafRec) * F);
+    L.pbox = take(sizeof(PairBox) * F);
     L.tris = take(sizeof(TriRec) * F);
     L.attr = take(sizeof(TriAttr) * F);
     L.slot2face = take(sizeof(int32_t) * F);
diff --git a/icon_amd/csrc/query_kernels.hip b/icon_amd/csrc/query_kernels.hip
--- a/icon_amd/csrc/query_kernels.hip
+++ b/icon_amd/csrc/query_kernels.hip
@@ -160,6 +160,23 @@
     if ((threadIdx.x & 63) == 0) atomicMax(&out[4], (unsigned long long)(nn + nt));
 }
 
+__global__ __launch_bounds__(kBlock) void k_pair_stats(MeshDev m, LatticeMap L, unsigned long long *out )
+{
+    __shared__ int lds[(kBlock / 64) * kStackDepth];
+    L = lattice_trim(L, m);
+    if ((int)blockIdx.x >= L.tx * L.ty * L.tz) return;
+    int ix, iy, iz, cx, cy, cz;
+    const bool live = lattice_point(L, ix, iy, iz);
+    lattice_clamp(L, ix, iy, iz, cx, cy, cz);
+    const f3 p = lattice_world(L.res, cx, cy, cz + L.z0);
+    int nn = 0, nt = 0, no = 0, ns = 0;
+    nearest_packet<true>(m, p, live, lds + (threadIdx.x >> 6) * kStackDepth, &nn, &nt, INFINITY, nullptr, packet_center_lane(L), false, 0, &no, &ns);
+    if ((threadIdx.x & 63) == 0) {
+        atomicAdd(&out[0], 1ull); atomicAdd(&out[1], (unsigned long long)nn);
+        atomicAdd(&out[2], (unsigned long long)no); atomicAdd(&out[3], (unsigned long long)ns);
+    }
+}
+
 __global__ __launch_bounds__(kBlock) void k_row_crossings(MeshDev m, LatticeMap L, int32_t *row_count, int32_t *row_slots, LatticeFast *lf)
 {
     if (lf && blockIdx.x == 0 && threadIdx.x == 0) lattice_fast_write(lf, L, m);
@@ -740,6 +757,12 @@
 namespace icon {
 int g_share_ring = 0, g_share_lose = 0, g_share_spin_log2 = 0;
 int g_lattice_fast = -1;
+int g_pair_box = -1;
+int pair_box_enabled()
+{
+    if (g_pair_box < 0) g_pair_box = getenv("ICON_AMD_PAIR_BOX") ? (atoi(getenv("ICON_AMD_PAIR_BOX")) != 0) : 1;
+    return g_pair_box;
+}
 int g_share_waves = -2;
 int share_waves_override()
 {
@@ -1333,6 +1356,24 @@
     return ICON_OK;
 }
 
+extern "C" int icon_debug_pair_stats(const icon_mesh_t *mesh, int res, int z0, int z1, uint64_t out[4])
+{
+    ICON_ARG(mesh && out, "icon_debug_pair_stats: null argument");
+    LatticeMap L;
+    int rc = lattice_map(res, z0, z1, mesh, 0.05f, true, &L);
+    if (rc) return rc;
+    unsigned long long *d = nullptr;
+    ICON_HIP(hipMalloc((void **)&d, 4 * sizeof(unsigned long long)));
+    ICON_HIP(hipMemset(d, 0, 4 * sizeof(unsigned long long)));
+    hipLaunchKernelGGL(k_pair_stats, dim3((unsigned)(L.tx * L.ty * L.tz)), dim3(kBlock), 0, 0, mesh->dev, L, d);
+    unsigned long long h[4];
+    hipError_t e = hipMemcpy(h, d, sizeof(h), hipMemcpyDeviceToHost);
+    (void)hipFree(d);
+    if (e != hipSuccess) return fail(ICON_ERR_HIP, std::string("pair stats: ") + hipGetErrorString(e));
+    for (int k = 0; k < 4; ++k) out[k] = h[k];
+    return ICON_OK;
+}
+
 extern "C" int icon_grid_eval_slab(const icon_mesh_t *mesh, const icon_feat_t *feat, const icon_mlp_t *mlp,
                                    int prior_type, float sdf_clip, int cmap_mode,
                                    int res, int z0, int z1, float *d_occ,
@@ -1358,6 +1399,7 @@
     const std::string k(key);
     if (k == "lattice_fast") g_lattice_fast = value ? 1 : 0;
     else if (k == "share_waves") { ICON_ARG(value == -1 || value == 1 || value == 4 || value == 8 || value == 16, "share_waves: -1 (by launch size), 1, 4, 8 or 16"); g_share_waves = value; }
+    else if (k == "pair_box") g_pair_box = value ? 1 : 0;
     else if (k == "share_ring") { ICON_ARG(value == 0 || (value >= 2 && value <= 64 && (value & (value - 1)) == 0), "share_ring: 0 or a power of two in 2..64"); g_share_ring = value; }
     else if (k == "share_lose_push") { ICON_ARG(value >= 0, "share_lose_push: a ticket >= 1, or 0"); g_share_lose = value; }
     else if (k == "share_spin_log2") { ICON_ARG(value >= 0 && value < 30, "share_spin_log2: 0..29"); g_share_spin_log2 = value; }
diff --git a/icon_amd/engine.py b/icon_amd/engine.py
--- a/icon_amd/engine.py
+++ b/icon_amd/engine.py
@@ -104,6 +104,14 @@
               "icon_debug_traversal_stats")
         return dict(waves=arr[0], nodes=arr[1], tris=arr[2], nodes_per_wave=arr[1] / max(arr[0], 1),
                     tris_per_wave=arr[2] / max(arr[0], 1), longest_walk=arr[3])
+
+    def pair_stats(self, res: int, z0: int = 0, z1: Optional[int] = None) -> dict:
+        arr = (C.c_uint64 * 4)()
+        check(_lib.lib().icon_debug_pair_stats(self.h, C.c_int(res), C.c_int(z0), C.c_int(res if z1 is None else z1), arr),
+              "icon_debug_pair_stats")
+        n = max(arr[0], 1)
+        return dict(packets=arr[0], nodes=arr[1], pairs_offered=arr[2], pairs_tested=arr[3], nodes_per_packet=arr[1] / n,
+                    pairs_offered_per_packet=arr[2] / n, pairs_tested_per_packet=arr[3] / n)
 
     def sdf_query(self, points: torch.Tensor, search: str = "bvh"):
         p = _dev_f32(points, "points").reshape(-1, 3)
diff --git a/include/icon_amd.h b/include/icon_amd.h
--- a/include/icon_amd.h
+++ b/include/icon_amd.h
@@ -147,6 +147,9 @@
 int icon_work_set_tie_rule(icon_work_t *work, int rule, int ulps);
 
 int icon_debug_traversal_stats(const icon_mesh_t *mesh, int res, int z0, int z1, uint64_t out[4]);
+int icon_debug_pair_stats(const icon_mesh_t *mesh, int res, int z0, int z1, uint64_t out[4]);
+int icon_debug_pair_box(const float *corners, int64_t n_pairs, const float *pts, int64_t n_pts, int shared_pts,
+                        float *rec, int32_t *kind, float *bound);
 
 int icon_volume_any_above(const float *d_occ, int res, int sx, int sy, int sz, float level, icon_work_t *work, void *stream, int *h_any);
 
```
